# beehive-lab/GPULlama3.java

Measured on NVIDIA H100. Metric: decode_tokens_per_s, higher is better.
Workload: dtype q8_0xq8_0->int32, f32 accumulate

## Files before the change

### gpullama3.java_b200/csrc/decode_kernels.cuh

```cuda
#pragma once
#include "common.cuh"
#include "seqsum2.cuh"

enum { MODE_STORE = 0, MODE_RESID = 1 };

__device__ __forceinline__ float emb_get_raw(const DevMat &e, int token, int i) {
    size_t idx = (size_t)token * e.cols + i;
    if (e.type == 8) {
        float q = (float)((const int8_t *)e.qs)[idx];
        return __fmul_rn(q, __half2float(e.sc[idx >> 5]));
    } else if (e.type == 1) {
        return __half2float(((const __half *)e.qs)[idx]);
    }
    return ((const float *)e.qs)[idx];
}
__device__ __forceinline__ float emb_get(const DevMat &e, int token, int i, float es) { return __fmul_rn(emb_get_raw(e, token, i), es); }

#define NORM_THREADS SEQSUM2_THREADS
__host__ __device__ inline int norm_padded(int dim) { return (dim + SEQSUM2_THREADS - 1) / SEQSUM2_THREADS * SEQSUM2_THREADS; }
__host__ __device__ inline size_t norm_smem_bytes(int dim) { return (size_t)norm_padded(dim) * 4 + 16 + seqsum2_scratch_bytes(); }

template <bool EMBED>
__device__ __forceinline__ void rmsnorm_quant_row(float *__restrict__ x, const int *__restrict__ tok, const DevMat &emb, float emb_scale,
                                                  const float *__restrict__ w, float eps, int dim, int8_t *__restrict__ xq,
                                                  float *__restrict__ xs, float *__restrict__ xb, long long *__restrict__ prof,
                                                  const TraceBuf &tr, const TpCtx &tp, int tp_wait_op) {
    extern __shared__ __align__(16) float sm[];
    float *sq = sm;
    __shared__ float s_ss;
    const int tid = threadIdx.x;
    long long t0 = 0, t1 = 0, t2 = 0, t3 = 0;
    if (prof) t0 = clock64();
    trace_entry(tr);
    pdl_launch_dependents();
    pdl_wait();
    trace_mark(tr, 2);
    if (prof) t1 = clock64();
    if (tp.n > 1 && tp_wait_op >= 0) {
        if (tid == 0) tp_wait(tp, TP_SLOT_X, tp_seq(tp, (unsigned)tp_wait_op));
        __syncthreads();
    }
    int token = 0;
    if (EMBED) token = *tok;
    for (int i = tid; i < dim; i += NORM_THREADS) {
        float v;
        if (EMBED) { v = emb_get(emb, token, i, emb_scale); x[i] = v; }
        else v = ldcg_f32c(x + i);
        sq[i] = __fmul_rn(v, v);
    }
    for (int i = dim + tid; i < norm_padded(dim); i += NORM_THREADS) sq[i] = 0.0f;
    __syncthreads();
    if (prof) t2 = clock64();
    int info0 = 0, info1 = 0;
    SeqSum2Scratch scratch = seqsum2_carve(reinterpret_cast<unsigned char *>(sm + norm_padded(dim)));
    float ss = block_seqsum_exact_v2(sq, dim, scratch);
    if (prof && tid == 0) { info0 = scratch.info[0]; info1 = scratch.info[1]; }
    if (prof) t3 = clock64();
    if (EMBED) __threadfence_block();
    if (tid == 0) {
        ss = __fdiv_rn(ss, (float)dim);
        ss = __fadd_rn(ss, eps);
        s_ss = (float)(1.0 / sqrt((double)ss));
    }
    __syncthreads();
    ss = s_ss;
    const int lane = tid & 31, warp = tid >> 5;
    constexpr int NWN = NORM_THREADS / 32;
    const int nb = dim / 32;
#pragma unroll 1
    for (int b0 = warp; b0 < nb; b0 += 4 * NWN) {
        float xv[4], wv[4];
#pragma unroll
        for (int u = 0; u < 4; u++) {
            const int b = b0 + u * NWN;
            xv[u] = 0.0f; wv[u] = 0.0f;
            if (b < nb) { xv[u] = ldcg_f32c(x + b * 32 + lane); wv[u] = w[b * 32 + lane]; }
        }
#pragma unroll
        for (int u = 0; u < 4; u++) {
            const int b = b0 + u * NWN;
            if (b < nb) {
                const int i = b * 32 + lane;
                const float v = __fmul_rn(wv[u], __fmul_rn(ss, xv[u]));
                if (xb) xb[i] = v;
                if (xq) {
                    float as;
                    int q = quant_block_lane(v, as);
                    xq[i] = (int8_t)q;
                    if (lane == 0) xs[b] = as;
                }
            }
        }
    }
    trace_mark(tr, 3);
    if (prof) {
        __syncthreads();
        if (tid == 0) { long long t4 = clock64(); prof[0] = t1 - t0; prof[1] = t2 - t1; prof[2] = t3 - t2; prof[3] = t4 - t3;
                        prof[4] = info0; prof[5] = info1; prof[6] = 0; }
    }
}

template <bool EMBED>
__global__ void __launch_bounds__(NORM_THREADS, 1) k_rmsnorm_quant(float *__restrict__ x, const StepState *__restrict__ st,
                                                               DevMat emb, float emb_scale, const float *__restrict__ w, float eps, int dim,
                                                               int8_t *__restrict__ xq, float *__restrict__ xs,
                                                               float *__restrict__ xb, long long *__restrict__ prof, TraceBuf tr, TpCtx tp, int tp_wait_op) {
    rmsnorm_quant_row<EMBED>(x, &st->token, emb, emb_scale, w, eps, dim, xq, xs, xb, prof, tr, tp, tp_wait_op);
}

template <int T>
__global__ void __launch_bounds__(T, 1) k_test_seqsum2(const float *__restrict__ terms, int n, float *__restrict__ out, int *__restrict__ info) {
    extern __shared__ __align__(16) float sm[];
    float *sq = sm;
    const int E = (n + T - 1) / T, np = T * E;
    SeqSum2Scratch scratch = seqsum2_carve(reinterpret_cast<unsigned char *>(sm + np), T);
    for (int i = threadIdx.x; i < np; i += T) sq[i] = i < n ? terms[i] : 0.0f;
    if (threadIdx.x == 0) { scratch.info[0] = -1; scratch.info[1] = -2; }
    __syncthreads();
    const float s = block_seqsum_exact_v2_t<T>(sq, n, scratch, (int)threadIdx.x, SeqSum2BlockSync());
    if (threadIdx.x == 0) { out[0] = s; info[0] = scratch.info[0]; info[1] = scratch.info[1]; }
}

template <int R>
__device__ __forceinline__ void q8_row_terms(const int8_t *__restrict__ qs, const __half *__restrict__ sc, size_t row0,
                                             int cols, int nb, const int4 *__restrict__ sxq, const float *__restrict__ sxs,
                                             float *__restrict__ terms, int nbp, int lane) {
    constexpr int JB = R >= 4 ? 2 : 4;
    for (int b0 = 0; b0 < nb; b0 += 32 * JB) {
        int wv[R][JB][8];
        __half sv[R][JB];
#pragma unroll
        for (int r = 0; r < R; r++)
#pragma unroll
            for (int j = 0; j < JB; j++) {
                int b = b0 + j * 32 + lane;
                if (b < nb) {
                    ldg256_stream(qs + (row0 + r) * (size_t)cols + (size_t)b * 32, wv[r][j]);
                    sv[r][j] = sc[(row0 + r) * (size_t)nb + b];
                }
            }
#pragma unroll
        for (int j = 0; j < JB; j++) {
            int b = b0 + j * 32 + lane;
            if (b < nb) {
                int4 a0 = sxq[b], a1 = sxq[nb + b];
                float as = sxs[b];
#pragma unroll
                for (int r = 0; r < R; r++) {
                    int isum = __dp4a(wv[r][j][0], a0.x, 0);
                    isum = __dp4a(wv[r][j][1], a0.y, isum);
                    isum = __dp4a(wv[r][j][2], a0.z, isum);
                    isum = __dp4a(wv[r][j][3], a0.w, isum);
                    isum = __dp4a(wv[r][j][4], a1.x, isum);
                    isum = __dp4a(wv[r][j][5], a1.y, isum);
                    isum = __dp4a(wv[r][j][6], a1.z, isum);
                    isum = __dp4a(wv[r][j][7], a1.w, isum);
                    terms[r * nbp + b] = __fmul_rn((float)isum, __fmul_rn(__half2float(sv[r][j]), as));
                }
            }
        }
    }
}

__device__ __forceinline__ void stage_activation(const int8_t *__restrict__ xq, const float *__restrict__ xs, int cols,
                                                 int4 *sxq, float *sxs) {
    const int nb = cols >> 5;
    const int4 *src = reinterpret_cast<const int4 *>(xq);
    for (int c = threadIdx.x; c < cols / 16; c += blockDim.x) sxq[(c & 1) * nb + (c >> 1)] = src[c];
    for (int b = threadIdx.x; b < nb; b += blockDim.x) sxs[b] = xs[b];
}

__host__ __device__ inline size_t q8_smem_bytes(int cols, int rows_per_warp, int warps) {
    int nb = cols / 32, nbp = nb | 1;
    return (size_t)cols + (size_t)nb * 4 + (size_t)warps * rows_per_warp * nbp * 4 + 64;
}

template <int R, int MODE>
__global__ void __launch_bounds__(256) k_matvec_q8(const int8_t *__restrict__ qs, const __half *__restrict__ sc,
                                                   const int8_t *__restrict__ xq, const float *__restrict__ xs, int rows,
                                                   int cols, float *__restrict__ out, float oscale) {
    extern __shared__ __align__(16) unsigned char smraw[];
    const int nb = cols >> 5, nbp = nb | 1;
    int4 *sxq = reinterpret_cast<int4 *>(smraw);
    float *sxs = reinterpret_cast<float *>(smraw + cols);
    float *terms_all = sxs + nb;
    stage_activation(xq, xs, cols, sxq, sxs);
    __syncthreads();
    const int lane = threadIdx.x & 31, warp = threadIdx.x >> 5;
    float *terms = terms_all + (size_t)warp * R * nbp;
    const int nwarps_total = gridDim.x * (blockDim.x >> 5);
    for (size_t row0 = (size_t)(blockIdx.x * (blockDim.x >> 5) + warp) * R; row0 < (size_t)rows; row0 += (size_t)nwarps_total * R) {
        q8_row_terms<R>(qs, sc, row0, cols, nb, sxq, sxs, terms, nbp, lane);
        __syncwarp();
        if (lane < R) {
            const float *t = terms + lane * nbp;
            float acc = 0.0f;
            for (int b = 0; b < nb; b++) acc = __fadd_rn(acc, t[b]);
            size_t row = row0 + lane;
            acc = __fmul_rn(acc, oscale);
            if (MODE == MODE_RESID) out[row] = __fadd_rn(out[row], acc);
            else out[row] = acc;
        }
        __syncwarp();
    }
}

__device__ __forceinline__ float swiglu(float g, float u) {
    float s = __fdiv_rn(g, (float)(1.0 + exp((double)(-g))));
    return __fmul_rn(s, u);
}

__global__ void __launch_bounds__(256) k_gateup_q8(const int8_t *__restrict__ qs1, const __half *__restrict__ sc1,
                                                   const int8_t *__restrict__ qs3, const __half *__restrict__ sc3,
                                                   const int8_t *__restrict__ xq, const float *__restrict__ xs, int hidden,
                                                   int cols, int8_t *__restrict__ hq, float *__restrict__ hs,
                                                   float *__restrict__ hb_dbg) {
    extern __shared__ __align__(16) unsigned char smraw[];
    __shared__ float hvals[32];
    const int nb = cols >> 5, nbp = nb | 1;
    int4 *sxq = reinterpret_cast<int4 *>(smraw);
    float *sxs = reinterpret_cast<float *>(smraw + cols);
    float *terms_all = sxs + nb;
    stage_activation(xq, xs, cols, sxq, sxs);
    __syncthreads();
    const int lane = threadIdx.x & 31, warp = threadIdx.x >> 5;
    float *terms = terms_all + (size_t)warp * 4 * nbp;
    for (int blk = blockIdx.x; blk < hidden / 32; blk += gridDim.x) {
#pragma unroll 1
        for (int half = 0; half < 2; half++) {
            int u0 = blk * 32 + warp * 4 + half * 2;
            q8_row_terms<2>(qs1, sc1, (size_t)u0, cols, nb, sxq, sxs, terms, nbp, lane);
            q8_row_terms<2>(qs3, sc3, (size_t)u0, cols, nb, sxq, sxs, terms + 2 * nbp, nbp, lane);
            __syncwarp();
            float acc = 0.0f;
            if (lane < 4) {
                const float *t = terms + lane * nbp;
                for (int b = 0; b < nb; b++) acc = __fadd_rn(acc, t[b]);
            }
            float up = __shfl_down_sync(0xffffffffu, acc, 2);
            if (lane < 2) hvals[warp * 4 + half * 2 + lane] = swiglu(acc, up);
            __syncwarp();
        }
        __syncthreads();
        if (warp == 0) {
            float v = hvals[lane];
            if (hb_dbg) hb_dbg[blk * 32 + lane] = v;
            float as;
            int q = quant_block_lane(v, as);
            hq[blk * 32 + lane] = (int8_t)q;
            if (lane == 0) hs[blk] = as;
        }
        __syncthreads();
    }
}

template <int MODE>
__global__ void __launch_bounds__(256) k_matvec_f16(const __half *__restrict__ w, const float *__restrict__ x, int rows,
                                                    int cols, int lanes, float *__restrict__ out, float oscale) {
    extern __shared__ __align__(16) unsigned char smraw[];
    float *sx = reinterpret_cast<float *>(smraw);
    constexpr int TC = 256;
    __half *tiles = reinterpret_cast<__half *>(smraw + (size_t)cols * 4);
    for (int i = threadIdx.x; i < cols; i += blockDim.x) sx[i] = x[i];
    __syncthreads();
    const int lane = threadIdx.x & 31, warp = threadIdx.x >> 5;
    const int L = lanes > 0 ? lanes : 1;
    const int RW = 32 / L;
    __half *tile = tiles + (size_t)warp * RW * TC;
    const int r = lane / L, c = lane % L;
    const int nwarps_total = gridDim.x * (blockDim.x >> 5);
    const int upper = lanes > 0 ? cols - (cols % L) : 0;
    for (size_t row0 = (size_t)(blockIdx.x * (blockDim.x >> 5) + warp) * RW; row0 < (size_t)rows; row0 += (size_t)nwarps_total * RW) {
        float acc = 0.0f;
        for (int c0 = 0; c0 < cols; c0 += TC) {
            int tc = min(TC, cols - c0);
            int chunks_per_row = tc >> 3;
            for (int q = lane; q < RW * chunks_per_row; q += 32) {
                int rr = q / chunks_per_row, cc = q % chunks_per_row;
                size_t row = row0 + rr;
                int4 v = make_int4(0, 0, 0, 0);
                if (row < (size_t)rows) v = ldg128_stream(w + row * (size_t)cols + c0 + cc * 8);
                *reinterpret_cast<int4 *>(tile + rr * TC + cc * 8) = v;
            }
            __syncwarp();
            if (lanes > 0) {
                int lim = min(tc, upper - c0);
                for (int i = c; i < lim; i += L) {
                    float wf = f16_bits_to_f32_daz(__half_as_ushort(tile[r * TC + i]));
                    acc = fmaf(wf, sx[c0 + i], acc);
                }
            } else {
                for (int i = 0; i < tc; i++) acc = __fadd_rn(acc, __fmul_rn(__half2float(tile[r * TC + i]), sx[c0 + i]));
            }
            __syncwarp();
        }
        float result = acc;
        if (lanes > 0) {
            result = 0.0f;
            for (int k = 0; k < L; k++) {
                float a = __shfl_sync(0xffffffffu, acc, r * L + k);
                result = __fadd_rn(result, a);
            }
            size_t row = row0 + r;
            if (row < (size_t)rows)
                for (int j = upper; j < cols; j++)
                    result = __fadd_rn(result, __fmul_rn(__half2float(w[row * (size_t)cols + j]), sx[j]));
        }
        size_t row = row0 + r;
        if (c == 0 && row < (size_t)rows) {
            result = __fmul_rn(result, oscale);
            if (MODE == MODE_RESID) out[row] = __fadd_rn(out[row], result);
            else out[row] = result;
        }
    }
}

__global__ void k_swiglu(float *__restrict__ hb, const float *__restrict__ hb2, int n) {
    int i = blockIdx.x * blockDim.x + threadIdx.x;
    if (i < n) hb[i] = swiglu(hb[i], hb2[i]);
}

#define ATT_THREADS 512

template <int HS>
__device__ __forceinline__ void rope_kv_prologue(float *qkv, const float *qsrc, const float *ksrc, const float *vsrc, float *kc, float *vc, int pos,
                                                 int h, int kv_mul, int kvh, int qd, int kvd, const float *cr, const float *ci, int arch,
                                                 const float *qnorm_w, const float *knorm_w, const float *qkv_bias, float eps, float *sq, float *sk,
                                                 float *so, float *s_val) {
    const int tid = threadIdx.x;
    constexpr int HALF = HS / 2;
    if (tid < HS) {
        const bool is_q = tid < HALF;
        const int p = is_q ? tid : tid - HALF;
        const float *src = is_q ? qsrc : ksrc;
        int i0, i1;
        if (arch & KF_NEOX) { i0 = p; i1 = p + HALF; } else { i0 = 2 * p; i1 = 2 * p + 1; }
        float v0 = src[i0], v1 = src[i1];
        if (arch & KF_QKVBIAS) {
            const float *b = qkv_bias + (is_q ? h * HS : qd + kvh * HS);
            v0 = __fadd_rn(v0, b[i0]);
            v1 = __fadd_rn(v1, b[i1]);
        }
        if (arch & KF_QKNORM) {
            float *sqr = is_q ? so : sk;
            sqr[i0] = __fmul_rn(v0, v0);
            sqr[i1] = __fmul_rn(v1, v1);
        }
        if (arch & KF_QKNORM) {
            asm volatile("bar.sync 3, %0;" ::"n"(HS) : "memory");
            if (p == 0) {
                const float *sqr = is_q ? so : sk;
                float ss = 0.0f;
                for (int i = 0; i < HS; i++) ss = __fadd_rn(ss, sqr[i]);
                ss = __fdiv_rn(ss, (float)HS);
                ss = __fadd_rn(ss, eps);
                s_val[is_q ? 0 : 1] = (float)(1.0 / sqrt((double)ss));
            }
            asm volatile("bar.sync 3, %0;" ::"n"(HS) : "memory");
            const float ss = s_val[is_q ? 0 : 1];
            const float *nw = is_q ? qnorm_w : knorm_w;
            v0 = __fmul_rn(nw[i0], __fmul_rn(ss, v0));
            v1 = __fmul_rn(nw[i1], __fmul_rn(ss, v1));
            asm volatile("bar.sync 3, %0;" ::"n"(HS) : "memory");
        }
        const float fcr = cr[(size_t)pos * HALF + p], fci = ci[(size_t)pos * HALF + p];
        const float r0 = __fsub_rn(__fmul_rn(v0, fcr), __fmul_rn(v1, fci));
        const float r1 = __fadd_rn(__fmul_rn(v0, fci), __fmul_rn(v1, fcr));
        float *dst = is_q ? sq : sk;
        dst[i0] = r0;
        dst[i1] = r1;
        if (h % kv_mul == 0) {
            if (!is_q) {
                const size_t o = (size_t)pos * kvd + kvh * HS;
                kc[o + i0] = r0;
                kc[o + i1] = r1;
            }
        }
        if (is_q) { qkv[h * HS + i0] = r0; qkv[h * HS + i1] = r1; }
    } else if (tid < 2 * HS) {
        const int j = tid - HS;
        float w = vsrc[j];
        if (arch & KF_QKVBIAS) {
            w = __fadd_rn(w, qkv_bias[qd + kvd + kvh * HS + j]);
            so[j] = w;
        }
        if (h % kv_mul == 0) vc[(size_t)pos * kvd + kvh * HS + j] = w;
    }
}

template <bool CG, typename T> __device__ __forceinline__ T kv_ld(const T *p) {
    if constexpr (CG) return __ldcg(p);
    else return __ldg(p);
}

template <int HS, bool CACHED = false>
__device__ __forceinline__ void attention_head(float *__restrict__ qkv, float *__restrict__ kc, float *__restrict__ vc,
                                               const int *__restrict__ posp, const float *__restrict__ cr, const float *__restrict__ ci,
                                               int n_heads, int n_kv_heads, int arch, const float *__restrict__ qnorm_w,
                                               const float *__restrict__ knorm_w, const float *__restrict__ qkv_bias, float eps, float sqrt_hs,
                                               int8_t *__restrict__ xq, float *__restrict__ xs, float *__restrict__ xb, const TraceBuf &tr,
                                               const TpCtx &tp, unsigned tp_out_op, int head_base, float *att_scratch, int ctx) {
    extern __shared__ __align__(16) float sm[];
    __shared__ float red[ATT_THREADS / 32];
    __shared__ float s_val[2];
    float *sq = sm, *sk = sm + HS, *so = sm + 2 * HS;
    float *att = att_scratch ? att_scratch + (size_t)blockIdx.x * ctx : sm + 3 * HS;
    const int h = blockIdx.x, tid = threadIdx.x, lane = tid & 31, warp = tid >> 5;
    trace_entry(tr);
    pdl_launch_dependents();
    const int kv_mul = n_heads / n_kv_heads, kvh = h / kv_mul;
    const int qd = n_heads * HS, kvd = n_kv_heads * HS;
    pdl_wait();
    trace_mark(tr, 2);
    const int pos = *posp, nt = pos + 1;
    {
        constexpr int LINES = HS / 32;
        for (int i = tid; i < pos * LINES; i += ATT_THREADS) {
            const size_t off = (size_t)(i / LINES) * kvd + kvh * HS + (i % LINES) * 32;
            asm volatile("prefetch.global.L2 [%0];" ::"l"(kc + off));
            asm volatile("prefetch.global.L2 [%0];" ::"l"(vc + off));
        }
    }
    const float *qsrc = qkv + h * HS, *ksrc = qkv + qd + kvh * HS, *vsrc = qkv + qd + kvd + kvh * HS;
// ... 229 lines not shown
```

### gpullama3.java_b200/csrc/decode_persistent.cuh

```cuda
#pragma once
#include "decode_kernels.cuh"
#include "norm_slots.cuh"
#include "seqsum2.cuh"
#include "stream_matvec.cuh"

#define PD_WARPS 16
#define PD_CT (PD_WARPS * 32)
#define PD_THREADS (PD_CT + 32)
#define PD_MAX_STAGES 32
#define PD_TIMEOUT_NS 4000000000ull
#define PD_STAMPS 20

enum { PD_S_QKV = 0, PD_S_ATT = 1, PD_S_WO = 2, PD_S_GU = 3, PD_S_W2 = 4, PD_S_LM = 5, PD_S_ARG = 6, PD_S_SLOTS = 8,
       PD_S_TICK = 8, PD_S_LMTICK = 9, PD_S_ERR = 10, PD_S_WORDS = 16 };

struct PdLayer {
    TileMat qkv, wo, gu, w2;
    const float *attn_norm, *ffn_norm, *q_norm, *k_norm;
    const float *qkv_bias;
    float *kc, *vc;
};

struct PdArgs {
    const PdLayer *layers;
    int n_layers;
    TileMat lm_head;
    const float *out_norm;
    DevMat emb;
    int dim, hidden, qd;
    int n_heads, n_kv_heads;
    int head_size, arch , ctx;
    float eps, sqrt_hs;
    float emb_scale, res_scale, logit_scale;
    const float *rope_cr, *rope_ci;
    StepState *st;
    const int *seq_tokens;
    int *out_ids;
    float *x, *qkv, *hb, *logits;
    int8_t *attq;
    float *atts;
    int8_t *hq;
    float *hs;
    unsigned *blk_cnt;
    float *part_val;
    int *part_idx;
    unsigned *sync;
    unsigned *host_err;
    float *att_scratch;
    unsigned long long *trace;
    int with_logits;
    TpCtx tp;
    unsigned pd_flags_off;
    int head_base, dim_base, hid_base, voc_base;
};

struct PdSmem {
    size_t off_bar, off_xq, off_xs, off_nbuf, off_wbuf, off_rope, off_seq, off_terms, off_hvals, off_misc, off_ring, total;
    int stages, stage_bytes, tstride, nbuf_floats;
};

__host__ __device__ inline PdSmem pd_layout(int dim, int qd, int hidden, int head_size, int att_floats, int max_seg, size_t budget) {
    PdSmem L;
    const int unit = smv_unit_bytes(max_seg);
    L.stage_bytes = (4 * unit + 127) & ~127;
    L.tstride = ((max_seg / 32 + 3) & ~3) + 4;
    int maxc = dim > qd ? dim : qd;
    if (hidden > maxc) maxc = hidden;
    const int E = (dim + PD_CT - 1) / PD_CT;
    const int sq_floats = PD_CT * seqsum2_stride(E);
    L.nbuf_floats = sq_floats > att_floats ? sq_floats : att_floats;
    size_t o = 0;
    L.off_bar = o; o += 2 * PD_MAX_STAGES * 8 + PD_MAX_STAGES * 4;
    o = (o + 15) & ~(size_t)15;
    L.off_xq = o; o += (size_t)maxc;
    L.off_xs = o; o += (size_t)(maxc / 32) * 4;
    o = (o + 15) & ~(size_t)15;
    L.off_nbuf = o; o += (size_t)L.nbuf_floats * 4;
    o = (o + 15) & ~(size_t)15;
    L.off_wbuf = o; o += (size_t)dim * 4;
    L.off_rope = o; o += (size_t)head_size * 4;
    o = (o + 15) & ~(size_t)15;
    L.off_seq = o; o += seqsum2_scratch_bytes(PD_CT);
    o = (o + 15) & ~(size_t)15;
    L.off_terms = o; o += (size_t)PD_WARPS * 4 * L.tstride * 4;
    L.off_hvals = o; o += SMV_HVALS * 4;
    L.off_misc = o; o += 96 * 4;
    o = (o + 127) & ~(size_t)127;
    L.off_ring = o;
    long room = (long)budget - (long)o;
    int s = room > 0 ? (int)(room / L.stage_bytes) : 0;
    if (s > PD_MAX_STAGES) s = PD_MAX_STAGES;
    L.stages = s;
    L.total = o + (size_t)s * L.stage_bytes;
    return L;
}

__device__ __forceinline__ unsigned pd_ld_relaxed_gpu(const unsigned *p) {
    unsigned v;
    asm volatile("ld.relaxed.gpu.global.u32 %0, [%1];" : "=r"(v) : "l"(p) : "memory");
    return v;
}
__device__ __forceinline__ unsigned pd_ld_relaxed_sys(const unsigned *p) {
    unsigned v;
    asm volatile("ld.relaxed.sys.global.u32 %0, [%1];" : "=r"(v) : "l"(p) : "memory");
    return v;
}
template <bool SYS> __device__ __noinline__ void pd_spin(const unsigned *p, unsigned target, unsigned *err, unsigned *host_err, unsigned code) {
    unsigned it = 0;
    unsigned long long t0 = 0;
    for (;;) {
        const unsigned v = SYS ? pd_ld_relaxed_sys(p) : pd_ld_relaxed_gpu(p);
        if ((int)(v - target) >= 0) {
            unsigned w;
            if (SYS) asm volatile("ld.acquire.sys.global.u32 %0, [%1];" : "=r"(w) : "l"(p) : "memory");
            else asm volatile("ld.acquire.gpu.global.u32 %0, [%1];" : "=r"(w) : "l"(p) : "memory");
            return;
        }
        if ((++it & 255u) == 0u) {
            if (*reinterpret_cast<volatile unsigned *>(err)) return;
            const unsigned long long now = gtime();
            if (!t0) t0 = now;
            else if (now - t0 > PD_TIMEOUT_NS) {
                atomicCAS(err, 0u, code);
                *reinterpret_cast<volatile unsigned *>(host_err) = code;
                return;
            }
        }
    }
}

__device__ __forceinline__ void pd_bar_sync() { asm volatile("bar.sync 1, %0;" ::"n"(PD_CT) : "memory"); }

struct PdConsumerSync {
    __device__ __forceinline__ void operator()() const { pd_bar_sync(); }
};

__device__ __noinline__ void pd_arrive(const PdArgs &a, int slot, unsigned target, unsigned epoch, bool cross, int tid) {
    pd_bar_sync();
    if (tid == 0) {
        const bool x = cross && a.tp.n > 1;
        __threadfence();
        const unsigned old = atomicAdd(a.sync + slot, 1u);
        if (x && old + 1u == target) {
            __threadfence_system();
            for (int k = 0; k < a.tp.n; k++) {
                unsigned *f = reinterpret_cast<unsigned *>(a.tp.peer[k] + a.pd_flags_off) + slot * TP_MAX + a.tp.rank;
                asm volatile("st.relaxed.sys.global.u32 [%0], %1;" ::"l"(f), "r"(epoch) : "memory");
            }
        }
    }
}
__device__ __noinline__ void pd_wait(const PdArgs &a, int slot, unsigned target, unsigned epoch, bool cross, int tid) {
    if (tid == 0) {
        if (cross && a.tp.n > 1) {
            const unsigned *f = reinterpret_cast<const unsigned *>(a.tp.peer[a.tp.rank] + a.pd_flags_off) + slot * TP_MAX;
            for (int k = 0; k < a.tp.n; k++) pd_spin<true>(f + k, epoch, a.sync + PD_S_ERR, a.host_err, 1u + (unsigned)slot);
        } else pd_spin<false>(a.sync + slot, target, a.sync + PD_S_ERR, a.host_err, 1u + (unsigned)slot);
    }
    pd_bar_sync();
}

__device__ __forceinline__ void pd_stamp(const PdArgs &a, int layer, int k, int tid) {
    if (a.trace && tid == 0) a.trace[((size_t)blockIdx.x * (a.n_layers + 1) + layer) * PD_STAMPS + k] = gtime();
}

struct PdWalk {
    const PdArgs *a;
    int n_mats, mi;
    TileMat W;
    int g1, gb, nw, s, w;
    unsigned tile_bytes;
    __device__ __forceinline__ void open() {
        for (; mi < n_mats; mi++) {
            const int l = mi >> 2;
            if (l < a->n_layers) {
                const PdLayer &Ly = a->layers[l];
                const int k = mi & 3;
                W = k == 0 ? Ly.qkv : k == 1 ? Ly.wo : k == 2 ? Ly.gu : Ly.w2;
            } else W = a->lm_head;
            const int ngroups = tile_groups(W);
            gb = (int)(((long long)blockIdx.x * ngroups) / gridDim.x);
            g1 = (int)(((long long)(blockIdx.x + 1) * ngroups) / gridDim.x);
            if (gb < g1) {
                nw = min(PD_WARPS, g1 - gb);
                s = 0; w = 0;
                tile_bytes = 4u * (unsigned)W.unit_bytes;
                return;
            }
        }
    }
    __device__ __forceinline__ void init(const PdArgs *args) {
        a = args;
        n_mats = 4 * a->n_layers + (a->with_logits ? 1 : 0);
        mi = 0;
        open();
    }
    __device__ __forceinline__ bool valid() const { return mi < n_mats; }
    __device__ __forceinline__ const unsigned char *addr() const { return W.base + ((size_t)(gb + w) * W.nseg + s) * tile_bytes; }
    __device__ __forceinline__ void next() {
        if (++w < nw) return;
        w = 0;
        if (++s < W.nseg) return;
        s = 0;
        gb += PD_WARPS;
        if (gb < g1) { nw = min(PD_WARPS, g1 - gb); return; }
        mi++;
        open();
    }
};

__device__ __forceinline__ void pd_produce(const PdArgs &a, unsigned char *smem, const PdSmem &L, unsigned bar0) {
    const int S = L.stages;
    const unsigned long long pol = l2_policy_evict_first();
    PdWalk cur;
    cur.init(&a);
    for (unsigned seq = 0; cur.valid(); cur.next(), seq++) {
        const int st = seq % S;
        mbar_wait(bar0 + 8 * (PD_MAX_STAGES + st), ((seq / S) & 1u) ^ 1u);
        const unsigned full = bar0 + 8 * st;
        mbar_expect_tx(full, cur.tile_bytes);
        bulk_g2s_evict_first(smem_u32(smem + L.off_ring + (size_t)st * L.stage_bytes), cur.addr(), cur.tile_bytes, full, pol);
    }
}

__device__ __noinline__ float pd_walk_rolled(float acc, const float *t, int nbs) {
    int b = 0;
    if (nbs >= 4) {
        float4 c = *reinterpret_cast<const float4 *>(t);
#pragma unroll 1
        for (; b + 4 <= nbs; b += 4) {
            float4 n = c;
            if (b + 8 <= nbs) n = *reinterpret_cast<const float4 *>(t + b + 4);
            acc = __fadd_rn(acc, c.x); acc = __fadd_rn(acc, c.y); acc = __fadd_rn(acc, c.z); acc = __fadd_rn(acc, c.w);
            c = n;
        }
    }
#pragma unroll 1
    for (; b < nbs; b++) acc = __fadd_rn(acc, t[b]);
    return acc;
}
__device__ __noinline__ float pd_swiglu(float g, float u) { return swiglu_exact(g, u); }
__device__ __noinline__ int pd_quant_block(float v, float *ascale) {
    float as;
    const int q = quant_block_lane(v, as);
    *ascale = as;
    return q;
}
__device__ __noinline__ float pd_emb_get(const DevMat &e, int token, int i, float es) { return emb_get(e, token, i, es); }
__device__ __noinline__ float pd_exp_narrow(float x) { return (float)exp((double)x); }

template <int MODE>
__device__ __noinline__ void pd_consume_matrix(const TileMat &W, const PdArgs &a, unsigned char *smem, const PdSmem &L, unsigned bar0, volatile unsigned *rel,
                                                  unsigned &seq_base, float *out, bool argmax, bool l0_emb, int token, int row_base, int tid) {
    const int lane = tid & 31, warp = tid >> 5, S = L.stages, tstride = L.tstride, stage_bytes = L.stage_bytes;
    const int w_unit = W.unit_bytes, w_seg = W.seg;
    const int ngroups = tile_groups(W);
    const float oscale = MODE == SMV_RESID ? a.res_scale : argmax ? a.logit_scale : 1.0f;
    const int g0 = (int)(((long long)blockIdx.x * ngroups) / gridDim.x), g1 = (int)(((long long)(blockIdx.x + 1) * ngroups) / gridDim.x);
    const int nseg = W.nseg, nbs = w_seg >> 5;
    const unsigned char *ring = smem + L.off_ring;
    const int tp_n = a.tp.n;
    float *terms = reinterpret_cast<float *>(smem + L.off_terms) + (size_t)warp * 4 * tstride;
    const unsigned char *sact = smem + L.off_xq;
    const float *sxs = reinterpret_cast<const float *>(smem + L.off_xs);
    float *hvals = reinterpret_cast<float *>(smem + L.off_hvals);
    const int hsel = (lane >> 2) & 1;
    float best = -INFINITY;
    int best_i = 0x7fffffff;
#pragma unroll 1
    for (int gb = g0; gb < g1; gb += PD_WARPS) {
        const int nw = min(PD_WARPS, g1 - gb);
        if (warp < nw) {
            const int G = gb + warp;
            float acc = 0.0f;
#pragma unroll 1
            for (int s = 0; s < nseg; s++) {
                const unsigned seq = seq_base + (unsigned)(s * nw + warp);
                const int st = seq % S;
                const unsigned lap = seq / S;
                if (lane == 0)
                    while (rel[st] != lap) {}
                __syncwarp();
                mbar_wait(bar0 + 8 * st, lap & 1u);
                const unsigned char *tile = ring + (size_t)st * stage_bytes;
#pragma unroll 1
                for (int b = lane; b < nbs; b += 32) {
                    const unsigned char *ab = sact + ((size_t)(s * nbs + b) << 5);
                    const int4 a0 = *reinterpret_cast<const int4 *>(ab + 16 * hsel);
                    const int4 a1 = *reinterpret_cast<const int4 *>(ab + 16 * (hsel ^ 1));
                    const float as = sxs[s * nbs + b];
#pragma unroll
                    for (int r = 0; r < 4; r++) {
                        const unsigned char *wb = tile + (size_t)r * w_unit + ((size_t)b << 5);
                        const int4 w0 = *reinterpret_cast<const int4 *>(wb + 16 * hsel);
                        const int4 w1 = *reinterpret_cast<const int4 *>(wb + 16 * (hsel ^ 1));
                        const __half sc = *reinterpret_cast<const __half *>(tile + (size_t)r * w_unit + w_seg + 2 * b);
                        int isum = __dp4a(w0.x, a0.x, 0);
                        isum = __dp4a(w0.y, a0.y, isum);
                        isum = __dp4a(w0.z, a0.z, isum);
                        isum = __dp4a(w0.w, a0.w, isum);
                        isum = __dp4a(w1.x, a1.x, isum);
                        isum = __dp4a(w1.y, a1.y, isum);
                        isum = __dp4a(w1.z, a1.z, isum);
                        isum = __dp4a(w1.w, a1.w, isum);
                        terms[r * tstride + b] = __fmul_rn((float)isum, __fmul_rn(__half2float(sc), as));
                    }
                }
                __syncwarp();
                if (lane == 0) {
                    rel[st] = lap + 1u;
                    mbar_arrive(bar0 + 8 * (PD_MAX_STAGES + st));
                }
                if (lane < 4) acc = pd_walk_rolled(acc, terms + lane * tstride, nbs);
                __syncwarp();
            }
            if (MODE == SMV_GATEUP) {
                const float up = __shfl_down_sync(0xffffffffu, acc, 2);
                if (lane < 2) {
                    const int unit = 2 * G + lane;
                    const float hval = pd_swiglu(acc, up);
                    out[unit] = hval;
                    hvals[unit - 2 * g0] = hval;
                }
            } else if (lane < 4 && 4 * G + lane < W.rows) {
                const size_t row = (size_t)4 * G + lane;
                acc = __fmul_rn(acc, oscale);
                if (MODE == SMV_RESID) {
                    const size_t grow = (size_t)row_base + row;
                    const float base = l0_emb ? pd_emb_get(a.emb, token, (int)grow, a.emb_scale) : out[grow];
                    const float v = __fadd_rn(base, acc);
                    if (tp_n > 1) {
                        for (int k = 0; k < tp_n; k++) tp_ptr<float>(a.tp, k, a.tp.off_x)[grow] = v;
                    } else out[grow] = v;
                } else {
                    out[row] = acc;
                    const int grow = row_base + (int)row;
                    if (acc > best) { best = acc; best_i = grow; }
                }
            }
        }
        seq_base += (unsigned)(nseg * nw);
    }
    if (MODE == SMV_GATEUP) {
        pd_bar_sync();
        const int u0 = 2 * g0, u1 = 2 * g1;
        if (u1 > u0) {
            for (int blk = (u0 >> 5) + warp; blk <= ((u1 - 1) >> 5); blk += PD_WARPS) {
                const int lo = max(blk << 5, u0), hi = min((blk << 5) + 32, u1);
                float v = 0.0f;
                bool mine = true;
                if (hi - lo == 32) v = hvals[(blk << 5) + lane - u0];
                else {
                    unsigned old = 0;
                    if (lane == 0) {
                        __threadfence();
                        old = atomicAdd(&a.blk_cnt[blk], (unsigned)(hi - lo));
                    }
                    old = __shfl_sync(0xffffffffu, old, 0);
                    mine = (old + (unsigned)(hi - lo) == 32u);
                    if (mine) {
                        __threadfence();
                        v = ldcg_f32(out + (blk << 5) + lane);
                        if (lane == 0) a.blk_cnt[blk] = 0u;
                    }
                }
                if (mine) {
                    float as;
                    const int q = pd_quant_block(v, &as);
                    const int gblk = (row_base >> 5) + blk;
                    if (a.tp.n > 1) {
                        for (int k = 0; k < a.tp.n; k++) {
                            tp_ptr<int8_t>(a.tp, k, a.tp.off_hq)[(gblk << 5) + lane] = (int8_t)q;
                            if (lane == 0) tp_ptr<float>(a.tp, k, a.tp.off_hs)[gblk] = as;
                        }
                    } else {
                        a.hq[(gblk << 5) + lane] = (int8_t)q;
                        if (lane == 0) a.hs[gblk] = as;
                    }
                }
            }
        }
    } else if (MODE == SMV_STORE && argmax) {
        int *cand_i = reinterpret_cast<int *>(hvals + 64);
        pd_bar_sync();
        if (lane < 4) { hvals[warp * 4 + lane] = best; cand_i[warp * 4 + lane] = best_i; }
        pd_bar_sync();
        if (tid == 0) {
            float bv = -INFINITY;
            int bi = 0x7fffffff;
            for (int k = 0; k < PD_WARPS * 4; k++) {
                const float v = hvals[k];
                const int ix = cand_i[k];
                if (v > bv || (v == bv && ix < bi)) { bv = v; bi = ix; }
            }
            a.part_val[blockIdx.x] = bv;
            a.part_idx[blockIdx.x] = bi;
        }
    }
}

__device__ __noinline__ float pd_seqsum(const float *sq, int n, int S, unsigned char *smem, const PdSmem &L, int tid) {
    SeqSum2Scratch scratch = seqsum2_carve(smem + L.off_seq, PD_CT);
    return block_seqsum_exact_v2_t<PD_CT>(sq, n, scratch, tid, PdConsumerSync(), S);
}

__device__ __forceinline__ void pd_prefetch_w(const float *w, float *sbuf, int dim, int tid) {
    const int n4 = dim >> 2;
    for (int i4 = tid; i4 < n4; i4 += PD_CT)
        asm volatile("cp.async.cg.shared.global [%0], [%1], 16;" ::"r"(smem_u32(sbuf + 4 * i4)), "l"(w + 4 * i4) : "memory");
    asm volatile("cp.async.commit_group;" ::: "memory");
}

struct PdNormOps {
    const PdArgs &a;
    const float *wbuf;
    unsigned char *smem;
    const PdSmem &L;
    int tid, stamp_layer;
    __device__ __forceinline__ void sync() const { pd_bar_sync(); }
    __device__ __forceinline__ float seqsum(const float *sq, int n, int S) const { return pd_seqsum(sq, n, S, smem, L, tid); }
    __device__ __forceinline__ float emb(int token, int i) const { return pd_emb_get(a.emb, token, i, a.emb_scale); }
    __device__ __forceinline__ float4 x4(int i4) const { return ldcg_f32x4(a.x + 4 * i4); }
    __device__ __forceinline__ void store_x(int, float4) const {}
    __device__ __forceinline__ float scale(float ss, int dim, float eps) const {
        float *misc = reinterpret_cast<float *>(smem + L.off_misc);
        if (tid == 0) {
            ss = __fdiv_rn(ss, (float)dim);
            ss = __fadd_rn(ss, eps);
            misc[20] = (float)(1.0 / sqrt((double)ss));
        }
        asm volatile("cp.async.wait_group 0;" ::: "memory");
        pd_bar_sync();
        return misc[20];
    }
    template <int U> __device__ __forceinline__ float4 w4(const float4 (&)[U], int, int i4) const { return *reinterpret_cast<const float4 *>(wbuf + 4 * i4); }
    __device__ __forceinline__ void stamp(int k) const { if (stamp_layer >= 0) pd_stamp(a, stamp_layer, k, tid); }
};

template <int U>
__device__ __noinline__ void pd_norm_u(const PdArgs &a, const float *wbuf, bool from_emb, int token, unsigned char *smem, const PdSmem &L, int tid, int stamp_layer) {
    const float4 wv[U] = {};
    norm_quant_slots<PD_CT, U>(PdNormOps{a, wbuf, smem, L, tid, stamp_layer}, from_emb, token, a.dim, a.eps, wv, reinterpret_cast<float *>(smem + L.off_nbuf),
                               reinterpret_cast<unsigned *>(smem + L.off_xq), reinterpret_cast<float *>(smem + L.off_xs), tid);
}

__device__ __forceinline__ void pd_norm_to_smem(const PdArgs &a, const float *wbuf, bool from_emb, int token, unsigned char *smem, const PdSmem &L, int tid, int stamp_layer = -1) {
    const int U = ((a.dim >> 2) + PD_CT - 1) / PD_CT;
    if (U <= 1) pd_norm_u<1>(a, wbuf, from_emb, token, smem, L, tid, stamp_layer);
    else if (U == 2) pd_norm_u<2>(a, wbuf, from_emb, token, smem, L, tid, stamp_layer);
    else pd_norm_u<4>(a, wbuf, from_emb, token, smem, L, tid, stamp_layer);
}

__device__ __noinline__ void pd_load_act(const int8_t *q, const float *s, int cols, unsigned char *smem, const PdSmem &L, int tid) {
    int4 *sxq = reinterpret_cast<int4 *>(smem + L.off_xq);
    float *sxs = reinterpret_cast<float *>(smem + L.off_xs);
    const int4 *src = reinterpret_cast<const int4 *>(q);
    const int n16 = cols >> 4, nb = cols >> 5;
    for (int c0 = 0; c0 < n16; c0 += 4 * PD_CT) {
        int4 v[4];
        float sc[2];
#pragma unroll
        for (int u = 0; u < 4; u++) {
            const int c = c0 + u * PD_CT + tid;
            v[u] = c < n16 ? __ldcg(src + c) : make_int4(0, 0, 0, 0);
        }
#pragma unroll
        for (int u = 0; u < 2; u++) {
            const int b = (c0 >> 1) + u * PD_CT + tid;
            sc[u] = b < nb ? __ldcg(s + b) : 0.0f;
        }
#pragma unroll
        for (int u = 0; u < 4; u++) {
            const int c = c0 + u * PD_CT + tid;
            if (c < n16) sxq[c] = v[u];
        }
#pragma unroll
        for (int u = 0; u < 2; u++) {
            const int b = (c0 >> 1) + u * PD_CT + tid;
            if (b < nb) sxs[b] = sc[u];
        }
    }
    pd_bar_sync();
}

template <int HS>
__device__ __noinline__ void pd_attention_head(const PdArgs &a, const PdLayer &Ly, int h, int pos, unsigned char *smem, const PdSmem &L, int tid, int layer) {
    float *sm = reinterpret_cast<float *>(smem + L.off_nbuf);
    float *misc = reinterpret_cast<float *>(smem + L.off_misc);
    float *red = misc, *s_val = misc + 16;
    float *sq = sm, *sk = sm + HS, *so = sm + 2 * HS;
    const int ctx_pad = (a.ctx + PD_CT - 1) / PD_CT * PD_CT;
    float *att = a.att_scratch ? a.att_scratch + (size_t)h * ctx_pad : sm + 3 * HS;
    const int lane = tid & 31, warp = tid >> 5;
    constexpr int HALF = HS / 2;
    const int nt = pos + 1;
    const int kv_mul = a.n_heads / a.n_kv_heads, kvh = h / kv_mul;
    const int qd = a.n_heads * HS, kvd = a.n_kv_heads * HS;
    float *qkv = a.qkv, *kc = Ly.kc, *vc = Ly.vc;
    const float *qsrc = qkv + h * HS, *ksrc = qkv + qd + kvh * HS, *vsrc = qkv + qd + kvd + kvh * HS;
    float vcur_own = 0.0f;
    if (tid < HS) {
        const bool is_q = tid < HALF;
        const int p = is_q ? tid : tid - HALF;
        const float *src = is_q ? qsrc : ksrc;
        int i0, i1;
        if (a.arch & KF_NEOX) { i0 = p; i1 = p + HALF; } else { i0 = 2 * p; i1 = 2 * p + 1; }
        float v0 = ldcg_f32c(src + i0), v1 = ldcg_f32c(src + i1);
        if (a.arch & KF_QKVBIAS) {
            const float *b = Ly.qkv_bias + (is_q ? h * HS : qd + kvh * HS);
            v0 = __fadd_rn(v0, b[i0]);
            v1 = __fadd_rn(v1, b[i1]);
        }
        const float *srope = reinterpret_cast<const float *>(smem + L.off_rope);
        const float fcr = srope[p], fci = srope[HALF + p];
        const bool owner = (h % kv_mul == 0) && !is_q;
        if (a.arch & KF_QKNORM) {
            float *sqr = is_q ? so : sk;
            sqr[i0] = __fmul_rn(v0, v0);
            sqr[i1] = __fmul_rn(v1, v1);
            asm volatile("bar.sync 3, %0;" ::"n"(HS) : "memory");
            if (p == 0) {
                float ss = 0.0f;
                for (int i = 0; i < HS; i++) ss = __fadd_rn(ss, sqr[i]);
                ss = __fdiv_rn(ss, (float)HS);
                ss = __fadd_rn(ss, a.eps);
                s_val[is_q ? 0 : 1] = (float)(1.0 / sqrt((double)ss));
            }
            asm volatile("bar.sync 3, %0;" ::"n"(HS) : "memory");
            const float ss = s_val[is_q ? 0 : 1];
            const float *nw = is_q ? Ly.q_norm : Ly.k_norm;
            v0 = __fmul_rn(nw[i0], __fmul_rn(ss, v0));
            v1 = __fmul_rn(nw[i1], __fmul_rn(ss, v1));
            asm volatile("bar.sync 3, %0;" ::"n"(HS) : "memory");
        }
        const float r0 = __fsub_rn(__fmul_rn(v0, fcr), __fmul_rn(v1, fci));
        const float r1 = __fadd_rn(__fmul_rn(v0, fci), __fmul_rn(v1, fcr));
        float *dst = is_q ? sq : sk;
        dst[i0] = r0;
        dst[i1] = r1;
        if (owner) {
            const size_t o = (size_t)pos * kvd + kvh * HS;
            kc[o + i0] = r0;
            kc[o + i1] = r1;
        }
    } else if (tid < 2 * HS) {
        const int j = tid - HS;
        vcur_own = ldcg_f32c(vsrc + j);
        if (a.arch & KF_QKVBIAS) vcur_own = __fadd_rn(vcur_own, Ly.qkv_bias[qd + kvd + kvh * HS + j]);
        if (h % kv_mul == 0) vc[(size_t)pos * kvd + kvh * HS + j] = vcur_own;
    }
    pd_bar_sync();
    if (tid >= HS && tid < 2 * HS) so[tid - HS] = vcur_own;
    constexpr int QE = HS / 4, QV = HS / 16;
    const int quad = tid & 3, qbase = lane & ~3;
    constexpr int VB = 32;
    const int vd = tid >> 2;
    const bool vlive = vd < HS;
    float vv[VB];
    {
        const float *vcol = vc + kvh * HS + vd;
        const int vt0 = quad * VB;
#pragma unroll
        for (int u = 0; u < VB; u++) vv[u] = (vlive && vt0 + u < pos) ? __ldcg(vcol + (size_t)(vt0 + u) * kvd) : 0.0f;
    }
    float lmax = -INFINITY;
#pragma unroll 1
    for (int t0 = 0; t0 < nt; t0 += PD_CT / 4) {
        const int t = t0 + (tid >> 2);
        float4 kk[QV];
        if (t < pos) {
            const float4 *k = reinterpret_cast<const float4 *>(kc + (size_t)t * kvd + kvh * HS + quad * QE);
#pragma unroll
            for (int u = 0; u < QV; u++) kk[u] = __ldcg(k + u);
        } else {
#pragma unroll
            for (int u = 0; u < QV; u++) kk[u] = t == pos ? *reinterpret_cast<const float4 *>(sk + quad * QE + 4 * u) : make_float4(0.f, 0.f, 0.f, 0.f);
        }
        float acc = 0.0f;
#pragma unroll 1
        for (int qd = 0; qd < 4; qd++) {
            if (quad == qd) {
                const float *qq = sq + qd * QE;
#pragma unroll
                for (int u = 0; u < QV; u++) {
                    acc = __fadd_rn(acc, __fmul_rn(qq[4 * u + 0], kk[u].x));
                    acc = __fadd_rn(acc, __fmul_rn(qq[4 * u + 1], kk[u].y));
                    acc = __fadd_rn(acc, __fmul_rn(qq[4 * u + 2], kk[u].z));
                    acc = __fadd_rn(acc, __fmul_rn(qq[4 * u + 3], kk[u].w));
                }
            }
            acc = __shfl_sync(0xffffffffu, acc, qbase + qd);
        }
        if (quad == 0 && t < nt) {
            const float sc = (a.arch & KF_ATTSCALE) ? __fmul_rn(acc, a.sqrt_hs) : __fdiv_rn(acc, a.sqrt_hs);
            att[t] = sc;
            lmax = fmaxf(lmax, sc);
        }
    }
    lmax = warp_max_f(lmax);
    if (lane == 0) red[warp] = lmax;
    pd_bar_sync();
    pd_stamp(a, layer, 13, tid);
    float mx = red[0];
#pragma unroll
    for (int w = 1; w < PD_WARPS; w++) mx = fmaxf(mx, red[w]);
    for (int t = tid; t < nt; t += PD_CT) att[t] = pd_exp_narrow(__fsub_rn(att[t], mx));
    pd_bar_sync();
    float sum;
    if (nt >= 512) {
        const int E = (nt + PD_CT - 1) / PD_CT;
        for (int t = nt + tid; t < PD_CT * E; t += PD_CT) att[t] = 0.0f;
        pd_bar_sync();
        sum = pd_seqsum(att, nt, 0, smem, L, tid);
    } else {
        if (tid == 0) s_val[0] = seq2_literal(0.0f, att, nt, (reinterpret_cast<uintptr_t>(att) & 15) == 0);
        pd_bar_sync();
        sum = s_val[0];
    }
    for (int t = tid; t < nt; t += PD_CT) att[t] = __fdiv_rn(att[t], sum);
    pd_bar_sync();
    pd_stamp(a, layer, 14, tid);
    {
        const float *vcol = vc + kvh * HS + vd;
        const float vcur = vlive ? so[vd] : 0.0f;
        float acc = 0.0f;
#pragma unroll 1
        for (int r0 = 0; r0 < pos; r0 += 4 * VB) {
            if (r0 > 0) {
                const int vt0 = r0 + quad * VB;
#pragma unroll
                for (int u = 0; u < VB; u++) vv[u] = (vlive && vt0 + u < pos) ? __ldcg(vcol + (size_t)(vt0 + u) * kvd) : 0.0f;
            }
#pragma unroll 1
            for (int qd = 0; qd < 4; qd++) {
                if (quad == qd) {
                    const int vt0 = r0 + qd * VB;
#pragma unroll
                    for (int u = 0; u < VB; u++)
                        if (vt0 + u < pos) acc = __fadd_rn(__fmul_rn(att[vt0 + u], vv[u]), acc);
                }
                acc = __shfl_sync(0xffffffffu, acc, qbase + qd);
            }
        }
        if (vlive && quad == 0) so[vd] = __fadd_rn(__fmul_rn(att[pos], vcur), acc);
    }
    pd_bar_sync();
    const int gh = a.head_base + h;
    for (int b = warp; b < HS / 32; b += PD_WARPS) {
        float as;
        const int q = pd_quant_block(so[b * 32 + lane], &as);
        if (a.tp.n > 1) {
            for (int k = 0; k < a.tp.n; k++) {
                tp_ptr<int8_t>(a.tp, k, a.tp.off_attq)[gh * HS + b * 32 + lane] = (int8_t)q;
                if (lane == 0) tp_ptr<float>(a.tp, k, a.tp.off_atts)[(gh * HS) / 32 + b] = as;
            }
        } else {
            a.attq[gh * HS + b * 32 + lane] = (int8_t)q;
            if (lane == 0) a.atts[(gh * HS) / 32 + b] = as;
        }
    }
    pd_stamp(a, layer, 15, tid);
}

template <int HS>
__global__ void __launch_bounds__(PD_THREADS, 1) k_decode_persistent(const __grid_constant__ PdArgs a, const __grid_constant__ PdSmem L) {
    extern __shared__ __align__(128) unsigned char smem[];
    const int tid = threadIdx.x, lane = tid & 31, warp = tid >> 5;
    const int S = L.stages;
    const unsigned bar0 = smem_u32(smem + L.off_bar);
    volatile unsigned *rel = reinterpret_cast<volatile unsigned *>(smem + L.off_bar + 2 * PD_MAX_STAGES * 8);
    if (tid == 0) {
        for (int s = 0; s < S; s++) {
            mbar_init(bar0 + 8 * s, 1);
            mbar_init(bar0 + 8 * (PD_MAX_STAGES + s), 1);
            rel[s] = 0u;
        }
        asm volatile("fence.mbarrier_init.release.cluster;" ::: "memory");
    }
    __syncthreads();

    if (warp == PD_WARPS) {
        if (lane == 0) pd_produce(a, smem, L, bar0);
        return;
    }

    const int token = a.st->token, pos = a.st->pos;
    const unsigned tick = *reinterpret_cast<volatile unsigned *>(a.sync + PD_S_TICK);
    const unsigned lmtick = *reinterpret_cast<volatile unsigned *>(a.sync + PD_S_LMTICK);
    const unsigned nC = gridDim.x, nL = (unsigned)a.n_layers, nH = (unsigned)a.n_heads;
    float *wbufA = reinterpret_cast<float *>(smem + L.off_wbuf), *wbufF = wbufA;
    pd_prefetch_w(a.n_layers ? a.layers[0].attn_norm : a.out_norm, wbufA, a.dim, tid);
    if (tid < a.head_size) {
        const int half = a.head_size >> 1;
        float *srope = reinterpret_cast<float *>(smem + L.off_rope);
        srope[tid] = tid < half ? __ldg(a.rope_cr + (size_t)pos * half + tid) : __ldg(a.rope_ci + (size_t)pos * half + (tid - half));
    }
    unsigned seq_base = 0;
#pragma unroll 1
    for (int l = 0; l < a.n_layers; l++) {
        const PdLayer &Ly = a.layers[l];
        const unsigned e = tick * nL + (unsigned)l + 1u;
        pd_stamp(a, l, 0, tid);
        pd_norm_to_smem(a, wbufA, l == 0, token, smem, L, tid, l);
        if (a.trace && l == 1) {
            const int E = (a.dim + PD_CT - 1) / PD_CT;
            pd_stamp(a, l, 16, tid);
            const float again = pd_seqsum(reinterpret_cast<const float *>(smem + L.off_nbuf), a.dim, seqsum2_stride(E), smem, L, tid);
            if (tid == 0) reinterpret_cast<float *>(smem + L.off_misc)[30] = again;
            pd_stamp(a, l, 17, tid);
        }
        pd_prefetch_w(Ly.ffn_norm, wbufF, a.dim, tid);
        pd_stamp(a, l, 1, tid);
        pd_consume_matrix<SMV_STORE>(Ly.qkv, a, smem, L, bar0, rel, seq_base, a.qkv, false, false, token, 0, tid);
        pd_stamp(a, l, 2, tid);
        if (blockIdx.x < nH) {
            const int kvh = (int)blockIdx.x / (a.n_heads / a.n_kv_heads), kvd = a.n_kv_heads * a.head_size;
            const int lines = a.head_size >> 5;
            for (int i = tid; i < pos * lines; i += PD_CT) {
                const size_t off = (size_t)(i / lines) * kvd + kvh * a.head_size + (i % lines) * 32;
                asm volatile("prefetch.global.L2 [%0];" ::"l"(Ly.kc + off));
                asm volatile("prefetch.global.L2 [%0];" ::"l"(Ly.vc + off));
            }
        }
        pd_arrive(a, PD_S_QKV, e * nC, e, false, tid);
        if (blockIdx.x < nH) {
            pd_wait(a, PD_S_QKV, e * nC, e, false, tid);
            pd_stamp(a, l, 12, tid);
            pd_attention_head<HS>(a, Ly, blockIdx.x, pos, smem, L, tid, l);
            pd_arrive(a, PD_S_ATT, e * nH, e, true, tid);
        }
        pd_wait(a, PD_S_ATT, e * nH, e, true, tid);
        pd_stamp(a, l, 3, tid);
        pd_load_act(a.attq, a.atts, a.qd, smem, L, tid);
        pd_consume_matrix<SMV_RESID>(Ly.wo, a, smem, L, bar0, rel, seq_base, a.x, false, l == 0, token, a.dim_base, tid);
        pd_stamp(a, l, 4, tid);
        pd_arrive(a, PD_S_WO, e * nC, e, true, tid);
        pd_wait(a, PD_S_WO, e * nC, e, true, tid);
        pd_stamp(a, l, 5, tid);
        pd_norm_to_smem(a, wbufF, false, token, smem, L, tid);
        pd_prefetch_w(l + 1 < a.n_layers ? a.layers[l + 1].attn_norm : a.out_norm, wbufA, a.dim, tid);
        pd_stamp(a, l, 6, tid);
        pd_consume_matrix<SMV_GATEUP>(Ly.gu, a, smem, L, bar0, rel, seq_base, a.hb, false, false, token, a.hid_base, tid);
        pd_stamp(a, l, 7, tid);
        pd_arrive(a, PD_S_GU, e * nC, e, true, tid);
        pd_wait(a, PD_S_GU, e * nC, e, true, tid);
        pd_load_act(a.hq, a.hs, a.hidden, smem, L, tid);
        pd_stamp(a, l, 8, tid);
        pd_consume_matrix<SMV_RESID>(Ly.w2, a, smem, L, bar0, rel, seq_base, a.x, false, false, token, a.dim_base, tid);
        pd_stamp(a, l, 9, tid);
        pd_arrive(a, PD_S_W2, e * nC, e, true, tid);
        pd_wait(a, PD_S_W2, e * nC, e, true, tid);
    }
    int best_i = 0;
    if (a.with_logits) {
        const unsigned le = lmtick + 1u;
        pd_stamp(a, a.n_layers, 0, tid);
        pd_norm_to_smem(a, wbufA, false, token, smem, L, tid);
        pd_stamp(a, a.n_layers, 1, tid);
        pd_consume_matrix<SMV_STORE>(a.lm_head, a, smem, L, bar0, rel, seq_base, a.logits, true, false, token, a.voc_base, tid);
        pd_stamp(a, a.n_layers, 2, tid);
        pd_arrive(a, PD_S_LM, le * nC, le, false, tid);
        if (blockIdx.x != 0) return;
        pd_wait(a, PD_S_LM, le * nC, le, false, tid);
        float best = -INFINITY;
        best_i = 0x7fffffff;
        for (int i = tid; i < (int)nC; i += PD_CT) argmax_merge(best, best_i, ldcg_f32c(a.part_val + i), __ldcg(a.part_idx + i));
#pragma unroll
        for (int o = 16; o > 0; o >>= 1) {
            const float ov = __shfl_xor_sync(0xffffffffu, best, o);
            const int oi = __shfl_xor_sync(0xffffffffu, best_i, o);
            argmax_merge(best, best_i, ov, oi);
        }
        float *sv = reinterpret_cast<float *>(smem + L.off_misc) + 32;
        int *si = reinterpret_cast<int *>(sv + 16);
        if (lane == 0) { sv[warp] = best; si[warp] = best_i; }
        pd_bar_sync();
        if (tid == 0) {
            best = sv[0]; best_i = si[0];
            for (int w = 1; w < PD_WARPS; w++) argmax_merge(best, best_i, sv[w], si[w]);
            if (a.tp.n > 1) {
                for (int k = 0; k < a.tp.n; k++) {
                    tp_ptr<float>(a.tp, k, a.tp.off_pv)[a.tp.rank] = best;
                    tp_ptr<int>(a.tp, k, a.tp.off_pi)[a.tp.rank] = best_i;
                }
                __threadfence_system();
                for (int k = 0; k < a.tp.n; k++) {
                    unsigned *f = reinterpret_cast<unsigned *>(a.tp.peer[k] + a.pd_flags_off) + PD_S_ARG * TP_MAX + a.tp.rank;
                    asm volatile("st.relaxed.sys.global.u32 [%0], %1;" ::"l"(f), "r"(le) : "memory");
                }
                const unsigned *f = reinterpret_cast<const unsigned *>(a.tp.peer[a.tp.rank] + a.pd_flags_off) + PD_S_ARG * TP_MAX;
                for (int k = 0; k < a.tp.n; k++) pd_spin<true>(f + k, le, a.sync + PD_S_ERR, a.host_err, 1u + PD_S_ARG);
                best = -INFINITY; best_i = 0x7fffffff;
                for (int k = 0; k < a.tp.n; k++)
                    argmax_merge(best, best_i, ldcg_f32c(tp_ptr<float>(a.tp, a.tp.rank, a.tp.off_pv) + k),
                                 __float_as_int(ldcg_f32c(reinterpret_cast<const float *>(tp_ptr<int>(a.tp, a.tp.rank, a.tp.off_pi)) + k)));
            }
            if (best_i == 0x7fffffff) best_i = 0;
        }
    } else if (blockIdx.x != 0) {
        return;
    }
    if (tid == 0) {
        StepState *st = a.st;
        const int step = st->step;
        if (a.with_logits && a.out_ids) a.out_ids[step] = best_i;
        const int next = step + 1;
        if (st->feedback && a.with_logits) st->token = best_i;
        else if (next < st->n_seq) st->token = a.seq_tokens[next];
        st->step = next;
        st->pos = st->pos + 1;
        *reinterpret_cast<volatile unsigned *>(a.sync + PD_S_TICK) = tick + 1u;
        if (a.with_logits) *reinterpret_cast<volatile unsigned *>(a.sync + PD_S_LMTICK) = lmtick + 1u;
        pd_stamp(a, a.n_layers, 3, tid);
    }
}
```

### gpullama3.java_b200/csrc/plan.cu

```cuda
#include "../../include/b200llama.h"
#include "decode_kernels.cuh"
#include "prefill.cuh"
#include "stream_matvec.cuh"
#include "stream_matvec_f16.cuh"
#include "kquant.cuh"
#include "decode_persistent.cuh"
#include "sampler.cuh"
#include "decode_batch.cuh"
#include "moe.cuh"

#include <math.h>
#include <stdarg.h>
#include <stdio.h>
#include <stdlib.h>
#include <string.h>

#include <chrono>
#include <string>
#include <thread>
#include <utility>
#include <vector>

namespace {

// ... 2169 lines not shown
                        (long long)start_positions[i] + lengths[i] - 1, c.context_length);
        off[i] = (int)total;
        total += lengths[i];
    }
    if (total && !tokens) return fail(p, B200_ERR_BAD_ARG, "tokens must not be NULL");
    for (int i = 0; i < n_seqs; i++)
        for (int j = 0; j < lengths[i]; j++)
            if (tokens[off[i] + j] < 0 || tokens[off[i] + j] >= c.vocab_size)
                return fail(p, B200_ERR_BAD_ARG, "sequence %d: token %d (index %d) out of range", i, tokens[off[i] + j], j);
    const PrefillCtx &pc = p->prefill;
    const bool tc = (pc.ready && pc.mode == B200_PREFILL_TENSOR_CORE) || (pc.q8_ready && pc.mode == B200_PREFILL_TENSOR_CORE_W8A16);
    if (tc && total > p->prefill_batch) {
        int i = 0;
        while (off[i] + lengths[i] <= p->prefill_batch) i++;
        return fail(p, B200_ERR_BAD_ARG, "sequence %d: the call's %lld tokens exceed prefill_batch_size %d (split the prompts into chunks)", i, (long long)total,
                    p->prefill_batch);
    }
    if (!total) return B200_OK;
    CK(cudaSetDevice(p->device));
    return tc ? prefill_slots_tc(p, n_seqs, slots, start_positions, lengths, off.data(), tokens, (int)total)
              : prefill_slots_exact(p, n_seqs, slots, start_positions, lengths, off.data(), tokens);
}

int b200_decode_multi_rows(b200_plan *p, int32_t *max_rows) {
    if (!p || !max_rows) return B200_ERR_BAD_ARG;
    *max_rows = multi_why(p) ? 0 : batch_max_rows(p);
    return B200_OK;
}

int b200_forward_decode_multi(b200_plan *p, int32_t slot, int32_t n, const int32_t *tokens, int32_t start_pos, int32_t *ids_out, float *logits) {
    if (!p) return B200_ERR_BAD_ARG;
    if (const char *why = multi_why(p)) return fail(p, B200_ERR_UNSUPPORTED, "%s", why);
    auto &B = p->bt;
    const b200_config &c = p->cfg;
    const int R = batch_max_rows(p);
    if (!tokens || !ids_out) return fail(p, B200_ERR_BAD_ARG, "tokens and ids_out must not be NULL");
    if (n < 1 || n > R) return fail(p, B200_ERR_BAD_ARG, "n = %d rows: need 1 <= n <= %d (b200_decode_multi_rows)", n, R);
    if (slot < -1 || slot >= B.n_slots) return fail(p, B200_ERR_BAD_ARG, "slot %d out of range (%d slots; -1 is the plan's own cache)", slot, B.n_slots);
    for (int i = 0; i < n; i++) {
        if (tokens[i] < 0 || tokens[i] >= c.vocab_size) return fail(p, B200_ERR_BAD_ARG, "row %d: token %d out of range", i, tokens[i]);
        if (start_pos < 0 || (int64_t)start_pos + i >= c.context_length)
            return fail(p, B200_ERR_BAD_ARG, "row %d: position %lld outside the KV cache (%d)", i, (long long)start_pos + i, c.context_length);
    }
    CK(cudaSetDevice(p->device));
    int rc;
    if ((rc = multi_ready(p))) return rc;
    const bool own = slot < 0;
    if (!B.gs[own][1][n] && (rc = capture_batch(p, n, false, true, own))) return rc;
    for (int i = 0; i < n; i++) { B.h_rows->token[i] = tokens[i]; B.h_rows->pos[i] = start_pos + i; B.h_rows->slot[i] = own ? 0 : slot; }
    CK(cudaMemcpyAsync(B.rows, B.h_rows, sizeof(BatchRows), cudaMemcpyHostToDevice, p->stream));
    CK(cudaGraphLaunch(B.gs[own][1][n], p->stream));
    const size_t vpad = (size_t)sampler_padded(c.vocab_size);
    if (logits)
        for (int i = 0; i < n; i++) CK(cudaMemcpyAsync(logits + (size_t)i * c.vocab_size, B.logits + i * vpad, (size_t)c.vocab_size * 4, cudaMemcpyDeviceToHost, p->stream));
    CK(cudaMemcpyAsync(B.h_out, B.ids, (size_t)n * 4, cudaMemcpyDeviceToHost, p->stream));
    CK(cudaStreamSynchronize(p->stream));
    memcpy(ids_out, B.h_out, (size_t)n * 4);
    return B200_OK;
}

int b200_batch_info(b200_plan *p, int32_t *n_slots, int32_t *launches_per_step, float *device_ms_last_step) {
    if (!p) return B200_ERR_BAD_ARG;
    if (n_slots) *n_slots = p->bt.n_slots;
    if (launches_per_step) *launches_per_step = p->bt.last_n ? p->bt.launches[p->bt.last_n] : 0;
    if (device_ms_last_step) *device_ms_last_step = p->bt.last_ms;
    return B200_OK;
}

int b200_read_buffer(b200_plan *p, const char *name, int32_t layer, void *dst, size_t bytes) {
    if (!p || !name || !dst) return B200_ERR_BAD_ARG;
    const b200_config &c = p->cfg;
    const void *src = nullptr;
    size_t sz = 0;
    std::string s = name;
    size_t ctx_kv = (size_t)c.context_length * p->kvd_l;
    if (s == "x") { src = p->x; sz = (size_t)c.dim * 4; }
    else if (s == "xb") { src = p->xb; sz = (size_t)(c.dim > p->qd ? c.dim : p->qd) * 4; }
    else if (s == "q" || s == "qkv") { src = p->qkv; sz = (size_t)(p->qd_l + 2 * p->kvd_l) * 4; }
    else if (s == "hb") { src = p->hb; sz = (size_t)(c.hidden_dim > p->moe_hv ? c.hidden_dim : p->moe_hv) * 4; }
    else if (s == "logits") { src = p->logits; sz = (size_t)c.vocab_size * 4; }
    else if (s == "xq") { src = p->xq; sz = (size_t)(c.dim > p->qd ? c.dim : p->qd); }
    else if (s == "xs") { src = p->xs; sz = (size_t)((c.dim > p->qd ? c.dim : p->qd) / 32) * 4; }
    else if (s == "hq") { src = p->hq; sz = (size_t)(c.hidden_dim > p->moe_hv ? c.hidden_dim : p->moe_hv); }
    else if (s == "hs") { src = p->hs; sz = (size_t)((c.hidden_dim > p->moe_hv ? c.hidden_dim : p->moe_hv) / 32) * 4; }
    else if (s == "moe_ids" || s == "moe_weights") {
        if (!p->is_moe) return fail(p, B200_ERR_BAD_ARG, "%s: not a Qwen2-MoE plan", name);
        const size_t k = (size_t)p->moe.n_experts_used;
        if (s == "moe_ids") { src = p->moe_ids; sz = (size_t)c.n_layers * k * 4; }
        else { src = p->moe_w; sz = (size_t)c.n_layers * (k + 1) * 4; }
    }
    else if (s == "key_cache" || s == "value_cache") {
        if (layer < 0 || layer >= c.n_layers) return fail(p, B200_ERR_BAD_ARG, "layer out of range");
        src = (s == "key_cache" ? p->key_cache : p->value_cache) + (size_t)layer * ctx_kv;
        sz = ctx_kv * 4;
    } else if (s == "slot_key_cache" || s == "slot_value_cache") {
        if (layer < 0 || layer >= p->bt.n_slots * c.n_layers) return fail(p, B200_ERR_BAD_ARG, "slot layer %d out of range (%d slots)", layer, p->bt.n_slots);
        src = (s == "slot_key_cache" ? p->bt.slot_k : p->bt.slot_v) + (size_t)layer * ctx_kv;
        sz = ctx_kv * 4;
    } else if (s.rfind("pf_", 0) == 0) {
        const PrefillCtx &pc = p->prefill;
        if (!pc.ready && !pc.q8_ready) return fail(p, B200_ERR_STATE, "%s: the plan has no tensor-core prefill buffers (%s)", name, pc.why);
        const size_t rows = (size_t)pc.bpad;
        if (s == "pf_x") { src = pc.X; sz = rows * c.dim * 4; }
        else if (s == "pf_qkv") { src = pc.QKV; sz = rows * (p->qd + 2 * p->kvd) * 4; }
        else if (s == "pf_a16") { src = pc.A16; sz = rows * c.dim * 2; }
        else if (s == "pf_att16") { src = pc.ATT16; sz = rows * p->qd * 2; }
        else if (s == "pf_h16") { src = pc.H16; sz = rows * c.hidden_dim * 2; }
        else return fail(p, B200_ERR_BAD_ARG, "unknown buffer %s", name);
    } else return fail(p, B200_ERR_BAD_ARG, "unknown buffer %s", name);
    if (bytes < sz) sz = bytes;
    CK(cudaSetDevice(p->device));
    CK(cudaStreamSynchronize(p->stream));
    CK(cudaMemcpy(dst, src, sz, cudaMemcpyDeviceToHost));
    return B200_OK;
}

int b200_time_kernel(b200_plan *p, int32_t which, int32_t reps, float *avg_ms, int64_t *algorithmic_bytes) {
    if (!p || !avg_ms || reps <= 0) return B200_ERR_BAD_ARG;
    if (p->cfg.tp_size > 1) return fail(p, B200_ERR_UNSUPPORTED, "b200_time_kernel is single-GPU only");
    if (p->is_moe) return fail(p, B200_ERR_UNSUPPORTED, "b200_time_kernel times the dense FFN and attention matrices; a Qwen2-MoE plan has no dense FFN");
    const b200_config &c = p->cfg;
    const bool q8 = p->wtype == B200_GGML_Q8_0;
    CK(cudaSetDevice(p->device));
    std::vector<float> save(c.dim);
    CK(cudaStreamSynchronize(p->stream));
    CK(cudaMemcpy(save.data(), p->x, (size_t)c.dim * 4, cudaMemcpyDeviceToHost));
    if (p->use_stream) {
        auto tb = [&](const TileMat &m) -> int64_t { return (int64_t)m.rows * m.cols / 32 * 34; };
        int64_t bytes = 0;
        int launches = 0, rc;
        auto one = [&](int l) -> int {
            LayerW &L = p->layers[l];
            bool keep = p->use_pdl;
            p->use_pdl = false;
            int r;
            const bool fz = p->fuse_norm;
            const int64_t nw = fz ? (int64_t)c.dim * 4 : 0;
            switch (which) {
            case 0:
                bytes = tb(L.tgu) + nw;
                r = fz ? launch_stream_norm<SMV_GATEUP>(p, L.tgu, L.ffn_norm, false, p->hb, p->hq, p->hs, false, TraceBuf{nullptr, 0, 0})
                       : launch_stream<SMV_GATEUP>(p, L.tgu, p->xq, p->xs, p->hb, p->hq, p->hs);
                break;
            case 1: bytes = tb(L.tw2); r = launch_stream<SMV_RESID>(p, L.tw2, p->hq, p->hs, p->x, nullptr, nullptr); break;
            case 2:
                bytes = tb(L.tqkv) + nw;
                r = fz ? launch_stream_norm<SMV_STORE>(p, L.tqkv, L.attn_norm, false, p->qkv, nullptr, nullptr, false, TraceBuf{nullptr, 0, 0})
                       : launch_stream<SMV_STORE>(p, L.tqkv, p->xq, p->xs, p->qkv, nullptr, nullptr);
                break;
            case 3: bytes = tb(L.two); r = launch_stream<SMV_RESID>(p, L.two, p->xq, p->xs, p->x, nullptr, nullptr); break;
            default:
                bytes = tb(p->tout) + nw;
                r = fz ? launch_stream_norm<SMV_STORE>(p, p->tout, p->out_norm, false, p->logits, nullptr, nullptr, false, TraceBuf{nullptr, 0, 0})
                       : launch_stream<SMV_STORE>(p, p->tout, p->xq, p->xs, p->logits, nullptr, nullptr);
                break;
            }
            p->use_pdl = keep;
            return r;
        };
        if (which < 0 || which > 4) return fail(p, B200_ERR_BAD_ARG, "unknown kernel id %d", which);
        for (int l = 0; l < c.n_layers; l++) if ((rc = one(l))) return rc;
        CK(cudaEventRecord(p->ev0, p->stream));
        for (int r = 0; r < reps; r++)
            for (int l = 0; l < c.n_layers; l++) { if ((rc = one(l))) return rc; launches++; }
        CK(cudaEventRecord(p->ev1, p->stream));
        CK(cudaStreamSynchronize(p->stream));
        float ms = 0;
        CK(cudaEventElapsedTime(&ms, p->ev0, p->ev1));
        *avg_ms = ms / launches;
        if (algorithmic_bytes) *algorithmic_bytes = bytes;
        CK(cudaMemcpy(p->x, save.data(), (size_t)c.dim * 4, cudaMemcpyHostToDevice));
        return B200_OK;
    }
    auto mat_bytes = [&](const DevMat &m) -> int64_t {
        int64_t e = (int64_t)m.rows * m.cols;
        return q8 ? e / 32 * 34 : e * 2;
    };
    int64_t bytes = 0;
    int launches = 0;
    const bool sf = p->use_f16_stream;
    auto one = [&](int l) -> int {
        LayerW &L = p->layers[l];
        if (sf) {
            const bool keep = p->use_pdl;
            p->use_pdl = false;
            int r;
            switch (which) {
            case 0: bytes = mat_bytes(L.w1) + mat_bytes(L.w3); r = launch_stream_f16<SF_GATEUP>(p, L.w1, &L.w3, p->xb, p->hb); break;
            case 1: bytes = mat_bytes(L.w2); r = launch_stream_f16<SF_RESID>(p, L.w2, nullptr, p->hb, p->x); break;
            case 2: bytes = mat_bytes(L.qkv); r = launch_stream_f16<SF_STORE>(p, L.qkv, nullptr, p->xb, p->qkv); break;
            case 3: bytes = mat_bytes(L.wo); r = launch_stream_f16<SF_RESID>(p, L.wo, nullptr, p->xb, p->x); break;
            default: bytes = mat_bytes(p->out); r = launch_stream_f16<SF_STORE>(p, p->out, nullptr, p->xb, p->logits); break;
            }
            p->use_pdl = keep;
            return r;
        }
        switch (which) {
        case 0:
            if (q8) {
                k_gateup_q8<<<c.hidden_dim / 32, 256, q8_smem_bytes(c.dim, 4, 8), p->stream>>>(
                    (const int8_t *)L.w1.qs, L.w1.sc, (const int8_t *)L.w3.qs, L.w3.sc, p->xq, p->xs, c.hidden_dim, c.dim, p->hq, p->hs, p->hb);
                CK(cudaGetLastError());
            } else {
                int rc;
                if ((rc = launch_matvec_f16<MODE_STORE>(p, L.w1, p->xb, p->hb))) return rc;
                if ((rc = launch_matvec_f16<MODE_STORE>(p, L.w3, p->xb, p->hb2))) return rc;
            }
            bytes = mat_bytes(L.w1) + mat_bytes(L.w3);
            return B200_OK;
        case 1: bytes = mat_bytes(L.w2); return q8 ? launch_matvec_q8<MODE_RESID>(p, L.w2, p->hq, p->hs, p->x) : launch_matvec_f16<MODE_RESID>(p, L.w2, p->hb, p->x);
        case 2: bytes = mat_bytes(L.qkv); return q8 ? launch_matvec_q8<MODE_STORE>(p, L.qkv, p->xq, p->xs, p->qkv) : launch_matvec_f16<MODE_STORE>(p, L.qkv, p->xb, p->qkv);
        case 3: bytes = mat_bytes(L.wo); return q8 ? launch_matvec_q8<MODE_RESID>(p, L.wo, p->xq, p->xs, p->x) : launch_matvec_f16<MODE_RESID>(p, L.wo, p->xb, p->x);
        default: bytes = mat_bytes(p->out); return q8 ? launch_matvec_q8<MODE_STORE>(p, p->out, p->xq, p->xs, p->logits) : launch_matvec_f16<MODE_STORE>(p, p->out, p->xb, p->logits);
        }
    };
    if (which < 0 || which > 4) return fail(p, B200_ERR_BAD_ARG, "unknown kernel id %d", which);
    int rc;
    for (int l = 0; l < c.n_layers; l++) if ((rc = one(l))) return rc;
    CK(cudaEventRecord(p->ev0, p->stream));
    for (int r = 0; r < reps; r++)
        for (int l = 0; l < c.n_layers; l++) { if ((rc = one(l))) return rc; launches++; }
    CK(cudaEventRecord(p->ev1, p->stream));
    CK(cudaStreamSynchronize(p->stream));
    float ms = 0;
    CK(cudaEventElapsedTime(&ms, p->ev0, p->ev1));
    *avg_ms = ms / launches;
    if (algorithmic_bytes) *algorithmic_bytes = bytes;
    CK(cudaMemcpy(p->x, save.data(), (size_t)c.dim * 4, cudaMemcpyHostToDevice));
    return B200_OK;
}

int b200_tp_handle(b200_plan *p, void *handle64) {
    if (!p || !handle64) return B200_ERR_BAD_ARG;
    if (p->cfg.tp_size <= 1 || !p->comm) return fail(p, B200_ERR_STATE, "not a tensor-parallel plan");
    CK(cudaSetDevice(p->device));
    cudaIpcMemHandle_t h;
    CK(cudaIpcGetMemHandle(&h, p->comm));
    static_assert(sizeof(cudaIpcMemHandle_t) == 64, "IPC handle size");
    memcpy(handle64, &h, 64);
    return B200_OK;
}

int b200_tp_attach(b200_plan *p, const void *handles, int32_t n) {
    if (!p || !handles) return B200_ERR_BAD_ARG;
    if (p->cfg.tp_size <= 1 || !p->comm) return fail(p, B200_ERR_STATE, "not a tensor-parallel plan");
    if (n != p->cfg.tp_size) return fail(p, B200_ERR_BAD_ARG, "expected %d handles, got %d", p->cfg.tp_size, n);
    if (p->attached) return fail(p, B200_ERR_STATE, "already attached");
    CK(cudaSetDevice(p->device));
    for (int k = 0; k < n; k++) {
        if (k == p->cfg.tp_rank) { p->tp.peer[k] = p->comm; continue; }
        cudaIpcMemHandle_t h;
        memcpy(&h, (const unsigned char *)handles + (size_t)k * 64, 64);
        void *ptr = nullptr;
        CK(cudaIpcOpenMemHandle(&ptr, h, cudaIpcMemLazyEnablePeerAccess));
        p->peer_open[k] = ptr;
        p->tp.peer[k] = (unsigned char *)ptr;
    }
    p->tp.n = n;
    p->attached = true;
    int rc;
    if ((rc = capture_all(p))) return rc;
    CK(cudaStreamSynchronize(p->stream));
    return B200_OK;
}

int b200_trace_decode(b200_plan *p, int32_t token, int32_t position, uint64_t *records, int32_t cap, int32_t *n_out) {
    if (!p || !records || !n_out) return B200_ERR_BAD_ARG;
    if (!p->g_trace) return fail(p, B200_ERR_UNSUPPORTED, "tracing needs a streaming path (Q8_0 tiles or the FP16 rings)");
    int rc;
    if ((rc = check_pos(p, token, position))) return rc;
    CK(cudaSetDevice(p->device));
    int n = p->launches_decode;
    std::vector<unsigned long long> init((size_t)n * 4);
    for (int i = 0; i < n; i++) { init[i * 4] = 0; init[i * 4 + 1] = ~0ull; init[i * 4 + 2] = 0; init[i * 4 + 3] = 0; }
    CK(cudaMemcpyAsync(p->trace_rec, init.data(), init.size() * 8, cudaMemcpyHostToDevice, p->stream));
    if ((rc = set_state(p, token, position, 0, 0))) return rc;
    CK(cudaGraphLaunch(p->g_trace, p->stream));
    CK(cudaStreamSynchronize(p->stream));
    int m = n < cap ? n : cap;
    CK(cudaMemcpy(records, p->trace_rec, (size_t)m * 32, cudaMemcpyDeviceToHost));
    *n_out = m;
    return B200_OK;
}

int b200_profile_norm(b200_plan *p, int64_t *cycles4) {
    if (!p || !cycles4) return B200_ERR_BAD_ARG;
    CK(cudaSetDevice(p->device));
    long long *d = nullptr;
    CK(cudaMalloc(&d, 128));
    const b200_config &c = p->cfg;
    const size_t norm_smem = norm_smem_bytes(c.dim);
    const bool q8 = p->wtype == B200_GGML_Q8_0;
    for (int i = 0; i < 3; i++)
        k_rmsnorm_quant<false><<<1, NORM_THREADS, norm_smem, p->stream>>>(p->x, p->st, p->emb, 1.0f, p->layers[0].attn_norm, c.rms_norm_eps, c.dim,
                                                                 q8 ? p->xq : nullptr, q8 ? p->xs : nullptr, q8 ? nullptr : p->xb, d, TraceBuf{nullptr, 0, 0}, p->tp, -1);
    cudaError_t e = cudaStreamSynchronize(p->stream);
    long long h[6] = {0};
    if (e == cudaSuccess) e = cudaMemcpy(h, d, sizeof(h), cudaMemcpyDeviceToHost);
    cudaFree(d);
    for (int i = 0; i < 16; i++) cycles4[i] = i < 6 ? h[i] : 0;
    return e == cudaSuccess ? B200_OK : B200_ERR_CUDA;
}

int b200_test_seqsum2(const float *terms, int32_t n, int32_t threads, float *out, int32_t *info) {
    if (!terms || !out || n <= 0 || n > 8192) return B200_ERR_BAD_ARG;
    if (threads != 256 && threads != 512 && threads != 1024) return B200_ERR_BAD_ARG;
    float *d = nullptr, *o = nullptr;
    if (cudaMalloc(&d, (size_t)n * 4) != cudaSuccess) return B200_ERR_OOM;
    if (cudaMalloc(&o, 16) != cudaSuccess) { cudaFree(d); return B200_ERR_OOM; }
    cudaError_t e = cudaMemcpy(d, terms, (size_t)n * 4, cudaMemcpyHostToDevice);
    if (e == cudaSuccess) {
        if (threads == 1024) {
            const size_t smem = (size_t)1024 * ((n + 1023) / 1024) * 4 + seqsum2_scratch_bytes(1024);
            e = cudaFuncSetAttribute(k_test_seqsum2<1024>, cudaFuncAttributeMaxDynamicSharedMemorySize, (int)smem);
            if (e == cudaSuccess) k_test_seqsum2<1024><<<1, 1024, smem>>>(d, n, o, reinterpret_cast<int *>(o) + 1);
        } else if (threads == 512) {
            const size_t smem = (size_t)512 * ((n + 511) / 512) * 4 + seqsum2_scratch_bytes(512);
            e = cudaFuncSetAttribute(k_test_seqsum2<512>, cudaFuncAttributeMaxDynamicSharedMemorySize, (int)smem);
            if (e == cudaSuccess) k_test_seqsum2<512><<<1, 512, smem>>>(d, n, o, reinterpret_cast<int *>(o) + 1);
        } else {
            const size_t smem = (size_t)256 * ((n + 255) / 256) * 4 + seqsum2_scratch_bytes(256);
            e = cudaFuncSetAttribute(k_test_seqsum2<256>, cudaFuncAttributeMaxDynamicSharedMemorySize, (int)smem);
            if (e == cudaSuccess) k_test_seqsum2<256><<<1, 256, smem>>>(d, n, o, reinterpret_cast<int *>(o) + 1);
        }
    }
    if (e == cudaSuccess) e = cudaGetLastError();
    if (e == cudaSuccess) e = cudaDeviceSynchronize();
    int32_t host[3] = {0, 0, 0};
    if (e == cudaSuccess) e = cudaMemcpy(host, o, 12, cudaMemcpyDeviceToHost);
    memcpy(out, host, 4);
    if (info) { info[0] = host[1]; info[1] = host[2]; }
    cudaFree(d);
    cudaFree(o);
    return e == cudaSuccess ? B200_OK : B200_ERR_CUDA;
}

int b200_test_sample(const float *logits, int32_t n, float temperature, float topp, float uniform01, int32_t *token_out, int32_t *info, float *probs_out) {
    if (!logits || !token_out || n < 1) return B200_ERR_BAD_ARG;
    if (!(temperature > 0.0f) || !(uniform01 >= 0.0f && uniform01 < 1.0f)) return B200_ERR_BAD_ARG;
    const size_t padded = (size_t)sampler_padded(n) * 4;
    float *dl = nullptr;
    int *di = nullptr, *dout = nullptr;
    int rc = B200_OK;
    auto ok = [&](cudaError_t e) { if (e != cudaSuccess && rc == B200_OK) rc = e == cudaErrorMemoryAllocation ? B200_ERR_OOM : B200_ERR_CUDA; return rc == B200_OK; };
    if (ok(cudaMalloc(&dl, padded)) && ok(cudaMalloc(&di, (size_t)n * 4)) && ok(cudaMalloc(&dout, 8 * 4)) && ok(cudaMemset(dl, 0, padded)) &&
        ok(cudaMemcpy(dl, logits, (size_t)n * 4, cudaMemcpyHostToDevice)) && ok(cudaMemset(di, 0xFF, (size_t)n * 4)) && ok(cudaMemset(dout, 0xFF, 8 * 4)) &&
        ok(cudaFuncSetAttribute(k_sample, cudaFuncAttributeMaxDynamicSharedMemorySize, (int)sampler_smem_bytes()))) {
        SamplerArgs a;
        a.logits = dl; a.n = n; a.temperature = temperature; a.topp = topp; a.r01 = uniform01;
        a.indices = di; a.out_id = dout; a.info = dout + 1;
        k_sample<<<1, SAMPLER_THREADS, sampler_smem_bytes()>>>(a);
        int32_t h[5];
        if (ok(cudaGetLastError()) && ok(cudaDeviceSynchronize()) && ok(cudaMemcpy(h, dout, 5 * 4, cudaMemcpyDeviceToHost))) {
            *token_out = h[0];
            if (info) for (int k = 0; k < 4; k++) info[k] = h[1 + k];
            if (probs_out) ok(cudaMemcpy(probs_out, dl, (size_t)n * 4, cudaMemcpyDeviceToHost));
        }
    }
    cudaFree(dl); cudaFree(di); cudaFree(dout);
    return rc;
}

int b200_requant_kquant(int32_t ggml_type, const void *src, int64_t n_elems, void *dst_q8_0) {
    if (!src || !dst_q8_0 || n_elems <= 0 || n_elems % 256 || !kq_is_kquant(ggml_type)) return B200_ERR_BAD_ARG;
    const size_t raw = (size_t)(n_elems / 256) * kq_block_bytes(ggml_type), q8 = (size_t)(n_elems / 32) * 34;
    unsigned char *ds = nullptr, *dd = nullptr;
    int rc = B200_OK;
    auto ok = [&](cudaError_t e) { if (e != cudaSuccess && rc == B200_OK) rc = e == cudaErrorMemoryAllocation ? B200_ERR_OOM : B200_ERR_CUDA; return rc == B200_OK; };
    if (ok(cudaMalloc(&ds, raw)) && ok(cudaMalloc(&dd, q8)) && ok(cudaMemcpy(ds, src, raw, cudaMemcpyHostToDevice)) &&
        ok(launch_requant_kquant(ggml_type, ds, dd, n_elems / 32, 0)) && ok(cudaDeviceSynchronize()))
        ok(cudaMemcpy(dst_q8_0, dd, q8, cudaMemcpyDeviceToHost));
    cudaFree(ds); cudaFree(dd);
    return rc;
}

int b200_gemm_f16(const uint16_t *a, const uint16_t *b, float *c, int32_t m, int32_t n, int32_t k, int32_t iters, float *ms) {
    const int stages = getenv("B200_GEMM_STAGES") ? atoi(getenv("B200_GEMM_STAGES")) : 0;
    const int resid = getenv("B200_GEMM_RESID") ? atoi(getenv("B200_GEMM_RESID")) : 0;
    if (!a || !b || !c || m <= 0 || n <= 0 || k <= 0 || m % 128 || n % 128 || k % 64) return B200_ERR_BAD_ARG;
    __half *da = nullptr, *db = nullptr;
    float *dc = nullptr;
    cudaEvent_t e0 = nullptr, e1 = nullptr;
    int rc = B200_OK;
    auto ok = [&](cudaError_t e) { if (e != cudaSuccess && rc == B200_OK) rc = e == cudaErrorMemoryAllocation ? B200_ERR_OOM : B200_ERR_CUDA; return rc == B200_OK; };
    if (ok(cudaMalloc(&da, (size_t)m * k * 2)) && ok(cudaMalloc(&db, (size_t)n * k * 2)) && ok(cudaMalloc(&dc, (size_t)m * n * 4)) &&
        ok(cudaMemcpy(da, a, (size_t)m * k * 2, cudaMemcpyHostToDevice)) && ok(cudaMemcpy(db, b, (size_t)n * k * 2, cudaMemcpyHostToDevice)) &&
        ok(cudaMemset(dc, resid ? 0 : 0xFF, (size_t)m * n * 4))) {
        if (pg::gemm_f16(da, db, dc, m, n, k, stages, resid, 0)) rc = B200_ERR_CUDA;
        ok(cudaDeviceSynchronize());
        if (rc == B200_OK && iters > 0 && ms && ok(cudaEventCreate(&e0)) && ok(cudaEventCreate(&e1)) && ok(cudaEventRecord(e0, 0))) {
            for (int i = 0; i < iters && rc == B200_OK; i++)
                if (pg::gemm_f16(da, db, dc, m, n, k, stages, resid, 0)) rc = B200_ERR_CUDA;
            float t = 0.f;
            if (ok(cudaEventRecord(e1, 0)) && ok(cudaEventSynchronize(e1)) && ok(cudaEventElapsedTime(&t, e0, e1))) *ms = t / iters;
            if (rc == B200_OK && resid) {
                if (ok(cudaMemset(dc, 0, (size_t)m * n * 4)) && pg::gemm_f16(da, db, dc, m, n, k, stages, resid, 0)) rc = B200_ERR_CUDA;
                ok(cudaDeviceSynchronize());
            }
        }
        if (rc == B200_OK) ok(cudaMemcpy(c, dc, (size_t)m * n * 4, cudaMemcpyDeviceToHost));
    }
    if (e0) cudaEventDestroy(e0);
    if (e1) cudaEventDestroy(e1);
    cudaFree(da); cudaFree(db); cudaFree(dc);
    return rc;
}

int b200_test_gemm(int32_t mode, int32_t stages, int32_t splits, int32_t m, int32_t m_valid, int32_t n, int32_t k, const uint16_t *a, const uint16_t *b,
                   const uint16_t *b2, void *c) {
    const bool gateup = mode == pg::GEMM_GATEUP;
    if (mode < pg::GEMM_F32 || mode > pg::GEMM_GATEUP || (stages != pg::GEMM_STAGES && stages != pg::GEMM_STAGES_DEEP)) return B200_ERR_BAD_ARG;
    if (!a || !b || !c || (gateup && !b2) || m <= 0 || n <= 0 || k <= 0 || m % pg::BM || k % pg::BK || n % (gateup ? pg::BN / 2 : pg::BN)) return B200_ERR_BAD_ARG;
    if (m_valid < 1 || m_valid > m || splits < 1) return B200_ERR_BAD_ARG;
    const size_t c_bytes = (size_t)m * n * (gateup ? 2 : 4);
    __half *da = nullptr, *db = nullptr, *db2 = nullptr;
    void *dc = nullptr;
    int rc = B200_OK;
    auto ok = [&](cudaError_t e) { if (e != cudaSuccess && rc == B200_OK) rc = e == cudaErrorMemoryAllocation ? B200_ERR_OOM : B200_ERR_CUDA; return rc == B200_OK; };
    if (ok(cudaMalloc(&da, (size_t)m * k * 2)) && ok(cudaMalloc(&db, (size_t)n * k * 2)) && (!gateup || ok(cudaMalloc(&db2, (size_t)n * k * 2))) &&
        ok(cudaMalloc(&dc, c_bytes)) && ok(cudaMemcpy(da, a, (size_t)m * k * 2, cudaMemcpyHostToDevice)) &&
        ok(cudaMemcpy(db, b, (size_t)n * k * 2, cudaMemcpyHostToDevice)) && (!gateup || ok(cudaMemcpy(db2, b2, (size_t)n * k * 2, cudaMemcpyHostToDevice))) &&
        ok(cudaMemcpy(dc, c, c_bytes, cudaMemcpyHostToDevice))) {
        CUtensorMap ma, mb, mb2, mc;
        const uint32_t b_rows = gateup ? pg::BN / 2 : pg::BN;
        if (pg::make_map(&ma, da, (uint64_t)m, (uint64_t)k, pg::BM) || pg::make_map(&mb, db, (uint64_t)n, (uint64_t)k, b_rows) ||
            pg::make_map(&mb2, gateup ? db2 : db, (uint64_t)n, (uint64_t)k, b_rows) || (!gateup && pg::make_map_c(&mc, dc, (uint64_t)m, (uint64_t)n)))
            rc = B200_ERR_CUDA;
        if (gateup) mc = mb;
        int lr = 0;
        if (rc == B200_OK) {
            const int mt = m / pg::BM, nt = n / (gateup ? pg::BN / 2 : pg::BN);
            const bool deep = stages == pg::GEMM_STAGES_DEEP;
            if (mode == pg::GEMM_F32)
                lr = deep ? pg::gemm_launch<pg::GEMM_F32, pg::GEMM_STAGES_DEEP>(ma, mb, mb2, mc, dc, n, m_valid, mt, nt, k, 0, splits)
                          : pg::gemm_launch<pg::GEMM_F32, pg::GEMM_STAGES>(ma, mb, mb2, mc, dc, n, m_valid, mt, nt, k, 0, splits);
            else if (mode == pg::GEMM_RESID)
                lr = deep ? pg::gemm_launch<pg::GEMM_RESID, pg::GEMM_STAGES_DEEP>(ma, mb, mb2, mc, dc, n, m_valid, mt, nt, k, 0, splits)
                          : pg::gemm_launch<pg::GEMM_RESID, pg::GEMM_STAGES>(ma, mb, mb2, mc, dc, n, m_valid, mt, nt, k, 0, splits);
            else
                lr = deep ? pg::gemm_launch<pg::GEMM_GATEUP, pg::GEMM_STAGES_DEEP>(ma, mb, mb2, mc, dc, n, m_valid, mt, nt, k, 0, splits)
                          : pg::gemm_launch<pg::GEMM_GATEUP, pg::GEMM_STAGES>(ma, mb, mb2, mc, dc, n, m_valid, mt, nt, k, 0, splits);
            if (lr == -6) rc = B200_ERR_BAD_ARG;
            else if (lr) rc = B200_ERR_CUDA;
        }
        if (ok(cudaDeviceSynchronize()) && rc == B200_OK) ok(cudaMemcpy(c, dc, c_bytes, cudaMemcpyDeviceToHost));
    }
    cudaFree(da); cudaFree(db); cudaFree(db2); cudaFree(dc);
    return rc;
}

int b200_test_gemm_q8(int32_t mode, int32_t stages, int32_t splits, int32_t m, int32_t m_valid, int32_t n, int32_t k, const uint16_t *a, const void *bq,
                      const void *bq2, void *c) {
    const bool gateup = mode == pg::GEMM_GATEUP;
    if (mode < pg::GEMM_F32 || mode > pg::GEMM_GATEUP || (stages != pg::GEMM_STAGES && stages != pg::GEMM_STAGES_DEEP_Q8)) return B200_ERR_BAD_ARG;
    if (!a || !bq || !c || (gateup && !bq2) || m <= 0 || n <= 0 || k <= 0 || m % pg::BM || k % pg::BK || n % (gateup ? pg::BN / 2 : pg::BN)) return B200_ERR_BAD_ARG;
    if (m_valid < 1 || m_valid > m || splits < 1) return B200_ERR_BAD_ARG;
    const int nseg = smv_pick_nseg(k);
    if (!nseg || (k / nseg) % pg::BK) return B200_ERR_BAD_ARG;
    const int seg = k / nseg, unit = smv_unit_bytes(seg), rows = gateup ? 2 * n : n;
    const size_t c_bytes = (size_t)m * n * (gateup ? 2 : 4), q8_bytes = (size_t)n * (k / 32) * 34, stream_bytes = (size_t)rows * nseg * unit;
    __half *da = nullptr;
    unsigned char *draw = nullptr, *dstream = nullptr;
    void *dc = nullptr;
    int rc = B200_OK;
    auto ok = [&](cudaError_t e) { if (e != cudaSuccess && rc == B200_OK) rc = e == cudaErrorMemoryAllocation ? B200_ERR_OOM : B200_ERR_CUDA; return rc == B200_OK; };
    if (ok(cudaMalloc(&da, (size_t)m * k * 2)) && ok(cudaMalloc(&draw, q8_bytes * (gateup ? 2 : 1))) && ok(cudaMalloc(&dstream, stream_bytes)) &&
        ok(cudaMalloc(&dc, c_bytes)) && ok(cudaMemcpy(da, a, (size_t)m * k * 2, cudaMemcpyHostToDevice)) && ok(cudaMemcpy(draw, bq, q8_bytes, cudaMemcpyHostToDevice)) &&
        (!gateup || ok(cudaMemcpy(draw + q8_bytes, bq2, q8_bytes, cudaMemcpyHostToDevice))) && ok(cudaMemcpy(dc, c, c_bytes, cudaMemcpyHostToDevice))) {
        RepackSrc src{};
        src.raw[0] = draw;
        src.rows[0] = n;
        if (gateup) { src.raw[1] = draw + q8_bytes; src.rows[1] = n; }
        src.gateup = gateup ? 1 : 0;
        k_repack_tiles<<<(unsigned)((size_t)rows * nseg), 128>>>(src, dstream, rows, k, seg, nseg, unit);
        ok(cudaGetLastError());
        CUtensorMap ma, mq, ms, mc;
        if (rc == B200_OK && (pg::make_map(&ma, da, (uint64_t)m, (uint64_t)k, pg::BM) || pg::make_map_q8(&mq, dstream, (uint64_t)rows, nseg, unit, 0) ||
                              pg::make_map_q8(&ms, dstream, (uint64_t)rows, nseg, unit, 1) || (!gateup && pg::make_map_c(&mc, dc, (uint64_t)m, (uint64_t)n))))
            rc = B200_ERR_CUDA;
        if (gateup) mc = mq;
        int lr = 0;
        if (rc == B200_OK) {
            using pg::B_Q8;
            constexpr int S4 = pg::GEMM_STAGES, S5 = pg::GEMM_STAGES_DEEP_Q8;
            const int mt = m / pg::BM, nt = n / (gateup ? pg::BN / 2 : pg::BN);
            const bool deep = stages == S5;
            if (mode == pg::GEMM_F32)
                lr = deep ? pg::gemm_launch<pg::GEMM_F32, S5, B_Q8>(ma, mq, ms, mc, dc, n, m_valid, mt, nt, k, 0, splits, seg)
                          : pg::gemm_launch<pg::GEMM_F32, S4, B_Q8>(ma, mq, ms, mc, dc, n, m_valid, mt, nt, k, 0, splits, seg);
            else if (mode == pg::GEMM_RESID)
                lr = deep ? pg::gemm_launch<pg::GEMM_RESID, S5, B_Q8>(ma, mq, ms, mc, dc, n, m_valid, mt, nt, k, 0, splits, seg)
                          : pg::gemm_launch<pg::GEMM_RESID, S4, B_Q8>(ma, mq, ms, mc, dc, n, m_valid, mt, nt, k, 0, splits, seg);
            else
                lr = deep ? pg::gemm_launch<pg::GEMM_GATEUP, S5, B_Q8>(ma, mq, ms, mc, dc, n, m_valid, mt, nt, k, 0, splits, seg)
                          : pg::gemm_launch<pg::GEMM_GATEUP, S4, B_Q8>(ma, mq, ms, mc, dc, n, m_valid, mt, nt, k, 0, splits, seg);
            if (lr == -6) rc = B200_ERR_BAD_ARG;
            else if (lr) rc = B200_ERR_CUDA;
        }
        if (ok(cudaDeviceSynchronize()) && rc == B200_OK) ok(cudaMemcpy(c, dc, c_bytes, cudaMemcpyDeviceToHost));
    }
    cudaFree(da); cudaFree(draw); cudaFree(dstream); cudaFree(dc);
    return rc;
}

int b200_test_pf_attention(const float *q, const float *k, const float *v, int32_t n, int32_t start_pos, int32_t n_heads, int32_t n_kv_heads,
                           int32_t head_size, int32_t out_rows, uint16_t *out) {
    if (!q || !k || !v || !out || n < 1 || start_pos < 0 || out_rows < n || n_kv_heads < 1 || n_heads % n_kv_heads) return B200_ERR_BAD_ARG;
    const int kv_mul = n_heads / n_kv_heads, hs = head_size;
    if ((hs != 64 && hs != 128) || kv_mul > 64) return B200_ERR_BAD_ARG;
    const int qd = n_heads * hs, kvd = n_kv_heads * hs, ldq = qd + 2 * kvd, nkeys = start_pos + n;
    const size_t kv_elems = (size_t)nkeys * kvd;
    float *dqkv = nullptr, *dk = nullptr, *dv = nullptr;
    __half *dkh = nullptr, *dvh = nullptr, *dout = nullptr;
    int rc = B200_OK;
    auto ok = [&](cudaError_t e) { if (e != cudaSuccess && rc == B200_OK) rc = e == cudaErrorMemoryAllocation ? B200_ERR_OOM : B200_ERR_CUDA; return rc == B200_OK; };
    if (ok(cudaMalloc(&dqkv, (size_t)n * ldq * 4)) && ok(cudaMalloc(&dk, kv_elems * 4)) && ok(cudaMalloc(&dv, kv_elems * 4)) &&
        ok(cudaMalloc(&dkh, kv_elems * 2)) && ok(cudaMalloc(&dvh, kv_elems * 2)) && ok(cudaMalloc(&dout, (size_t)out_rows * qd * 2)) &&
        ok(cudaMemset(dqkv, 0xFF, (size_t)n * ldq * 4)) && ok(cudaMemcpy2D(dqkv, (size_t)ldq * 4, q, (size_t)qd * 4, (size_t)qd * 4, n, cudaMemcpyHostToDevice)) &&
        ok(cudaMemcpy(dk, k, kv_elems * 4, cudaMemcpyHostToDevice)) && ok(cudaMemcpy(dv, v, kv_elems * 4, cudaMemcpyHostToDevice)) &&
        ok(cudaMemcpy(dout, out, (size_t)out_rows * qd * 2, cudaMemcpyHostToDevice))) {
        const float inv_sqrt_hs = (float)(1.0 / sqrt((double)hs));
        const int qt = PM_ROWS / kv_mul;
        const dim3 ag((n + qt - 1) / qt, n_kv_heads);
        const size_t n4 = kv_elems / 4;
        k_pf_kv_to_f16<<<(unsigned)((n4 + 255) / 256 < 1184 ? (n4 + 255) / 256 : 1184), 256, 0, 0>>>(dk, dv, dkh, dvh, n4);
        if (hs == 128) {
            if (ok(cudaFuncSetAttribute(k_pf_attention_mma<128>, cudaFuncAttributeMaxDynamicSharedMemorySize, (int)pm_smem_bytes<128>())))
                k_pf_attention_mma<128><<<ag, PM_THREADS, pm_smem_bytes<128>(), 0>>>(dqkv, ldq, dkh, dvh, kvd, kv_mul, n, start_pos, inv_sqrt_hs, dout, qd);
        } else {
            if (ok(cudaFuncSetAttribute(k_pf_attention_mma<64>, cudaFuncAttributeMaxDynamicSharedMemorySize, (int)pm_smem_bytes<64>())))
                k_pf_attention_mma<64><<<ag, PM_THREADS, pm_smem_bytes<64>(), 0>>>(dqkv, ldq, dkh, dvh, kvd, kv_mul, n, start_pos, inv_sqrt_hs, dout, qd);
        }
        if (ok(cudaGetLastError()) && ok(cudaDeviceSynchronize())) ok(cudaMemcpy(out, dout, (size_t)out_rows * qd * 2, cudaMemcpyDeviceToHost));
    }
    cudaFree(dqkv); cudaFree(dk); cudaFree(dv); cudaFree(dkh); cudaFree(dvh); cudaFree(dout);
    return rc;
}

int b200_test_pf_attention_packed(int32_t n_seqs, const int32_t *lengths, const int32_t *start_positions, const float *q, const float *k, const float *v,
                                  int32_t n_heads, int32_t n_kv_heads, int32_t head_size, uint16_t *out) {
    if (!lengths || !start_positions || !q || !k || !v || !out || n_seqs < 1 || n_kv_heads < 1 || n_heads % n_kv_heads) return B200_ERR_BAD_ARG;
    const int kv_mul = n_heads / n_kv_heads, hs = head_size;
    if ((hs != 64 && hs != 128) || kv_mul > 64) return B200_ERR_BAD_ARG;
    const int qd = n_heads * hs, kvd = n_kv_heads * hs, ldq = qd + 2 * kvd;
    std::vector<int> row0(n_seqs), hrow(n_seqs);
    int n = 0, rows = 0;
    for (int i = 0; i < n_seqs; i++) {
        if (lengths[i] < 1 || start_positions[i] < 0) return B200_ERR_BAD_ARG;
        row0[i] = n; hrow[i] = rows;
        n += lengths[i]; rows += start_positions[i] + lengths[i];
    }
    const std::vector<PfTile> tiles = pf_tiles(n_seqs, lengths, start_positions, row0.data(), hrow.data(), kv_mul);
    const size_t kv_elems = (size_t)rows * kvd;
    float *dqkv = nullptr, *dk = nullptr, *dv = nullptr;
    __half *dkh = nullptr, *dvh = nullptr, *dout = nullptr;
    PfTile *dt = nullptr;
    int rc = B200_OK;
    auto ok = [&](cudaError_t e) { if (e != cudaSuccess && rc == B200_OK) rc = e == cudaErrorMemoryAllocation ? B200_ERR_OOM : B200_ERR_CUDA; return rc == B200_OK; };
    if (ok(cudaMalloc(&dqkv, (size_t)n * ldq * 4)) && ok(cudaMalloc(&dk, kv_elems * 4)) && ok(cudaMalloc(&dv, kv_elems * 4)) &&
        ok(cudaMalloc(&dkh, kv_elems * 2)) && ok(cudaMalloc(&dvh, kv_elems * 2)) && ok(cudaMalloc(&dout, (size_t)n * qd * 2)) &&
        ok(cudaMalloc(&dt, tiles.size() * sizeof(PfTile))) &&
        ok(cudaMemset(dqkv, 0xFF, (size_t)n * ldq * 4)) && ok(cudaMemcpy2D(dqkv, (size_t)ldq * 4, q, (size_t)qd * 4, (size_t)qd * 4, n, cudaMemcpyHostToDevice)) &&
        ok(cudaMemcpy(dk, k, kv_elems * 4, cudaMemcpyHostToDevice)) && ok(cudaMemcpy(dv, v, kv_elems * 4, cudaMemcpyHostToDevice)) &&
        ok(cudaMemcpy(dout, out, (size_t)n * qd * 2, cudaMemcpyHostToDevice)) &&
        ok(cudaMemcpy(dt, tiles.data(), tiles.size() * sizeof(PfTile), cudaMemcpyHostToDevice))) {
        const float inv_sqrt_hs = (float)(1.0 / sqrt((double)hs));
        const dim3 ag((unsigned)tiles.size(), n_kv_heads);
        const size_t n4 = kv_elems / 4;
        k_pf_kv_to_f16<<<(unsigned)((n4 + 255) / 256 < 1184 ? (n4 + 255) / 256 : 1184), 256, 0, 0>>>(dk, dv, dkh, dvh, n4);
        if (hs == 128) {
            if (ok(cudaFuncSetAttribute(k_pf_attention_mma_packed<128>, cudaFuncAttributeMaxDynamicSharedMemorySize, (int)pm_smem_bytes<128>())))
                k_pf_attention_mma_packed<128><<<ag, PM_THREADS, pm_smem_bytes<128>(), 0>>>(dqkv, ldq, dkh, dvh, kvd, kv_mul, dt, inv_sqrt_hs, dout, qd);
        } else {
            if (ok(cudaFuncSetAttribute(k_pf_attention_mma_packed<64>, cudaFuncAttributeMaxDynamicSharedMemorySize, (int)pm_smem_bytes<64>())))
                k_pf_attention_mma_packed<64><<<ag, PM_THREADS, pm_smem_bytes<64>(), 0>>>(dqkv, ldq, dkh, dvh, kvd, kv_mul, dt, inv_sqrt_hs, dout, qd);
        }
        if (ok(cudaGetLastError()) && ok(cudaDeviceSynchronize())) ok(cudaMemcpy(out, dout, (size_t)n * qd * 2, cudaMemcpyDeviceToHost));
    }
    cudaFree(dqkv); cudaFree(dk); cudaFree(dv); cudaFree(dkh); cudaFree(dvh); cudaFree(dout); cudaFree(dt);
    return rc;
}

int b200_upload_info(b200_plan *p, double *seconds, double *host_copy_seconds, int64_t *h2d_bytes) {
    if (!p) return B200_ERR_BAD_ARG;
    if (seconds) *seconds = p->up.total_s;
    if (host_copy_seconds) *host_copy_seconds = p->up.host_copy_s;
    if (h2d_bytes) *h2d_bytes = p->up.h2d_bytes;
    return B200_OK;
}

int b200_launches_per_decode(b200_plan *p) {
    if (!p) return 0;
    return (p->decode_mode == B200_DECODE_PERSISTENT && p->g_pdecode) ? 1 : p->launches_decode;
}
int64_t b200_device_bytes(b200_plan *p) { return p ? p->bytes : 0; }

void b200_plan_free(b200_plan *p) {
    if (!p) return;
    cudaSetDevice(p->device);
    if (p->stream) cudaStreamSynchronize(p->stream);
    prefill_free(p->prefill);
    batch_free(p);
    if (p->g_decode) cudaGraphExecDestroy(p->g_decode);
    if (p->g_prefill) cudaGraphExecDestroy(p->g_prefill);
    if (p->g_trace) cudaGraphExecDestroy(p->g_trace);
    if (p->g_pdecode) cudaGraphExecDestroy(p->g_pdecode);
    if (p->g_pprefill) cudaGraphExecDestroy(p->g_pprefill);
    if (p->g_ptrace) cudaGraphExecDestroy(p->g_ptrace);
    if (p->h_err) cudaFreeHost(p->h_err);
    for (int k = 0; k < TP_MAX; k++) if (p->peer_open[k]) cudaIpcCloseMemHandle(p->peer_open[k]);
    for (void *d : p->allocs) cudaFree(d);
    if (p->h_st) cudaFreeHost(p->h_st);
    if (p->h_ids) cudaFreeHost(p->h_ids);
    if (p->ev0) cudaEventDestroy(p->ev0);
    if (p->ev1) cudaEventDestroy(p->ev1);
    if (p->stream) cudaStreamDestroy(p->stream);
    delete p;
}

const char *b200_last_error(b200_plan *p) { return p ? p->err.c_str() : "null plan"; }
const char *b200_version(void) { return "b200llama 0.1 sm_90a"; }

}
```

### gpullama3.java_b200/csrc/sampler.cuh

```cuda
#pragma once
#include "common.cuh"
#include "seqsum2.cuh"

#define SAMPLER_THREADS 1024

struct SamplerArgs {
    float *logits;
    int n;
    float temperature, topp, r01;
    int *indices;
    int *out_id;
    int *info;
};

__host__ __device__ inline int sampler_padded(int n) { return (n + SAMPLER_THREADS - 1) / SAMPLER_THREADS * SAMPLER_THREADS; }
__host__ __device__ inline size_t sampler_smem_bytes() { return seqsum2_scratch_bytes(SAMPLER_THREADS) + 96 * 4; }

__device__ __forceinline__ int sampler_cmp(const float *p, int a, int b) {
    const float va = p[a], vb = p[b];
    return vb < va ? -1 : (vb > va ? 1 : 0);
}
__device__ void sampler_sift_down(int *arr, int from, int n, const float *p) {
    int prev = from, next;
    while ((next = 2 * prev + 1) < n) {
        const int r = 2 * prev + 2;
        if (r < n && sampler_cmp(p, arr[r], arr[next]) < 0) next = r;
        if (sampler_cmp(p, arr[next], arr[prev]) < 0) {
            const int t = arr[prev]; arr[prev] = arr[next]; arr[next] = t;
            prev = next;
        } else break;
    }
}

__global__ void __launch_bounds__(SAMPLER_THREADS, 1) k_sample(SamplerArgs a) {
    extern __shared__ __align__(16) unsigned char smp_sm[];
    SeqSum2Scratch scratch = seqsum2_carve(smp_sm, SAMPLER_THREADS);
    float *red = reinterpret_cast<float *>(smp_sm + seqsum2_scratch_bytes(SAMPLER_THREADS));
    int *redi = reinterpret_cast<int *>(red + 32);
    const int tid = threadIdx.x, lane = tid & 31, warp = tid >> 5, n = a.n;
    float *p = a.logits;

    float mx = -INFINITY;
    for (int i = tid; i < n; i += SAMPLER_THREADS) {
        const float v = __fdiv_rn(p[i], a.temperature);
        p[i] = v;
        mx = fmaxf(mx, v);
    }
    mx = warp_max_f(mx);
    if (lane == 0) red[warp] = mx;
    __syncthreads();
    mx = red[0];
    for (int w = 1; w < SAMPLER_THREADS / 32; w++) mx = fmaxf(mx, red[w]);
    for (int i = tid; i < n; i += SAMPLER_THREADS) p[i] = (float)exp((double)__fsub_rn(p[i], mx));
    __syncthreads();
    const float sum = block_seqsum_exact_v2_t<SAMPLER_THREADS>(p, n, scratch, tid, SeqSum2BlockSync());
    if (tid == 0 && a.info) { a.info[2] = scratch.info[0]; a.info[3] = scratch.info[1]; }
    __syncthreads();
    for (int i = tid; i < n; i += SAMPLER_THREADS) p[i] = __fdiv_rn(p[i], sum);
    __syncthreads();

    const bool use_topp = a.topp > 0.0f && a.topp < 1.0f;
    if (!use_topp) {
        if (tid == 0) {
            float cdf = 0.0f;
            int id = n - 1;
            for (int i = 0; i < n; i++) {
                cdf = __fadd_rn(cdf, p[i]);
                if (a.r01 < cdf) { id = i; break; }
            }
            *a.out_id = id;
            if (a.info) { a.info[0] = n; a.info[1] = n; }
        }
        return;
    }
    const float cutoff = __fdiv_rn(__fsub_rn(1.0f, a.topp), (float)(n - 1));
    __shared__ int s_base;
    if (tid == 0) s_base = 0;
    __syncthreads();
    for (int c0 = 0; c0 < n; c0 += SAMPLER_THREADS) {
        const int i = c0 + tid;
        const bool keep = i < n && p[i] >= cutoff;
        const unsigned bal = __ballot_sync(0xffffffffu, keep);
        if (lane == 0) redi[warp] = __popc(bal);
        __syncthreads();
        if (warp == 0) {
            const int c = redi[lane];
            int v = c;
#pragma unroll
            for (int d = 1; d < 32; d <<= 1) {
                const int u = __shfl_up_sync(0xffffffffu, v, d);
                if (lane >= d) v += u;
            }
            redi[lane] = v - c;
            if (lane == 31) redi[32] = v;
        }
        __syncthreads();
        if (keep) a.indices[s_base + redi[warp] + __popc(bal & ((1u << lane) - 1u))] = i;
        __syncthreads();
        if (tid == 0) s_base += redi[32];
        __syncthreads();
    }
    if (tid != 0) return;
    int *idx = a.indices;
    const int n0 = s_base;
    if (n0 == 0) {
        *a.out_id = n - 1;
        if (a.info) { a.info[0] = 0; a.info[1] = 0; }
        return;
    }
    for (int i = n0 / 2 - 1; i >= 0; --i) sampler_sift_down(idx, i, n0, p);
    float cumulative = 0.0f;
    int last = 0;
    for (int i = n0 - 1; i >= 0; i--) {
        const int t = idx[0]; idx[0] = idx[i]; idx[i] = t;
        cumulative = __fadd_rn(cumulative, p[idx[i]]);
        if (cumulative > a.topp) { last = i; break; }
        sampler_sift_down(idx, 0, i - 1, p);
    }
    const float r = __fmul_rn(a.r01, cumulative);
    float cdf = 0.0f;
    int id = idx[last];
    for (int i = n0 - 1; i >= last; i--) {
        cdf = __fadd_rn(cdf, p[idx[i]]);
        if (r < cdf) { id = idx[i]; break; }
    }
    *a.out_id = id;
    if (a.info) { a.info[0] = n0; a.info[1] = n0 - last; }
}
```

### gpullama3.java_b200/csrc/seqsum2.cuh

```cuda
#pragma once
#include "common.cuh"

#define SEQSUM2_THREADS 1024
#define SEQSUM2_LITERAL INT_MIN

struct SeqPair {
    unsigned a0, a1;
};
__device__ __forceinline__ SeqPair seq_compose(SeqPair L, SeqPair R) {
    SeqPair o;
    o.a0 = L.a0 + ((L.a0 & 1u) ? R.a1 : R.a0);
    o.a1 = L.a1 + (((1u + L.a1) & 1u) ? R.a1 : R.a0);
    o.a0 = min(o.a0, 1u << 26);
    o.a1 = min(o.a1, 1u << 26);
    return o;
}

__device__ __forceinline__ int f32_exponent(float f) { return (int)((__float_as_uint(f) >> 23) & 0xffu) - 127; }

__device__ __forceinline__ bool seq_pair(float t, int e, SeqPair &pr) {
    const unsigned tb = __float_as_uint(t);
    const int et = (int)(tb >> 23);
    pr.a0 = pr.a1 = 0u;
    if (et == 0) return true;
    const unsigned m = (tb & 0x7fffffu) | 0x800000u;
    int shift = (e + 127) - et;
    if (shift < 0) return false;
    if (shift > 25) shift = 25;
    const unsigned k = m >> shift;
    const unsigned rem = m & ((1u << shift) - 1u);
    const unsigned half = shift ? (1u << (shift - 1)) : 0u;
    if (shift && rem == half) {
        pr.a0 = k + (k & 1u);
        pr.a1 = k + ((k + 1u) & 1u);
    } else {
        pr.a0 = pr.a1 = k + ((shift && rem > half) ? 1u : 0u);
    }
    return true;
}

struct SeqItem {
    int cls;
    unsigned a0, a1;
    int last;
};

struct SeqSum2Scratch {
    float *wsum;
    SeqPair *wtail;
    int *wtail_f;
    int *wcls_last;
    int *wcls_first;
    int *wcnt;
    int *cls;
    SeqItem *items;
    float *result;
    int *info;
};
__host__ __device__ inline size_t seqsum2_scratch_bytes(int T = SEQSUM2_THREADS) {
    return 32 * 4 + 32 * sizeof(SeqPair) + 4 * 32 * 4 + (size_t)T * 4 + (size_t)T * sizeof(SeqItem) + 16 + 16;
}
__device__ __forceinline__ SeqSum2Scratch seqsum2_carve(unsigned char *p, int T = SEQSUM2_THREADS) {
    SeqSum2Scratch s;
    s.items = reinterpret_cast<SeqItem *>(p); p += (size_t)T * sizeof(SeqItem);
    s.wtail = reinterpret_cast<SeqPair *>(p); p += 32 * sizeof(SeqPair);
    s.cls = reinterpret_cast<int *>(p); p += (size_t)T * 4;
    s.wsum = reinterpret_cast<float *>(p); p += 32 * 4;
    s.wtail_f = reinterpret_cast<int *>(p); p += 32 * 4;
    s.wcls_last = reinterpret_cast<int *>(p); p += 32 * 4;
    s.wcls_first = reinterpret_cast<int *>(p); p += 32 * 4;
    s.wcnt = reinterpret_cast<int *>(p); p += 32 * 4;
    s.result = reinterpret_cast<float *>(p); p += 16;
    s.info = reinterpret_cast<int *>(p);
    return s;
}

__device__ __noinline__ void seq2_warp_segscan(SeqPair &p, int &f, int lane) {
#pragma unroll 1
    for (int d = 1; d < 32; d <<= 1) {
        const unsigned u0 = __shfl_up_sync(0xffffffffu, p.a0, d), u1 = __shfl_up_sync(0xffffffffu, p.a1, d);
        const int fu = __shfl_up_sync(0xffffffffu, f, d);
        if (lane >= d && !f) {
            SeqPair L;
            L.a0 = u0; L.a1 = u1;
            p = seq_compose(L, p);
            f = fu;
        }
    }
}

struct SeqSum2BlockSync {
    __device__ __forceinline__ void operator()() const { __syncthreads(); }
};

__host__ __device__ inline int seqsum2_stride(int E) { return (E % 4 == 0 && (E / 4) % 2 == 0) ? E + 4 : E; }

__device__ __noinline__ float seq2_literal(float s, const float *q, int E, bool vec) {
    int k = 0;
    if (vec) {
#pragma unroll 1
        for (; k + 4 <= E; k += 4) {
            const float4 v = *reinterpret_cast<const float4 *>(q + k);
            s = __fadd_rn(s, v.x); s = __fadd_rn(s, v.y); s = __fadd_rn(s, v.z); s = __fadd_rn(s, v.w);
        }
    }
#pragma unroll 1
    for (; k < E; k++) s = __fadd_rn(s, q[k]);
    return s;
}

__device__ __noinline__ float seq2_warp_scan_f(float v, int lane) {
#pragma unroll 1
    for (int d = 1; d < 32; d <<= 1) {
        const float u = __shfl_up_sync(0xffffffffu, v, d);
        if (lane >= d) v += u;
    }
    return v;
}

template <int T, class Sync>
__device__ float block_seqsum_exact_v2_t(const float *sq, int n, SeqSum2Scratch sc, int tid, Sync sync, int S = 0) {
    static_assert(T % 32 == 0 && T <= SEQSUM2_THREADS, "T threads = T/32 whole warps");
    constexpr int NW = T / 32;
    const int lane = tid & 31, warp = tid >> 5;
    const int E = (n + T - 1) / T;
    if (S == 0) S = E;
    const bool vec = ((E | S) & 3) == 0 && (reinterpret_cast<uintptr_t>(sq) & 15) == 0;
    const float *mine = sq + tid * S;

    float loc = 0.0f;
    {
        int k = 0;
        if (vec) {
#pragma unroll 1
            for (; k < E; k += 4) {
                const float4 v = *reinterpret_cast<const float4 *>(mine + k);
                loc += v.x; loc += v.y; loc += v.z; loc += v.w;
            }
        }
#pragma unroll 1
        for (; k < E; k++) loc += mine[k];
    }
    const float inc = seq2_warp_scan_f(loc, lane);
    if (lane == 31) sc.wsum[warp] = inc;
    sync();
    if (warp == 0) {
        const float w = lane < NW ? sc.wsum[lane] : 0.0f;
        const float v = seq2_warp_scan_f(w, lane);
        if (lane < NW) sc.wsum[lane] = v - w;
    }
    sync();
    const float wex = sc.wsum[warp];
    const float p_end = wex + inc, p_start = wex + (inc - loc);

    int cls = SEQSUM2_LITERAL;
    SeqPair pr;
    pr.a0 = pr.a1 = 0u;
    {
        const int e = f32_exponent(p_start);
        if (p_start > 0.0f && e > -100 && e < 128 && f32_exponent(p_end) == e) {
            const float b = __uint_as_float((unsigned)(e + 127) << 23);
            if (p_start >= b * (1.0f + 0x1p-9f) && p_end <= 2.0f * b * (1.0f - 0x1p-9f)) {
                bool ok = true;
                int k = 0;
                if (vec)
#pragma unroll 1
                    for (; k < E; k += 4) {
                        const float4 v = *reinterpret_cast<const float4 *>(mine + k);
                        SeqPair q0, q1, q2, q3;
                        const bool o0 = seq_pair(v.x, e, q0), o1 = seq_pair(v.y, e, q1), o2 = seq_pair(v.z, e, q2), o3 = seq_pair(v.w, e, q3);
                        ok = ok && o0 && o1 && o2 && o3;
                        pr = seq_compose(pr, seq_compose(seq_compose(q0, q1), seq_compose(q2, q3)));
                    }
#pragma unroll 1
                for (; ok && k < E; k++) {
                    SeqPair q;
                    if (!seq_pair(mine[k], e, q)) { ok = false; break; }
                    pr = seq_compose(pr, q);
                }
                if (ok) cls = e;
            }
        }
    }
    sc.cls[tid] = cls;
    if (lane == 31) sc.wcls_last[warp] = cls;
    if (lane == 0) sc.wcls_first[warp] = cls;
    sync();

    int prev_cls = __shfl_up_sync(0xffffffffu, cls, 1);
    if (lane == 0) prev_cls = warp ? sc.wcls_last[warp - 1] : SEQSUM2_LITERAL;
    int next_cls = __shfl_down_sync(0xffffffffu, cls, 1);
    if (lane == 31) next_cls = warp < NW - 1 ? sc.wcls_first[warp + 1] : SEQSUM2_LITERAL;
    const bool clean = cls != SEQSUM2_LITERAL;
    int f = (clean && prev_cls == cls) ? 0 : 1;
    seq2_warp_segscan(pr, f, lane);
    if (lane == 31) { sc.wtail[warp] = pr; sc.wtail_f[warp] = f; }
    sync();
    if (warp == 0) {
        SeqPair t;
        t.a0 = t.a1 = 0u;
        int tf = 1;
        if (lane < NW) { t = sc.wtail[lane]; tf = sc.wtail_f[lane]; }
        seq2_warp_segscan(t, tf, lane);
        if (lane < NW) sc.wtail[lane] = t;
    }
    sync();
    if (!f && warp > 0) pr = seq_compose(sc.wtail[warp - 1], pr);

    const bool is_item = !clean || next_cls != cls;
    const unsigned bal = __ballot_sync(0xffffffffu, is_item);
    if (lane == 0) sc.wcnt[warp] = __popc(bal);
    sync();
    if (warp == 0) {
        const int c = lane < NW ? sc.wcnt[lane] : 0;
        int v = c;
#pragma unroll 1
        for (int d = 1; d < 32; d <<= 1) {
            const int u = __shfl_up_sync(0xffffffffu, v, d);
            if (lane >= d) v += u;
        }
        if (lane < NW) sc.wcnt[lane] = v - c;
        if (lane == 31) sc.info[0] = v;
    }
    sync();
    if (is_item) {
        SeqItem it;
        it.cls = cls; it.a0 = pr.a0; it.a1 = pr.a1; it.last = tid;
        sc.items[sc.wcnt[warp] + __popc(bal & ((1u << lane) - 1u))] = it;
    }
    sync();

    if (tid == 0) {
        const int n_items = sc.info[0];
        float s = 0.0f;
        int fallbacks = 0;
        SeqItem nxt = sc.items[0];
#pragma unroll 1
        for (int i = 0; i < n_items; i++) {
            const SeqItem it = nxt;
            if (i + 1 < n_items) nxt = sc.items[i + 1];
            if (it.cls == SEQSUM2_LITERAL) {
                s = seq2_literal(s, sq + it.last * S, E, vec);
                continue;
            }
            const unsigned sb = __float_as_uint(s);
            bool ok = f32_exponent(s) == it.cls && (sb >> 23) != 0u;
            if (ok) {
                const unsigned M = (sb & 0x7fffffu) | 0x800000u;
                const unsigned M2 = M + ((M & 1u) ? it.a1 : it.a0);
                if (M2 < (1u << 24)) s = __uint_as_float(((unsigned)(it.cls + 127) << 23) | (M2 & 0x7fffffu));
                else ok = false;
            }
            if (!ok) {
                int first = it.last;
                while (first > 0 && sc.cls[first - 1] == it.cls) first--;
#pragma unroll 1
                for (int j = first; j <= it.last; j++) s = seq2_literal(s, sq + j * S, E, vec);
                fallbacks++;
            }
        }
        sc.result[0] = s;
        sc.info[1] = fallbacks;
    }
    sync();
    return sc.result[0];
}

__device__ __forceinline__ float block_seqsum_exact_v2(const float *sq, int n, SeqSum2Scratch sc) {
    return block_seqsum_exact_v2_t<SEQSUM2_THREADS>(sq, n, sc, (int)threadIdx.x, SeqSum2BlockSync());
}
```

### gpullama3.java_b200/csrc/stream_matvec.cuh

```cuda
#pragma once
#include "common.cuh"
#include "decode_kernels.cuh"
#include "norm_slots.cuh"

#define SMV_CONSUMER_WARPS 8
#define SMV_THREADS ((SMV_CONSUMER_WARPS + 1) * 32)
#define SMV_MAX_STAGES 16
#define SMV_HVALS 512

enum { SMV_STORE = 0, SMV_RESID = 1, SMV_GATEUP = 2 };

struct TileMat {
    const unsigned char *base;
    int rows, cols;
    int seg, nseg;
    int unit_bytes;
};

__host__ __device__ inline int smv_pick_nseg(int cols) {
    for (int n = 1; n <= 64; n++)
        if (cols % n == 0 && (cols / n) % 32 == 0 && cols / n <= 2560) return n;
    return 0;
}
__host__ __device__ inline int smv_unit_bytes(int seg) { return (seg + seg / 16 + 15) & ~15; }
__host__ __device__ inline int tile_groups(const TileMat &W) { return (W.rows + 3) >> 2; }

struct SmvSmem {
    size_t off_bar, off_xq, off_xs, off_terms, off_hvals, off_ring, total;
    int stages, stage_bytes, nbs_pad;
};

__host__ __device__ inline SmvSmem smv_layout(int cols, int seg, size_t budget) {
    SmvSmem L;
    int unit = smv_unit_bytes(seg);
    L.stage_bytes = (4 * unit + 127) & ~127;
    L.nbs_pad = ((seg / 32 + 3) & ~3) + 4;
    size_t o = 0;
    L.off_bar = o; o += 2 * SMV_MAX_STAGES * 8 + SMV_MAX_STAGES * 4;
    L.off_xq = o; o += (size_t)cols;
    L.off_xs = o; o += (size_t)(cols / 32) * 4;
    o = (o + 15) & ~(size_t)15;
    L.off_terms = o; o += (size_t)SMV_CONSUMER_WARPS * 4 * L.nbs_pad * 4;
    L.off_hvals = o; o += SMV_HVALS * 4;
    o = (o + 127) & ~(size_t)127;
    L.off_ring = o;
    long room = (long)budget - (long)o;
    int s = room > 0 ? (int)(room / L.stage_bytes) : 0;
    if (s > SMV_MAX_STAGES) s = SMV_MAX_STAGES;
    L.stages = s;
    L.total = o + (size_t)s * L.stage_bytes;
    return L;
}

__device__ __forceinline__ unsigned smem_u32(const void *p) { return (unsigned)__cvta_generic_to_shared(p); }
__device__ __forceinline__ void mbar_init(unsigned bar, unsigned count) {
    asm volatile("mbarrier.init.shared::cta.b64 [%0], %1;" ::"r"(bar), "r"(count));
}
__device__ __forceinline__ void mbar_expect_tx(unsigned bar, unsigned bytes) {
    asm volatile("mbarrier.arrive.expect_tx.shared::cta.b64 _, [%0], %1;" ::"r"(bar), "r"(bytes) : "memory");
}
__device__ __forceinline__ void mbar_arrive(unsigned bar) {
    asm volatile("mbarrier.arrive.shared::cta.b64 _, [%0];" ::"r"(bar) : "memory");
}
__device__ __forceinline__ void mbar_wait(unsigned bar, unsigned parity) {
    asm volatile(
        "{\n"
        ".reg .pred p;\n"
        "WAIT_LOOP:\n"
        "mbarrier.try_wait.parity.shared::cta.b64 p, [%0], %1;\n"
        "@p bra WAIT_DONE;\n"
        "bra WAIT_LOOP;\n"
        "WAIT_DONE:\n"
        "}\n" ::"r"(bar), "r"(parity)
        : "memory");
}
__device__ __forceinline__ unsigned long long l2_policy_evict_first() {
    unsigned long long pol;
    asm volatile("createpolicy.fractional.L2::evict_first.b64 %0, 1.0;" : "=l"(pol));
    return pol;
}
__device__ __forceinline__ void bulk_g2s_evict_first(unsigned dst, const void *src, unsigned bytes, unsigned bar, unsigned long long pol) {
    asm volatile("cp.async.bulk.shared::cluster.global.mbarrier::complete_tx::bytes.L2::cache_hint [%0], [%1], %2, [%3], %4;" ::"r"(dst), "l"(src),
                 "r"(bytes), "r"(bar), "l"(pol)
                 : "memory");
}
__device__ __forceinline__ void consumer_bar_sync() { asm volatile("bar.sync 1, %0;" ::"n"(SMV_CONSUMER_WARPS * 32) : "memory"); }
struct SmvConsumerSync {
    __device__ __forceinline__ void operator()() const { consumer_bar_sync(); }
};

__device__ __forceinline__ float ldcg_f32(const float *p) {
    float v;
    asm volatile("ld.global.cg.f32 %0, [%1];" : "=f"(v) : "l"(p));
    return v;
}

__device__ __forceinline__ float swiglu_exact(float g, float u) {
    float s = __fdiv_rn(g, (float)(1.0 + exp((double)(-g))));
    return __fmul_rn(s, u);
}

__device__ __forceinline__ float pd_walk_terms(float acc, const float *t, int nbs) {
    int b = 0;
    if (nbs >= 16) {
        float4 c0 = *reinterpret_cast<const float4 *>(t), c1 = *reinterpret_cast<const float4 *>(t + 4);
        float4 c2 = *reinterpret_cast<const float4 *>(t + 8), c3 = *reinterpret_cast<const float4 *>(t + 12);
        for (; b + 16 <= nbs; b += 16) {
            float4 n0 = c0, n1 = c1, n2 = c2, n3 = c3;
            if (b + 32 <= nbs) {
                n0 = *reinterpret_cast<const float4 *>(t + b + 16); n1 = *reinterpret_cast<const float4 *>(t + b + 20);
                n2 = *reinterpret_cast<const float4 *>(t + b + 24); n3 = *reinterpret_cast<const float4 *>(t + b + 28);
            }
            acc = __fadd_rn(acc, c0.x); acc = __fadd_rn(acc, c0.y); acc = __fadd_rn(acc, c0.z); acc = __fadd_rn(acc, c0.w);
            acc = __fadd_rn(acc, c1.x); acc = __fadd_rn(acc, c1.y); acc = __fadd_rn(acc, c1.z); acc = __fadd_rn(acc, c1.w);
            acc = __fadd_rn(acc, c2.x); acc = __fadd_rn(acc, c2.y); acc = __fadd_rn(acc, c2.z); acc = __fadd_rn(acc, c2.w);
            acc = __fadd_rn(acc, c3.x); acc = __fadd_rn(acc, c3.y); acc = __fadd_rn(acc, c3.z); acc = __fadd_rn(acc, c3.w);
            c0 = n0; c1 = n1; c2 = n2; c3 = n3;
        }
    }
    for (; b + 4 <= nbs; b += 4) {
        const float4 v = *reinterpret_cast<const float4 *>(t + b);
        acc = __fadd_rn(acc, v.x); acc = __fadd_rn(acc, v.y); acc = __fadd_rn(acc, v.z); acc = __fadd_rn(acc, v.w);
    }
    for (; b < nbs; b++) acc = __fadd_rn(acc, t[b]);
    return acc;
}

struct SmvArgs {
    TileMat W;
    const int8_t *xq;
    const float *xs;
    float *out;
    float oscale;
    int8_t *hq;
    float *hs;
    unsigned *blk_cnt;
    float *part_val;
    int *part_idx;
    TraceBuf tr;
    TpCtx tp;
    int wait_slot;
    unsigned wait_op;
    int out_slot;
    unsigned out_op;
    int row_base;
};

struct SmvNormArgs {
    const float *x;
    const float *w;
    const StepState *st;
    DevMat emb;
    float emb_scale, eps;
    int from_emb;
    float *x_out;
    unsigned off_sq, off_seq;
};

__host__ inline SmvSmem smv_layout_norm(int cols, int seg, size_t budget, unsigned *off_sq, unsigned *off_seq) {
    SmvSmem L = smv_layout(cols, seg, budget);
    const size_t sq = (size_t)norm_slots_sq_floats(cols, SMV_CONSUMER_WARPS * 32) * 4;
    const size_t nb = sq + seqsum2_scratch_bytes(SMV_CONSUMER_WARPS * 32);
    *off_sq = (unsigned)L.off_terms;
    *off_seq = (unsigned)(L.off_terms + sq);
    const size_t dead = L.off_ring - L.off_terms;
    size_t o = L.off_terms + (nb > dead ? nb : dead);
    o = (o + 127) & ~(size_t)127;
    L.off_ring = o;
    long room = (long)budget - (long)o;
    int s = room > 0 ? (int)(room / L.stage_bytes) : 0;
    if (s > SMV_MAX_STAGES) s = SMV_MAX_STAGES;
    L.stages = s;
    L.total = o + (size_t)s * L.stage_bytes;
    return L;
}

__device__ __noinline__ float smv_seqsum(const float *sq, int n, int S, unsigned char *scratch, int tid) {
    return block_seqsum_exact_v2_t<SMV_CONSUMER_WARPS * 32>(sq, n, seqsum2_carve(scratch, SMV_CONSUMER_WARPS * 32), tid, SmvConsumerSync(), S);
}

struct SmvNormOps {
    const SmvNormArgs &n;
    unsigned char *smem;
    int tid;
    bool write_x;
    __device__ __forceinline__ void sync() const { consumer_bar_sync(); }
    __device__ __forceinline__ float seqsum(const float *sq, int cnt, int S) const { return smv_seqsum(sq, cnt, S, smem + n.off_seq, tid); }
    __device__ __forceinline__ float emb(int token, int i) const { return emb_get(n.emb, token, i, n.emb_scale); }
    __device__ __forceinline__ float4 x4(int i4) const { return ldcg_f32x4(n.x + 4 * i4); }
    __device__ __forceinline__ void store_x(int i4, float4 v) const {
        if (write_x) *reinterpret_cast<float4 *>(n.x_out + 4 * i4) = v;
    }
    __device__ __forceinline__ float scale(float ss, int dim, float eps) const {
        ss = __fdiv_rn(ss, (float)dim);
        ss = __fadd_rn(ss, eps);
        return (float)(1.0 / sqrt((double)ss));
    }
    template <int U> __device__ __forceinline__ float4 w4(const float4 (&wv)[U], int u, int) const { return wv[u]; }
    __device__ __forceinline__ void stamp(int) const {}
};

template <int U>
__device__ __forceinline__ void smv_norm_prologue(const SmvNormArgs &n, int cols, unsigned char *smem, size_t off_xq, size_t off_xs, int tid, const TraceBuf &tr) {
    constexpr int T = SMV_CONSUMER_WARPS * 32;
    const int n4 = cols >> 2;
    float4 wv[U];
#pragma unroll
    for (int u = 0; u < U; u++) {
        const int i4 = u * T + tid;
        wv[u] = i4 < n4 ? __ldg(reinterpret_cast<const float4 *>(n.w) + i4) : make_float4(0.f, 0.f, 0.f, 0.f);
    }
    pdl_wait();
    trace_mark(tr, 2);
    const int token = n.from_emb ? n.st->token : 0;
    norm_quant_slots<T, U>(SmvNormOps{n, smem, tid, n.from_emb && blockIdx.x == 0}, n.from_emb != 0, token, cols, n.eps, wv,
                           reinterpret_cast<float *>(smem + n.off_sq), reinterpret_cast<unsigned *>(smem + off_xq), reinterpret_cast<float *>(smem + off_xs), tid);
}

template <int MODE, bool NORM>
__device__ __forceinline__ void smv_q8_body(const SmvArgs &a, const SmvSmem &L, const SmvNormArgs &na, unsigned char *smem) {
    const int tid = threadIdx.x, lane = tid & 31, warp = tid >> 5;
    const TileMat W = a.W;
    const int S = L.stages;
    const unsigned bar0 = smem_u32(smem + L.off_bar);
    const int ngroups = tile_groups(W);
    const int g0 = (int)(((long long)blockIdx.x * ngroups) / gridDim.x);
    const int g1 = (int)(((long long)(blockIdx.x + 1) * ngroups) / gridDim.x);
    const int nseg = W.nseg;
    const unsigned tile_bytes = 4u * (unsigned)W.unit_bytes;

    volatile unsigned *rel = reinterpret_cast<volatile unsigned *>(smem + L.off_bar + 2 * SMV_MAX_STAGES * 8);
    if (tid == 0) {
        for (int s = 0; s < S; s++) {
            mbar_init(bar0 + 8 * s, 1);
            mbar_init(bar0 + 8 * (SMV_MAX_STAGES + s), 1);
            rel[s] = 0u;
        }
        asm volatile("fence.mbarrier_init.release.cluster;" ::: "memory");
    }
    __syncthreads();
    trace_entry(a.tr);
    pdl_launch_dependents();

    if (warp == SMV_CONSUMER_WARPS) {
        if (lane == 0) {
            unsigned seq = 0;
            const unsigned long long pol = l2_policy_evict_first();
            for (int gb = g0; gb < g1; gb += SMV_CONSUMER_WARPS) {
                int nw = min(SMV_CONSUMER_WARPS, g1 - gb);
                for (int s = 0; s < nseg; s++)
#pragma unroll 1
                    for (int w = 0; w < nw; w++, seq++) {
                        int st = seq % S;
                        unsigned ph = (seq / S) & 1u;
                        mbar_wait(bar0 + 8 * (SMV_MAX_STAGES + st), ph ^ 1u);
                        unsigned full = bar0 + 8 * st;
                        mbar_expect_tx(full, tile_bytes);
                        const unsigned char *src = W.base + ((size_t)(gb + w) * nseg + s) * tile_bytes;
                        bulk_g2s_evict_first(smem_u32(smem + L.off_ring + (size_t)st * L.stage_bytes), src, tile_bytes, full, pol);
                    }
            }
        }
        return;
    }

    if (NORM) {
        const int U = ((W.cols >> 2) + SMV_CONSUMER_WARPS * 32 - 1) / (SMV_CONSUMER_WARPS * 32);
        if (U <= 1) smv_norm_prologue<1>(na, W.cols, smem, L.off_xq, L.off_xs, tid, a.tr);
        else if (U == 2) smv_norm_prologue<2>(na, W.cols, smem, L.off_xq, L.off_xs, tid, a.tr);
        else if (U <= 4) smv_norm_prologue<4>(na, W.cols, smem, L.off_xq, L.off_xs, tid, a.tr);
        else smv_norm_prologue<5>(na, W.cols, smem, L.off_xq, L.off_xs, tid, a.tr);
    } else {
        pdl_wait();
        trace_mark(a.tr, 2);
        if (a.tp.n > 1 && a.wait_slot >= 0) {
            if (tid == 0) tp_wait(a.tp, a.wait_slot, tp_seq(a.tp, a.wait_op));
            consumer_bar_sync();
        }
        {
            const int nb = W.cols >> 5;
            int4 *sxq = reinterpret_cast<int4 *>(smem + L.off_xq);
            float *sxs = reinterpret_cast<float *>(smem + L.off_xs);
            const int4 *src = reinterpret_cast<const int4 *>(a.xq);
            for (int c = tid; c < W.cols / 16; c += SMV_CONSUMER_WARPS * 32) sxq[c] = __ldcg(src + c);
            for (int b = tid; b < nb; b += SMV_CONSUMER_WARPS * 32) sxs[b] = __ldcg(a.xs + b);
        }
        consumer_bar_sync();
    }

    const int nbs = W.seg >> 5;
    float *terms = reinterpret_cast<float *>(smem + L.off_terms) + (size_t)warp * 4 * L.nbs_pad;
    const unsigned char *sact = smem + L.off_xq;
    const float *sxs = reinterpret_cast<const float *>(smem + L.off_xs);
    const int hsel = (lane >> 2) & 1;

    float *hvals = reinterpret_cast<float *>(smem + L.off_hvals);
    float best = -INFINITY;
    int best_i = 0x7fffffff;

    unsigned seq_base = 0;
    for (int gb = g0; gb < g1; gb += SMV_CONSUMER_WARPS) {
        const int nw = min(SMV_CONSUMER_WARPS, g1 - gb);
        if (warp < nw) {
            const int G = gb + warp;
            float acc = 0.0f;
            for (int s = 0; s < nseg; s++) {
                const unsigned seq = seq_base + (unsigned)(s * nw + warp);
                const int st = seq % S;
                const unsigned lap = seq / S;
                if (lane == 0)
                    while (rel[st] != lap) {}
                __syncwarp();
                mbar_wait(bar0 + 8 * st, lap & 1u);
                const unsigned char *tile = smem + L.off_ring + (size_t)st * L.stage_bytes;
                for (int b = lane; b < nbs; b += 32) {
                    const unsigned char *ab = sact + ((size_t)(s * nbs + b) << 5);
                    const int4 a0 = *reinterpret_cast<const int4 *>(ab + 16 * hsel);
                    const int4 a1 = *reinterpret_cast<const int4 *>(ab + 16 * (hsel ^ 1));
                    const float as = sxs[s * nbs + b];
#pragma unroll
                    for (int r = 0; r < 4; r++) {
                        const unsigned char *wb = tile + (size_t)r * W.unit_bytes + ((size_t)b << 5);
                        const int4 w0 = *reinterpret_cast<const int4 *>(wb + 16 * hsel);
                        const int4 w1 = *reinterpret_cast<const int4 *>(wb + 16 * (hsel ^ 1));
                        const __half sc = *reinterpret_cast<const __half *>(tile + (size_t)r * W.unit_bytes + W.seg + 2 * b);
                        int isum = __dp4a(w0.x, a0.x, 0);
                        isum = __dp4a(w0.y, a0.y, isum);
                        isum = __dp4a(w0.z, a0.z, isum);
                        isum = __dp4a(w0.w, a0.w, isum);
                        isum = __dp4a(w1.x, a1.x, isum);
                        isum = __dp4a(w1.y, a1.y, isum);
                        isum = __dp4a(w1.z, a1.z, isum);
                        isum = __dp4a(w1.w, a1.w, isum);
                        terms[r * L.nbs_pad + b] = __fmul_rn((float)isum, __fmul_rn(__half2float(sc), as));
                    }
                }
                __syncwarp();
                if (lane == 0) {
                    rel[st] = lap + 1u;
                    mbar_arrive(bar0 + 8 * (SMV_MAX_STAGES + st));
                }
                if (lane < 4) acc = pd_walk_terms(acc, terms + lane * L.nbs_pad, nbs);
                __syncwarp();
            }
            if (MODE == SMV_GATEUP) {
                const float up = __shfl_down_sync(0xffffffffu, acc, 2);
                if (lane < 2) {
                    const int unit = 2 * G + lane;
                    const float hval = swiglu_exact(acc, up);
                    a.out[unit] = hval;
                    hvals[unit - 2 * g0] = hval;
                }
            } else if (lane < 4 && 4 * G + lane < W.rows) {
                const size_t row = (size_t)4 * G + lane;
                acc = __fmul_rn(acc, a.oscale);
                if (MODE == SMV_RESID) {
                    if (a.tp.n > 1) {
                        const size_t grow = (size_t)a.row_base + row;
                        const float v = __fadd_rn(ldcg_f32c(a.out + grow), acc);
                        for (int k = 0; k < a.tp.n; k++) tp_ptr<float>(a.tp, k, a.tp.off_x)[grow] = v;
                    } else a.out[row] = __fadd_rn(a.out[row], acc);
                } else {
                    a.out[row] = acc;
                    const int grow = a.row_base + (int)row;
                    if (acc > best) { best = acc; best_i = grow; }
                }
            }
        }
        seq_base += (unsigned)(nseg * nw);
    }

    if (MODE == SMV_GATEUP) {
        consumer_bar_sync();
        const int u0 = 2 * g0, u1 = 2 * g1;
        if (u1 > u0) {
            for (int blk = (u0 >> 5) + warp; blk <= ((u1 - 1) >> 5); blk += SMV_CONSUMER_WARPS) {
                const int lo = max(blk << 5, u0), hi = min((blk << 5) + 32, u1);
                float v = 0.0f;
                bool mine = true;
                if (hi - lo == 32) v = hvals[(blk << 5) + lane - u0];
                else {
                    unsigned old = 0;
                    if (lane == 0) {
                        __threadfence();
                        old = atomicAdd(&a.blk_cnt[blk], (unsigned)(hi - lo));
                    }
                    old = __shfl_sync(0xffffffffu, old, 0);
                    mine = (old + (unsigned)(hi - lo) == 32u);
                    if (mine) {
                        __threadfence();
                        v = ldcg_f32(a.out + (blk << 5) + lane);
                        if (lane == 0) a.blk_cnt[blk] = 0u;
                    }
                }
                if (mine) {
                    float as;
                    int q = quant_block_lane(v, as);
                    if (a.tp.n > 1) {
                        const int gblk = (a.row_base >> 5) + blk;
                        for (int k = 0; k < a.tp.n; k++) {
                            tp_ptr<int8_t>(a.tp, k, a.tp.off_hq)[(gblk << 5) + lane] = (int8_t)q;
                            if (lane == 0) tp_ptr<float>(a.tp, k, a.tp.off_hs)[gblk] = as;
                        }
                    } else {
                        a.hq[(blk << 5) + lane] = (int8_t)q;
                        if (lane == 0) a.hs[blk] = as;
                    }
                }
            }
        }
    } else if (MODE == SMV_STORE) {
        if (a.part_val) {
            int *cand_i = reinterpret_cast<int *>(hvals + 64);
            if (lane < 4) { hvals[warp * 4 + lane] = best; cand_i[warp * 4 + lane] = best_i; }
            consumer_bar_sync();
            if (tid == 0) {
                float bv = -INFINITY;
                int bi = 0x7fffffff;
                for (int k = 0; k < SMV_CONSUMER_WARPS * 4; k++) {
                    float v = hvals[k];
                    int ix = cand_i[k];
                    if (v > bv || (v == bv && ix < bi)) { bv = v; bi = ix; }
                }
                a.part_val[blockIdx.x] = bv;
                a.part_idx[blockIdx.x] = bi;
            }
        }
    }
    if (a.tp.n > 1 && a.out_slot >= 0) {
        consumer_bar_sync();
        if (tid == 0) tp_cta_done(a.tp, a.out_slot, tp_seq(a.tp, a.out_op), gridDim.x);
    }
    trace_mark(a.tr, 3);
}

template <int MODE>
__global__ void __launch_bounds__(SMV_THREADS, 1) k_stream_matvec_q8(SmvArgs a, SmvSmem L) {
    extern __shared__ __align__(128) unsigned char smem[];
    smv_q8_body<MODE, false>(a, L, SmvNormArgs{}, smem);
}

template <int MODE>
__global__ void __maxnreg__(96) k_stream_matvec_q8_norm(SmvArgs a, SmvSmem L, SmvNormArgs n) {
    static_assert(MODE != SMV_RESID, "a residual matvec consumes an activation, not the residual stream");
    extern __shared__ __align__(128) unsigned char smem[];
    smv_q8_body<MODE, true>(a, L, n, smem);
}

struct RepackSrc {
    const unsigned char *raw[3];
    int rows[3];
    int row0[3];
    int gateup;
};

__global__ void k_repack_tiles(RepackSrc src, unsigned char *dst, int rows, int cols, int seg, int nseg, int unit_bytes) {
    const long long unit_id = blockIdx.x;
    const int r = (int)(unit_id % 4);
    const int s = (int)((unit_id / 4) % nseg);
    const long long G = unit_id / (4LL * nseg);
    long long row;
    const unsigned char *raw;
    if (src.gateup) {
        raw = src.raw[r >> 1];
        row = src.row0[r >> 1] + 2 * G + (r & 1);
    } else {
        row = 4 * G + r;
        int k = 0;
        while (k < 2 && row >= src.rows[k]) { row -= src.rows[k]; k++; }
        raw = src.raw[k];
        row += src.row0[k];
    }
    const int nbs = seg / 32;
    const bool pad = !src.gateup && 4 * G + r >= rows;
    const unsigned char *blocks = pad ? nullptr : raw + ((size_t)row * (cols / 32) + (size_t)s * nbs) * 34;
    unsigned char *u = dst + (size_t)unit_id * unit_bytes;
    const int words = unit_bytes / 2;
    for (int w = threadIdx.x; w < words; w += blockDim.x) {
        unsigned short v = 0;
        if (pad) {
        } else if (w < seg / 2) {
// ... 27 lines not shown
```

### gpullama3.java_b200/native.py

```python
from __future__ import annotations

import ctypes as C
import os

import numpy as np

_HERE = os.path.dirname(os.path.abspath(__file__))
LIB_PATH = os.path.join(_HERE, "csrc", "libb200llama.so")

B200_OK = 0
ERRORS = {-1: "BAD_ARG", -2: "UNSUPPORTED", -3: "OOM", -4: "CUDA", -5: "NCCL", -6: "STATE"}


class B200Error(RuntimeError):
    def __init__(self, code: int, msg: str):
        super().__init__(f"b200llama error {ERRORS.get(code, code)}: {msg}")
        self.code = code


class UnsupportedOperation(B200Error):
    """Counterpart of the reference's UnsupportedOperationException (ForwardPlanFactory.java:84-87)."""


class Config(C.Structure):
    _fields_ = [(n, C.c_int32) for n in ("arch", "dim", "hidden_dim", "n_layers", "n_heads", "n_kv_heads", "head_size",
                                        "vocab_size", "context_length")] + \
               [("rms_norm_eps", C.c_float), ("rope_theta", C.c_float), ("fp16_lanes", C.c_int32),
                ("tp_rank", C.c_int32), ("tp_size", C.c_int32)]


class MoeConfig(C.Structure):
    _fields_ = [(n, C.c_int32) for n in ("n_experts", "n_experts_used", "expert_hidden_dim", "shared_hidden_dim")]


class GraniteConfig(C.Structure):
    _fields_ = [(n, C.c_float) for n in ("embedding_scale", "residual_scale", "attention_scale", "logit_scale")]


class Tensor(C.Structure):
    _fields_ = [("name", C.c_char_p), ("data", C.c_void_p), ("ggml_type", C.c_int32), ("n_dims", C.c_int32),
                ("dims", C.c_int64 * 4)]


EXPORTS = ["b200_plan_create", "b200_plan_create_moe", "b200_plan_create_granite", "b200_forward_decode", "b200_forward_prefill", "b200_forward_batch_prefill", "b200_set_prefill_mode", "b200_prefill_info",
           "b200_set_decode_mode", "b200_decode_info", "b200_trace_persistent", "b200_test_seqsum2", "b200_test_sample", "b200_forward_decode_sample", "b200_upload_info", "b200_requant_kquant",
           "b200_decode_sequence", "b200_time_kernel", "b200_tp_handle", "b200_tp_attach", "b200_trace_decode", "b200_profile_norm", "b200_gemm_f16", "b200_test_gemm", "b200_test_gemm_q8", "b200_test_pf_attention", "b200_kv_reset", "b200_read_buffer", "b200_launches_per_decode",
           "b200_set_decode_slots", "b200_forward_decode_batch", "b200_slot_reset", "b200_slot_copy_kv", "b200_prefill_slots", "b200_test_pf_attention_packed", "b200_batch_info",
           "b200_forward_decode_multi", "b200_decode_multi_rows",
           "b200_device_bytes", "b200_plan_free", "b200_last_error", "b200_version"]

_lib = None


def lib() -> C.CDLL:
    global _lib
    if _lib is not None:
        return _lib
    if not os.path.exists(LIB_PATH):
        raise RuntimeError(f"{LIB_PATH} is missing: run `python -c 'import __graft_entry__ as g; g.build()'` "
                           "(there is no CPU fallback)")
    L = C.CDLL(LIB_PATH)
    vp, i32 = C.c_void_p, C.c_int32
    L.b200_plan_create.argtypes = [C.POINTER(Config), C.POINTER(Tensor), i32, i32, i32, C.POINTER(vp), C.c_char_p, C.c_size_t]
    L.b200_plan_create_moe.argtypes = [C.POINTER(Config), C.POINTER(MoeConfig), C.POINTER(Tensor), i32, i32, i32, C.POINTER(vp), C.c_char_p, C.c_size_t]
    L.b200_plan_create_granite.argtypes = [C.POINTER(Config), C.POINTER(GraniteConfig), C.POINTER(Tensor), i32, i32, i32, C.POINTER(vp), C.c_char_p, C.c_size_t]
    L.b200_forward_decode.argtypes = [vp, i32, i32, vp, C.POINTER(i32)]
    L.b200_forward_prefill.argtypes = [vp, i32, i32]
    L.b200_forward_decode_sample.argtypes = [vp, i32, i32, C.c_float, C.c_float, C.c_float, C.POINTER(i32), C.POINTER(i32)]
    L.b200_forward_batch_prefill.argtypes = [vp, vp, i32, i32]
    L.b200_decode_sequence.argtypes = [vp, vp, i32, i32, i32, vp, C.POINTER(C.c_float)]
    L.b200_kv_reset.argtypes = [vp]
    L.b200_profile_norm.argtypes = [vp, C.POINTER(C.c_int64)]
    L.b200_trace_decode.argtypes = [vp, i32, i32, vp, i32, C.POINTER(i32)]
    L.b200_tp_handle.argtypes = [vp, vp]
    L.b200_tp_attach.argtypes = [vp, vp, i32]
    L.b200_set_prefill_mode.argtypes = [vp, i32]
    L.b200_set_decode_mode.argtypes = [vp, i32]
    L.b200_decode_info.argtypes = [vp, C.POINTER(i32), C.POINTER(i32), C.POINTER(i32), C.POINTER(i32)]
    L.b200_trace_persistent.argtypes = [vp, i32, i32, vp, C.c_int64, C.POINTER(i32), C.POINTER(i32), C.POINTER(i32)]
    L.b200_test_seqsum2.argtypes = [vp, i32, i32, C.POINTER(C.c_float), C.POINTER(i32)]
    L.b200_test_sample.argtypes = [vp, i32, C.c_float, C.c_float, C.c_float, C.POINTER(i32), C.POINTER(i32), vp]
    L.b200_prefill_info.argtypes = [vp, C.POINTER(i32), C.POINTER(i32), C.POINTER(C.c_float)]
    L.b200_gemm_f16.argtypes = [vp, vp, vp, i32, i32, i32, i32, C.POINTER(C.c_float)]
    L.b200_test_gemm.argtypes = [i32, i32, i32, i32, i32, i32, i32, vp, vp, vp, vp]
    L.b200_test_gemm_q8.argtypes = [i32, i32, i32, i32, i32, i32, i32, vp, vp, vp, vp]
    L.b200_test_pf_attention.argtypes = [vp, vp, vp, i32, i32, i32, i32, i32, i32, vp]
    L.b200_time_kernel.argtypes = [vp, i32, i32, C.POINTER(C.c_float), C.POINTER(C.c_int64)]
    L.b200_read_buffer.argtypes = [vp, C.c_char_p, i32, vp, C.c_size_t]
    L.b200_set_decode_slots.argtypes = [vp, i32]
    L.b200_forward_decode_batch.argtypes = [vp, i32, vp, vp, vp, vp, vp, vp]
    L.b200_slot_reset.argtypes = [vp, i32]
    L.b200_slot_copy_kv.argtypes = [vp, i32, i32]
    L.b200_prefill_slots.argtypes = [vp, i32, vp, vp, vp, vp]
    L.b200_test_pf_attention_packed.argtypes = [i32, vp, vp, vp, vp, vp, i32, i32, i32, vp]
    L.b200_batch_info.argtypes = [vp, C.POINTER(i32), C.POINTER(i32), C.POINTER(C.c_float)]
    L.b200_forward_decode_multi.argtypes = [vp, i32, i32, vp, i32, vp, vp]
    L.b200_decode_multi_rows.argtypes = [vp, C.POINTER(i32)]
    L.b200_upload_info.argtypes = [vp, C.POINTER(C.c_double), C.POINTER(C.c_double), C.POINTER(C.c_int64)]
    L.b200_launches_per_decode.argtypes = [vp]
    L.b200_device_bytes.argtypes = [vp]
    L.b200_device_bytes.restype = C.c_int64
    L.b200_plan_free.argtypes = [vp]
    L.b200_plan_free.restype = None
    L.b200_last_error.argtypes = [vp]
    L.b200_last_error.restype = C.c_char_p
    L.b200_version.restype = C.c_char_p
    _lib = L
    return L


def _raise(code: int, msg: str):
    if code == -2:
        raise UnsupportedOperation(code, msg)
    raise B200Error(code, msg)


def test_seqsum(terms, want_info: bool = False, threads: int = 1024):
    t = np.ascontiguousarray(terms, dtype=np.float32)
    out = C.c_float(0)
    info = (C.c_int32 * 2)()
    rc = lib().b200_test_seqsum2(t.ctypes.data, len(t), threads, C.byref(out), info)
    if rc != B200_OK:
        _raise(rc, "b200_test_seqsum2 failed")
    return (out.value, info[0], info[1]) if want_info else out.value


def test_sample(logits, temperature: float, topp: float, uniform01: float):
    lg = np.ascontiguousarray(logits, dtype=np.float32)
    probs = np.empty(len(lg), dtype=np.float32)
    out = C.c_int32(-1)
    info = (C.c_int32 * 4)()
    rc = lib().b200_test_sample(lg.ctypes.data, len(lg), temperature, topp, uniform01, C.byref(out), info, probs.ctypes.data)
    if rc != B200_OK:
        _raise(rc, "b200_test_sample failed")
    return out.value, list(info), probs


def requant_kquant(ggml_type: int, raw, n_elems: int) -> np.ndarray:
    raw = np.ascontiguousarray(raw, dtype=np.uint8)
    out = np.empty(n_elems // 32 * 34, dtype=np.uint8)
    lib().b200_requant_kquant.argtypes = [C.c_int32, C.c_void_p, C.c_int64, C.c_void_p]
    rc = lib().b200_requant_kquant(int(ggml_type), raw.ctypes.data, int(n_elems), out.ctypes.data)
    if rc != B200_OK:
        _raise(rc, "b200_requant_kquant failed")
    return out


def gemm_f16(a, b, iters: int = 0):
    a = np.ascontiguousarray(a, dtype=np.float16)
    b = np.ascontiguousarray(b, dtype=np.float16)
    m, k = a.shape
    n, k2 = b.shape
    if k != k2:
        raise ValueError("inner dimensions differ")
    c = np.empty((m, n), dtype=np.float32)
    ms = C.c_float(0)
    rc = lib().b200_gemm_f16(a.ctypes.data, b.ctypes.data, c.ctypes.data, m, n, k, iters, C.byref(ms))
    if rc != B200_OK:
        _raise(rc, "b200_gemm_f16 failed")
    return c, (ms.value if iters > 0 else None)


GEMM_MODES = {"f32": 0, "resid": 1, "gateup": 2}


def test_gemm(mode: str, a, b, c, b2=None, m_valid: int | None = None, stages: int = 4, splits: int = 1) -> np.ndarray:
    a = np.ascontiguousarray(a, dtype=np.float16)
    b = np.ascontiguousarray(b, dtype=np.float16)
    gateup = mode == "gateup"
    c = np.array(c, dtype=np.float16 if gateup else np.float32, order="C", copy=True)
    m, k = a.shape
    n = b.shape[0]
    if b.shape != (n, k) or c.shape != (m, n):
        raise ValueError("shapes do not match")
    if gateup:
        b2 = np.ascontiguousarray(b2, dtype=np.float16)
        if b2.shape != b.shape:
            raise ValueError("b2 must have the shape of b")
    rc = lib().b200_test_gemm(GEMM_MODES[mode], stages, splits, m, m if m_valid is None else m_valid, n, k, a.ctypes.data, b.ctypes.data,
                              b2.ctypes.data if gateup else None, c.ctypes.data)
    if rc != B200_OK:
        _raise(rc, "b200_test_gemm failed")
    return c


def test_gemm_q8(mode: str, a, bq, c, bq2=None, m_valid: int | None = None, stages: int = 4, splits: int = 1) -> np.ndarray:
    a = np.ascontiguousarray(a, dtype=np.float16)
    bq = np.ascontiguousarray(bq, dtype=np.uint8)
    gateup = mode == "gateup"
    c = np.array(c, dtype=np.float16 if gateup else np.float32, order="C", copy=True)
    m, k = a.shape
    n = bq.shape[0]
    if bq.shape != (n, k // 32 * 34) or k % 32 or c.shape != (m, n):
        raise ValueError("shapes do not match")
    if gateup:
        bq2 = np.ascontiguousarray(bq2, dtype=np.uint8)
        if bq2.shape != bq.shape:
            raise ValueError("bq2 must have the shape of bq")
    rc = lib().b200_test_gemm_q8(GEMM_MODES[mode], stages, splits, m, m if m_valid is None else m_valid, n, k, a.ctypes.data, bq.ctypes.data,
                                 bq2.ctypes.data if gateup else None, c.ctypes.data)
    if rc != B200_OK:
        _raise(rc, "b200_test_gemm_q8 failed")
    return c


def test_pf_attention_packed(qs, ks, vs, starts, n_heads: int, n_kv_heads: int, sentinel: int = 0x7E5A) -> list:
    lens = np.array([len(q) for q in qs], dtype=np.int32)
    st = np.ascontiguousarray(starts, dtype=np.int32)
    hs = qs[0].shape[1] // n_heads
    q = np.ascontiguousarray(np.concatenate(qs), dtype=np.float32)
    k = np.ascontiguousarray(np.concatenate(ks), dtype=np.float32)
    v = np.ascontiguousarray(np.concatenate(vs), dtype=np.float32)
    if len(st) != len(qs) or any(len(ks[i]) != st[i] + lens[i] or len(vs[i]) != st[i] + lens[i] for i in range(len(qs))):
        raise ValueError("ks[i] / vs[i] must be [starts[i] + n_i, n_kv_heads * head_size]")
    out = np.full((int(lens.sum()), n_heads * hs), sentinel, dtype=np.uint16)
    rc = lib().b200_test_pf_attention_packed(len(qs), lens.ctypes.data, st.ctypes.data, q.ctypes.data, k.ctypes.data, v.ctypes.data, n_heads,
                                             n_kv_heads, hs, out.ctypes.data)
    if rc != B200_OK:
        _raise(rc, "b200_test_pf_attention_packed failed")
    return np.split(out, np.cumsum(lens)[:-1])


def test_pf_attention(q, k, v, n_heads: int, n_kv_heads: int, start_pos: int, impl: str = "mma", out_rows: int | None = None,
                      sentinel: int = 0x7E5A) -> np.ndarray:
    if impl != "mma":
        raise ValueError(f"no prefill attention kernel {impl!r}: the prefill runs k_pf_attention_mma (impl='mma')")
    q = np.ascontiguousarray(q, dtype=np.float32)
    k = np.ascontiguousarray(k, dtype=np.float32)
    v = np.ascontiguousarray(v, dtype=np.float32)
    n, qd = q.shape
    hs = qd // n_heads
    if k.shape != (start_pos + n, n_kv_heads * hs) or v.shape != k.shape:
        raise ValueError("k / v must be [start_pos + n, n_kv_heads * head_size]")
    rows = n if out_rows is None else out_rows
    out = np.full((rows, qd), sentinel, dtype=np.uint16)
    rc = lib().b200_test_pf_attention(q.ctypes.data, k.ctypes.data, v.ctypes.data, n, start_pos, n_heads, n_kv_heads, hs,
                                      rows, out.ctypes.data)
    if rc != B200_OK:
        _raise(rc, "b200_test_pf_attention failed")
    return out


GGML_SIZES = {0: (4, 1), 1: (2, 1), 8: (34, 32), 12: (144, 256), 13: (176, 256), 14: (210, 256)}


class NativePlan:

    def __init__(self, cfg: Config, tensors: dict, prefill_batch_size: int = 0, device: int = 0, moe: MoeConfig | None = None,
                 granite: GraniteConfig | None = None):
        L = lib()
        arr = (Tensor * len(tensors))()
        self._keep = []
        for i, (name, (tt, dims, raw)) in enumerate(tensors.items()):
            raw = np.ascontiguousarray(raw)
            ts_bs = GGML_SIZES.get(int(tt))
            n_el = int(np.prod(dims))
            if ts_bs is not None and (n_el % ts_bs[1] or raw.nbytes != n_el // ts_bs[1] * ts_bs[0]):
                raise B200Error(-1, f"tensor {name}: {raw.nbytes} bytes do not hold {n_el} elements of ggml type {int(tt)}")
            self._keep.append(raw)
            arr[i].name = name.encode()
            arr[i].data = raw.ctypes.data
            arr[i].ggml_type = int(tt)
            arr[i].n_dims = len(dims)
            for k, d in enumerate(dims):
                arr[i].dims[k] = int(d)
        out = C.c_void_p()
        err = C.create_string_buffer(512)
        if granite is not None:
            rc = L.b200_plan_create_granite(C.byref(cfg), C.byref(granite), arr, len(tensors), prefill_batch_size, device, C.byref(out), err, 512)
        elif moe is not None:
            rc = L.b200_plan_create_moe(C.byref(cfg), C.byref(moe), arr, len(tensors), prefill_batch_size, device, C.byref(out), err, 512)
        else:
            rc = L.b200_plan_create(C.byref(cfg), arr, len(tensors), prefill_batch_size, device, C.byref(out), err, 512)
        self._keep = None
        if rc != B200_OK:
            _raise(rc, err.value.decode())
        self._p = out
        self.cfg = cfg
        self.moe = moe

    def _ck(self, rc: int):
        if rc != B200_OK:
            _raise(rc, lib().b200_last_error(self._p).decode())

    def forward_decode(self, token: int, position: int, want_logits: bool = True, want_argmax: bool = True):
        logits = np.empty(self.cfg.vocab_size, dtype=np.float32) if want_logits else None
        am = C.c_int32(-1)
        self._ck(lib().b200_forward_decode(self._p, token, position, logits.ctypes.data if want_logits else None,
                                           C.byref(am) if want_argmax else None))
        return logits, (am.value if want_argmax else None)

    def forward_decode_sample(self, token: int, position: int, temperature: float, topp: float, uniform01: float, want_info: bool = False):
        out = C.c_int32(-1)
        info = (C.c_int32 * 4)()
        self._ck(lib().b200_forward_decode_sample(self._p, token, position, temperature, topp, uniform01, C.byref(out), info))
        return (out.value, list(info)) if want_info else out.value

    def forward_prefill(self, token: int, position: int):
        self._ck(lib().b200_forward_prefill(self._p, token, position))

    def set_prefill_mode(self, mode: int):
        self._ck(lib().b200_set_prefill_mode(self._p, mode))

    def set_decode_mode(self, mode: int):
        self._ck(lib().b200_set_decode_mode(self._p, mode))

    def decode_info(self):
        a, b, c, d = C.c_int32(0), C.c_int32(0), C.c_int32(0), C.c_int32(0)
        self._ck(lib().b200_decode_info(self._p, C.byref(a), C.byref(b), C.byref(c), C.byref(d)))
        return a.value, b.value, c.value, d.value

    def trace_persistent(self, token: int, position: int) -> np.ndarray:
        cap = 200 * (self.cfg.n_layers + 1) * 32
        buf = np.zeros(cap, dtype=np.uint64)
        a, b, c = C.c_int32(0), C.c_int32(0), C.c_int32(0)
        self._ck(lib().b200_trace_persistent(self._p, token, position, buf.ctypes.data, cap, C.byref(a), C.byref(b), C.byref(c)))
        return buf[: a.value * b.value * c.value].reshape(a.value, b.value, c.value)

    def prefill_info(self):
        mode, launches, ms = C.c_int32(0), C.c_int32(0), C.c_float(0)
        self._ck(lib().b200_prefill_info(self._p, C.byref(mode), C.byref(launches), C.byref(ms)))
        return mode.value, launches.value, ms.value

    def forward_batch_prefill(self, tokens, start_pos: int):
        t = np.ascontiguousarray(tokens, dtype=np.int32)
        self._ck(lib().b200_forward_batch_prefill(self._p, t.ctypes.data, len(t), start_pos))

    def decode_sequence(self, tokens, n: int, start_pos: int, feedback: bool = False):
        t = np.ascontiguousarray(tokens, dtype=np.int32)
        out = np.empty(n, dtype=np.int32)
        ms = C.c_float(0)
        self._ck(lib().b200_decode_sequence(self._p, t.ctypes.data, n, start_pos, 1 if feedback else 0, out.ctypes.data, C.byref(ms)))
        return out, ms.value

    def set_decode_slots(self, n_slots: int):
        self._ck(lib().b200_set_decode_slots(self._p, n_slots))

    def forward_decode_batch(self, slots, tokens, positions, sampling=None, want_logits: bool = False):
        s = np.ascontiguousarray(slots, dtype=np.int32)
        t = np.ascontiguousarray(tokens, dtype=np.int32)
        p = np.ascontiguousarray(positions, dtype=np.int32)
        n = len(s)
        if len(t) != n or len(p) != n:
            raise ValueError("slots, tokens and positions must have the same length")
        smp = None
        if sampling is not None:
            smp = np.ascontiguousarray(sampling, dtype=np.float32).reshape(-1)
            if smp.size != 3 * n:
                raise ValueError("sampling must hold (temperature, topp, uniform01) per row")
        ids = np.empty(n, dtype=np.int32)
        lg = np.empty((n, self.cfg.vocab_size), dtype=np.float32) if want_logits else None
        self._ck(lib().b200_forward_decode_batch(self._p, n, s.ctypes.data, t.ctypes.data, p.ctypes.data, smp.ctypes.data if smp is not None else None,
                                                 ids.ctypes.data, lg.ctypes.data if want_logits else None))
        return ids, lg

    def slot_reset(self, slot: int):
        self._ck(lib().b200_slot_reset(self._p, slot))

    def slot_copy_kv(self, slot: int, n_positions: int):
        self._ck(lib().b200_slot_copy_kv(self._p, slot, n_positions))

    def prefill_slots(self, slots, start_positions, token_lists):
        s = np.ascontiguousarray(slots, dtype=np.int32)
        st = np.ascontiguousarray(start_positions, dtype=np.int32)
        if len(st) != len(s) or len(token_lists) != len(s):
            raise ValueError("slots, start_positions and token_lists must have the same length")
        ln = np.array([len(t) for t in token_lists], dtype=np.int32)
        toks = np.ascontiguousarray(np.concatenate([np.asarray(t, dtype=np.int32).reshape(-1) for t in token_lists]) if len(s) else np.zeros(0), dtype=np.int32)
        self._ck(lib().b200_prefill_slots(self._p, len(s), s.ctypes.data, st.ctypes.data, ln.ctypes.data, toks.ctypes.data))

    def batch_info(self):
        a, b, ms = C.c_int32(0), C.c_int32(0), C.c_float(0)
        self._ck(lib().b200_batch_info(self._p, C.byref(a), C.byref(b), C.byref(ms)))
        return a.value, b.value, ms.value

    def forward_decode_multi(self, slot: int, tokens, start_pos: int, want_logits: bool = False):
        t = np.ascontiguousarray(tokens, dtype=np.int32).reshape(-1)
        n = len(t)
        ids = np.empty(max(n, 1), dtype=np.int32)
        lg = np.empty((n, self.cfg.vocab_size), dtype=np.float32) if want_logits else None
        self._ck(lib().b200_forward_decode_multi(self._p, slot, n, t.ctypes.data, start_pos, ids.ctypes.data, lg.ctypes.data if want_logits else None))
        return ids[:n], lg

    def decode_multi_rows(self) -> int:
        r = C.c_int32(0)
        self._ck(lib().b200_decode_multi_rows(self._p, C.byref(r)))
        return r.value

    def time_kernel(self, which: int, reps: int = 3):
        ms, nbytes = C.c_float(0), C.c_int64(0)
        self._ck(lib().b200_time_kernel(self._p, which, reps, C.byref(ms), C.byref(nbytes)))
        return ms.value, nbytes.value

    def tp_handle(self) -> bytes:
        buf = C.create_string_buffer(64)
        self._ck(lib().b200_tp_handle(self._p, buf))
        return buf.raw

    def tp_attach(self, handles: list):
        blob = b"".join(handles)
        self._ck(lib().b200_tp_attach(self._p, blob, len(handles)))

    def trace_decode(self, token: int, position: int):
        cap = self.launches_per_decode + 8
        rec = np.zeros((cap, 4), dtype=np.uint64)
        n = C.c_int32(0)
        self._ck(lib().b200_trace_decode(self._p, token, position, rec.ctypes.data, cap, C.byref(n)))
        return rec[: n.value]

    def profile_norm(self):
        a = (C.c_int64 * 16)()
        self._ck(lib().b200_profile_norm(self._p, a))
        return list(a)

    def kv_reset(self):
        self._ck(lib().b200_kv_reset(self._p))

    def read_buffer(self, name: str, n: int, dtype=np.float32, layer: int = 0) -> np.ndarray:
        out = np.empty(n, dtype=dtype)
        self._ck(lib().b200_read_buffer(self._p, name.encode(), layer, out.ctypes.data, out.nbytes))
        return out

    def moe_routing(self):
        k = self.moe.n_experts_used
        ids = self.read_buffer("moe_ids", self.cfg.n_layers * k, np.int32).reshape(self.cfg.n_layers, k)
        w = self.read_buffer("moe_weights", self.cfg.n_layers * (k + 1)).reshape(self.cfg.n_layers, k + 1)
        return ids, w
# ... 26 lines not shown
```

### include/b200llama.h

```cpp
#ifndef B200LLAMA_H
#define B200LLAMA_H

#include <stddef.h>
#include <stdint.h>

#ifdef __cplusplus
extern "C" {
#endif

#define B200_OK 0
#define B200_ERR_BAD_ARG (-1)
#define B200_ERR_UNSUPPORTED (-2)
#define B200_ERR_OOM (-3)
#define B200_ERR_CUDA (-4)
#define B200_ERR_NCCL (-5)
#define B200_ERR_STATE (-6)

#define B200_ARCH_LLAMA 0
#define B200_ARCH_QWEN3 1
#define B200_ARCH_PHI3 2
#define B200_ARCH_QWEN2 3
#define B200_ARCH_QWEN2_MOE 4
#define B200_ARCH_GRANITE 5

#define B200_GGML_F32 0
#define B200_GGML_F16 1
#define B200_GGML_Q8_0 8
#define B200_GGML_Q4_K 12
#define B200_GGML_Q5_K 13
#define B200_GGML_Q6_K 14

typedef struct b200_config {
    int32_t arch;
    int32_t dim;
    int32_t hidden_dim;
    int32_t n_layers;
    int32_t n_heads;
    int32_t n_kv_heads;
    int32_t head_size;
    int32_t vocab_size;
    int32_t context_length;
    float rms_norm_eps;
    float rope_theta;
    int32_t fp16_lanes;
    int32_t tp_rank;
    int32_t tp_size;
} b200_config;

typedef struct b200_tensor {
    const char *name;
    const void *data;
    int32_t ggml_type;
    int32_t n_dims;
    int64_t dims[4];
} b200_tensor;

typedef struct b200_moe_config {
    int32_t n_experts;
    int32_t n_experts_used;
    int32_t expert_hidden_dim;
    int32_t shared_hidden_dim;
} b200_moe_config;

typedef struct b200_granite_config {
    float embedding_scale;
    float residual_scale;
    float attention_scale;
    float logit_scale;
} b200_granite_config;

typedef struct b200_plan b200_plan;

int b200_plan_create(const b200_config *cfg, const b200_tensor *tensors, int32_t n_tensors,
                     int32_t prefill_batch_size, int32_t device, b200_plan **out, char *err, size_t err_len);

int b200_plan_create_moe(const b200_config *cfg, const b200_moe_config *moe, const b200_tensor *tensors, int32_t n_tensors,
                         int32_t prefill_batch_size, int32_t device, b200_plan **out, char *err, size_t err_len);

int b200_plan_create_granite(const b200_config *cfg, const b200_granite_config *granite, const b200_tensor *tensors, int32_t n_tensors,
                             int32_t prefill_batch_size, int32_t device, b200_plan **out, char *err, size_t err_len);

int b200_forward_decode(b200_plan *plan, int32_t token, int32_t position, float *logits, int32_t *argmax);

int b200_forward_decode_sample(b200_plan *plan, int32_t token, int32_t position, float temperature, float topp, float uniform01,
                               int32_t *token_out, int32_t *info);

int b200_forward_prefill(b200_plan *plan, int32_t token, int32_t position);

int b200_forward_batch_prefill(b200_plan *plan, const int32_t *tokens, int32_t n, int32_t start_pos);

#define B200_PREFILL_EXACT 0
#define B200_PREFILL_TENSOR_CORE 1
#define B200_PREFILL_TENSOR_CORE_W8A16 2
int b200_set_prefill_mode(b200_plan *plan, int32_t mode);

int b200_prefill_info(b200_plan *plan, int32_t *mode, int32_t *launches, float *device_ms);

#define B200_DECODE_GRAPH 0
#define B200_DECODE_PERSISTENT 1
int b200_set_decode_mode(b200_plan *plan, int32_t mode);

int b200_decode_info(b200_plan *plan, int32_t *mode, int32_t *launches, int32_t *ring_stages, int32_t *smem_bytes);

int b200_decode_sequence(b200_plan *plan, const int32_t *tokens, int32_t n, int32_t start_pos,
                         int32_t feedback, int32_t *out_ids, float *device_ms);

int b200_kv_reset(b200_plan *plan);

#define B200_MAX_DECODE_SLOTS 8

int b200_set_decode_slots(b200_plan *plan, int32_t n_slots);

int b200_forward_decode_batch(b200_plan *plan, int32_t n, const int32_t *slots, const int32_t *tokens, const int32_t *positions,
                              const float *sampling , int32_t *ids_out, float *logits );

int b200_slot_reset(b200_plan *plan, int32_t slot);

int b200_slot_copy_kv(b200_plan *plan, int32_t slot, int32_t n_positions);

int b200_prefill_slots(b200_plan *plan, int32_t n_seqs, const int32_t *slots, const int32_t *start_positions, const int32_t *lengths,
                       const int32_t *tokens);

int b200_forward_decode_multi(b200_plan *plan, int32_t slot, int32_t n, const int32_t *tokens, int32_t start_pos, int32_t *ids_out,
                              float *logits );

int b200_decode_multi_rows(b200_plan *plan, int32_t *max_rows);

int b200_batch_info(b200_plan *plan, int32_t *n_slots, int32_t *launches_per_step, float *device_ms_last_step);

int b200_read_buffer(b200_plan *plan, const char *name, int32_t layer, void *dst, size_t bytes);

int b200_time_kernel(b200_plan *plan, int32_t which, int32_t reps, float *avg_ms, int64_t *algorithmic_bytes);

int b200_tp_handle(b200_plan *plan, void *handle64);
int b200_tp_attach(b200_plan *plan, const void *handles, int32_t n);

int b200_trace_decode(b200_plan *plan, int32_t token, int32_t position, uint64_t *records, int32_t cap, int32_t *n_out);

int b200_trace_persistent(b200_plan *plan, int32_t token, int32_t position, uint64_t *stamps, int64_t cap, int32_t *n_ctas, int32_t *n_rows, int32_t *n_stamps);

int b200_profile_norm(b200_plan *plan, int64_t *cycles);

int b200_test_seqsum2(const float *terms, int32_t n, int32_t threads, float *out, int32_t *info );

int b200_test_sample(const float *logits, int32_t n, float temperature, float topp, float uniform01,
                     int32_t *token_out, int32_t *info , float *probs_out );

int b200_requant_kquant(int32_t ggml_type, const void *src, int64_t n_elems, void *dst_q8_0);

int b200_gemm_f16(const uint16_t *a, const uint16_t *b, float *c, int32_t m, int32_t n, int32_t k, int32_t iters, float *ms );

int b200_test_gemm(int32_t mode, int32_t stages, int32_t splits, int32_t m, int32_t m_valid, int32_t n, int32_t k, const uint16_t *a, const uint16_t *b,
                   const uint16_t *b2 , void *c);

int b200_test_gemm_q8(int32_t mode, int32_t stages, int32_t splits, int32_t m, int32_t m_valid, int32_t n, int32_t k, const uint16_t *a, const void *bq,
                      const void *bq2 , void *c);

int b200_test_pf_attention(const float *q, const float *k, const float *v, int32_t n, int32_t start_pos, int32_t n_heads,
                           int32_t n_kv_heads, int32_t head_size, int32_t out_rows, uint16_t *out);

int b200_test_pf_attention_packed(int32_t n_seqs, const int32_t *lengths, const int32_t *start_positions, const float *q, const float *k,
                                  const float *v, int32_t n_heads, int32_t n_kv_heads, int32_t head_size, uint16_t *out);

int b200_upload_info(b200_plan *plan, double *seconds, double *host_copy_seconds, int64_t *h2d_bytes);

int b200_launches_per_decode(b200_plan *plan);

int64_t b200_device_bytes(b200_plan *plan);

void b200_plan_free(b200_plan *plan);

const char *b200_last_error(b200_plan *plan);

const char *b200_version(void);

#ifdef __cplusplus
}
#endif
#endif
```

Before: 241.9.

## Rewrite exact sequential block sum with fewer barriers and redundant final fold

```diff
diff --git a/gpullama3.java_b200/csrc/decode_kernels.cuh b/gpullama3.java_b200/csrc/decode_kernels.cuh
--- a/gpullama3.java_b200/csrc/decode_kernels.cuh
+++ b/gpullama3.java_b200/csrc/decode_kernels.cuh
@@ -17,8 +17,12 @@
 __device__ __forceinline__ float emb_get(const DevMat &e, int token, int i, float es) { return __fmul_rn(emb_get_raw(e, token, i), es); }
 
 #define NORM_THREADS SEQSUM2_THREADS
+#define NORM_SUM_THREADS 256
 __host__ __device__ inline int norm_padded(int dim) { return (dim + SEQSUM2_THREADS - 1) / SEQSUM2_THREADS * SEQSUM2_THREADS; }
-__host__ __device__ inline size_t norm_smem_bytes(int dim) { return (size_t)norm_padded(dim) * 4 + 16 + seqsum2_scratch_bytes(); }
+__host__ __device__ inline size_t norm_smem_bytes(int dim) { return (size_t)norm_padded(dim) * 4 + 16 + seqsum3_scratch_bytes(NORM_SUM_THREADS); }
+struct NormSumSync {
+    __device__ __forceinline__ void operator()() const { asm volatile("bar.sync 1, %0;" ::"n"(NORM_SUM_THREADS) : "memory"); }
+};
 
 template <bool EMBED>
 __device__ __forceinline__ void rmsnorm_quant_row(float *__restrict__ x, const int *__restrict__ tok, const DevMat &emb, float emb_scale,
@@ -52,8 +56,9 @@
     __syncthreads();
     if (prof) t2 = clock64();
     int info0 = 0, info1 = 0;
-    SeqSum2Scratch scratch = seqsum2_carve(reinterpret_cast<unsigned char *>(sm + norm_padded(dim)));
-    float ss = block_seqsum_exact_v2(sq, dim, scratch);
+    SeqSum3Scratch scratch = seqsum3_carve(reinterpret_cast<unsigned char *>(sm + norm_padded(dim)), NORM_SUM_THREADS);
+    float ss = 0.0f;
+    if (tid < NORM_SUM_THREADS) ss = block_seqsum_exact_v3_t<NORM_SUM_THREADS>(sq, dim, scratch, tid, NormSumSync());
     if (prof && tid == 0) { info0 = scratch.info[0]; info1 = scratch.info[1]; }
     if (prof) t3 = clock64();
     if (EMBED) __threadfence_block();
@@ -108,17 +113,35 @@
     rmsnorm_quant_row<EMBED>(x, &st->token, emb, emb_scale, w, eps, dim, xq, xs, xb, prof, tr, tp, tp_wait_op);
 }
 
+struct SeqClockStamp {
+    long long *c;
+    __device__ __forceinline__ void operator()(int k) const {
+        if (threadIdx.x == 0) c[k] = clock64();
+    }
+};
 template <int T>
-__global__ void __launch_bounds__(T, 1) k_test_seqsum2(const float *__restrict__ terms, int n, float *__restrict__ out, int *__restrict__ info) {
+__global__ void __launch_bounds__(T, 1) k_test_seqsum2(const float *__restrict__ terms, int n, float *__restrict__ out, int *__restrict__ info,
+                                                   long long *__restrict__ cyc) {
     extern __shared__ __align__(16) float sm[];
+    __shared__ long long st[12];
     float *sq = sm;
     const int E = (n + T - 1) / T, np = T * E;
-    SeqSum2Scratch scratch = seqsum2_carve(reinterpret_cast<unsigned char *>(sm + np), T);
+    SeqSum3Scratch scratch = seqsum3_carve(reinterpret_cast<unsigned char *>(sm + np), T);
     for (int i = threadIdx.x; i < np; i += T) sq[i] = i < n ? terms[i] : 0.0f;
     if (threadIdx.x == 0) { scratch.info[0] = -1; scratch.info[1] = -2; }
     __syncthreads();
-    const float s = block_seqsum_exact_v2_t<T>(sq, n, scratch, (int)threadIdx.x, SeqSum2BlockSync());
-    if (threadIdx.x == 0) { out[0] = s; info[0] = scratch.info[0]; info[1] = scratch.info[1]; }
+    float s = 0.0f;
+#pragma unroll 1
+    for (int r = 0; r < 2; r++) {
+        if (threadIdx.x == 0) st[6 * r] = clock64();
+        s = block_seqsum_exact_v3_t<T>(sq, n, scratch, (int)threadIdx.x, SeqSum2BlockSync(), 0, SeqClockStamp{st + 6 * r});
+        if (threadIdx.x == 0) st[6 * r + 5] = clock64();
+        __syncthreads();
+    }
+    if (threadIdx.x == 0) {
+        out[0] = s; info[0] = scratch.info[0]; info[1] = scratch.info[1];
+        for (int k = 0; k < 12; k++) cyc[k] = st[k];
+    }
 }
 
 template <int R>
diff --git a/gpullama3.java_b200/csrc/decode_persistent.cuh b/gpullama3.java_b200/csrc/decode_persistent.cuh
--- a/gpullama3.java_b200/csrc/decode_persistent.cuh
+++ b/gpullama3.java_b200/csrc/decode_persistent.cuh
@@ -80,7 +80,7 @@
     L.off_wbuf = o; o += (size_t)dim * 4;
     L.off_rope = o; o += (size_t)head_size * 4;
     o = (o + 15) & ~(size_t)15;
-    L.off_seq = o; o += seqsum2_scratch_bytes(PD_CT);
+    L.off_seq = o; o += seqsum3_scratch_bytes(PD_CT);
     o = (o + 15) & ~(size_t)15;
     L.off_terms = o; o += (size_t)PD_WARPS * 4 * L.tstride * 4;
     L.off_hvals = o; o += SMV_HVALS * 4;
@@ -400,8 +400,13 @@
 }
 
 __device__ __noinline__ float pd_seqsum(const float *sq, int n, int S, unsigned char *smem, const PdSmem &L, int tid) {
-    SeqSum2Scratch scratch = seqsum2_carve(smem + L.off_seq, PD_CT);
-    return block_seqsum_exact_v2_t<PD_CT>(sq, n, scratch, tid, PdConsumerSync(), S);
+    SeqSum3Scratch scratch = seqsum3_carve(smem + L.off_seq, PD_CT);
+    return block_seqsum_exact_v3_t<PD_CT>(sq, n, scratch, tid, PdConsumerSync(), S);
+}
+__device__ __noinline__ float pd_seqsum_fenced(const float *sq, int n, unsigned char *smem, const PdSmem &L, int tid) {
+    const float s = pd_seqsum(sq, n, 0, smem, L, tid);
+    pd_bar_sync();
+    return s;
 }
 
 __device__ __forceinline__ void pd_prefetch_w(const float *w, float *sbuf, int dim, int tid) {
@@ -423,15 +428,10 @@
     __device__ __forceinline__ float4 x4(int i4) const { return ldcg_f32x4(a.x + 4 * i4); }
     __device__ __forceinline__ void store_x(int, float4) const {}
     __device__ __forceinline__ float scale(float ss, int dim, float eps) const {
-        float *misc = reinterpret_cast<float *>(smem + L.off_misc);
-        if (tid == 0) {
-            ss = __fdiv_rn(ss, (float)dim);
-            ss = __fadd_rn(ss, eps);
-            misc[20] = (float)(1.0 / sqrt((double)ss));
-        }
+        ss = __fdiv_rn(ss, (float)dim);
+        ss = __fadd_rn(ss, eps);
         asm volatile("cp.async.wait_group 0;" ::: "memory");
-        pd_bar_sync();
-        return misc[20];
+        return (float)(1.0 / sqrt((double)ss));
     }
     template <int U> __device__ __forceinline__ float4 w4(const float4 (&)[U], int, int i4) const { return *reinterpret_cast<const float4 *>(wbuf + 4 * i4); }
     __device__ __forceinline__ void stamp(int k) const { if (stamp_layer >= 0) pd_stamp(a, stamp_layer, k, tid); }
@@ -611,7 +611,7 @@
         const int E = (nt + PD_CT - 1) / PD_CT;
         for (int t = nt + tid; t < PD_CT * E; t += PD_CT) att[t] = 0.0f;
         pd_bar_sync();
-        sum = pd_seqsum(att, nt, 0, smem, L, tid);
+        sum = pd_seqsum_fenced(att, nt, smem, L, tid);
     } else {
         if (tid == 0) s_val[0] = seq2_literal(0.0f, att, nt, (reinterpret_cast<uintptr_t>(att) & 15) == 0);
         pd_bar_sync();
diff --git a/gpullama3.java_b200/csrc/plan.cu b/gpullama3.java_b200/csrc/plan.cu
--- a/gpullama3.java_b200/csrc/plan.cu
+++ b/gpullama3.java_b200/csrc/plan.cu
@@ -2495,34 +2495,38 @@
     return e == cudaSuccess ? B200_OK : B200_ERR_CUDA;
 }
 
-int b200_test_seqsum2(const float *terms, int32_t n, int32_t threads, float *out, int32_t *info) {
+int b200_test_seqsum2(const float *terms, int32_t n, int32_t threads, float *out, int32_t *info, int64_t *cycles) {
     if (!terms || !out || n <= 0 || n > 8192) return B200_ERR_BAD_ARG;
     if (threads != 256 && threads != 512 && threads != 1024) return B200_ERR_BAD_ARG;
     float *d = nullptr, *o = nullptr;
     if (cudaMalloc(&d, (size_t)n * 4) != cudaSuccess) return B200_ERR_OOM;
-    if (cudaMalloc(&o, 16) != cudaSuccess) { cudaFree(d); return B200_ERR_OOM; }
+    if (cudaMalloc(&o, 16 + 12 * 8) != cudaSuccess) { cudaFree(d); return B200_ERR_OOM; }
+    long long *dc = reinterpret_cast<long long *>(o + 4);
     cudaError_t e = cudaMemcpy(d, terms, (size_t)n * 4, cudaMemcpyHostToDevice);
     if (e == cudaSuccess) {
         if (threads == 1024) {
-            const size_t smem = (size_t)1024 * ((n + 1023) / 1024) * 4 + seqsum2_scratch_bytes(1024);
+            const size_t smem = (size_t)1024 * ((n + 1023) / 1024) * 4 + seqsum3_scratch_bytes(1024);
             e = cudaFuncSetAttribute(k_test_seqsum2<1024>, cudaFuncAttributeMaxDynamicSharedMemorySize, (int)smem);
-            if (e == cudaSuccess) k_test_seqsum2<1024><<<1, 1024, smem>>>(d, n, o, reinterpret_cast<int *>(o) + 1);
+            if (e == cudaSuccess) k_test_seqsum2<1024><<<1, 1024, smem>>>(d, n, o, reinterpret_cast<int *>(o) + 1, dc);
         } else if (threads == 512) {
-            const size_t smem = (size_t)512 * ((n + 511) / 512) * 4 + seqsum2_scratch_bytes(512);
+            const size_t smem = (size_t)512 * ((n + 511) / 512) * 4 + seqsum3_scratch_bytes(512);
             e = cudaFuncSetAttribute(k_test_seqsum2<512>, cudaFuncAttributeMaxDynamicSharedMemorySize, (int)smem);
-            if (e == cudaSuccess) k_test_seqsum2<512><<<1, 512, smem>>>(d, n, o, reinterpret_cast<int *>(o) + 1);
+            if (e == cudaSuccess) k_test_seqsum2<512><<<1, 512, smem>>>(d, n, o, reinterpret_cast<int *>(o) + 1, dc);
         } else {
-            const size_t smem = (size_t)256 * ((n + 255) / 256) * 4 + seqsum2_scratch_bytes(256);
+            const size_t smem = (size_t)256 * ((n + 255) / 256) * 4 + seqsum3_scratch_bytes(256);
             e = cudaFuncSetAttribute(k_test_seqsum2<256>, cudaFuncAttributeMaxDynamicSharedMemorySize, (int)smem);
-            if (e == cudaSuccess) k_test_seqsum2<256><<<1, 256, smem>>>(d, n, o, reinterpret_cast<int *>(o) + 1);
+            if (e == cudaSuccess) k_test_seqsum2<256><<<1, 256, smem>>>(d, n, o, reinterpret_cast<int *>(o) + 1, dc);
         }
     }
     if (e == cudaSuccess) e = cudaGetLastError();
     if (e == cudaSuccess) e = cudaDeviceSynchronize();
     int32_t host[3] = {0, 0, 0};
     if (e == cudaSuccess) e = cudaMemcpy(host, o, 12, cudaMemcpyDeviceToHost);
+    long long hc[12] = {0};
+    if (e == cudaSuccess) e = cudaMemcpy(hc, dc, sizeof(hc), cudaMemcpyDeviceToHost);
     memcpy(out, host, 4);
     if (info) { info[0] = host[1]; info[1] = host[2]; }
+    if (cycles) for (int k = 0; k < 12; k++) cycles[k] = hc[k];
     cudaFree(d);
     cudaFree(o);
     return e == cudaSuccess ? B200_OK : B200_ERR_CUDA;
diff --git a/gpullama3.java_b200/csrc/sampler.cuh b/gpullama3.java_b200/csrc/sampler.cuh
--- a/gpullama3.java_b200/csrc/sampler.cuh
+++ b/gpullama3.java_b200/csrc/sampler.cuh
@@ -14,7 +14,7 @@
 };
 
 __host__ __device__ inline int sampler_padded(int n) { return (n + SAMPLER_THREADS - 1) / SAMPLER_THREADS * SAMPLER_THREADS; }
-__host__ __device__ inline size_t sampler_smem_bytes() { return seqsum2_scratch_bytes(SAMPLER_THREADS) + 96 * 4; }
+__host__ __device__ inline size_t sampler_smem_bytes() { return seqsum3_scratch_bytes(SAMPLER_THREADS) + 96 * 4; }
 
 __device__ __forceinline__ int sampler_cmp(const float *p, int a, int b) {
     const float va = p[a], vb = p[b];
@@ -34,8 +34,8 @@
 
 __global__ void __launch_bounds__(SAMPLER_THREADS, 1) k_sample(SamplerArgs a) {
     extern __shared__ __align__(16) unsigned char smp_sm[];
-    SeqSum2Scratch scratch = seqsum2_carve(smp_sm, SAMPLER_THREADS);
-    float *red = reinterpret_cast<float *>(smp_sm + seqsum2_scratch_bytes(SAMPLER_THREADS));
+    SeqSum3Scratch scratch = seqsum3_carve(smp_sm, SAMPLER_THREADS);
+    float *red = reinterpret_cast<float *>(smp_sm + seqsum3_scratch_bytes(SAMPLER_THREADS));
     int *redi = reinterpret_cast<int *>(red + 32);
     const int tid = threadIdx.x, lane = tid & 31, warp = tid >> 5, n = a.n;
     float *p = a.logits;
@@ -53,7 +53,7 @@
     for (int w = 1; w < SAMPLER_THREADS / 32; w++) mx = fmaxf(mx, red[w]);
     for (int i = tid; i < n; i += SAMPLER_THREADS) p[i] = (float)exp((double)__fsub_rn(p[i], mx));
     __syncthreads();
-    const float sum = block_seqsum_exact_v2_t<SAMPLER_THREADS>(p, n, scratch, tid, SeqSum2BlockSync());
+    const float sum = block_seqsum_exact_v3_t<SAMPLER_THREADS>(p, n, scratch, tid, SeqSum2BlockSync());
     if (tid == 0 && a.info) { a.info[2] = scratch.info[0]; a.info[3] = scratch.info[1]; }
     __syncthreads();
     for (int i = tid; i < n; i += SAMPLER_THREADS) p[i] = __fdiv_rn(p[i], sum);
diff --git a/gpullama3.java_b200/csrc/seqsum2.cuh b/gpullama3.java_b200/csrc/seqsum2.cuh
--- a/gpullama3.java_b200/csrc/seqsum2.cuh
+++ b/gpullama3.java_b200/csrc/seqsum2.cuh
@@ -40,43 +40,31 @@
 }
 
 struct SeqItem {
-    int cls;
+    unsigned lo;
     unsigned a0, a1;
-    int last;
-};
-
-struct SeqSum2Scratch {
+    unsigned span;
+};
+
+struct SeqSum3Scratch {
+    SeqItem *items;
     float *wsum;
-    SeqPair *wtail;
-    int *wtail_f;
-    int *wcls_last;
-    int *wcls_first;
     int *wcnt;
-    int *cls;
-    SeqItem *items;
-    float *result;
     int *info;
 };
-__host__ __device__ inline size_t seqsum2_scratch_bytes(int T = SEQSUM2_THREADS) {
-    return 32 * 4 + 32 * sizeof(SeqPair) + 4 * 32 * 4 + (size_t)T * 4 + (size_t)T * sizeof(SeqItem) + 16 + 16;
-}
-__device__ __forceinline__ SeqSum2Scratch seqsum2_carve(unsigned char *p, int T = SEQSUM2_THREADS) {
-    SeqSum2Scratch s;
+__host__ __device__ inline size_t seqsum3_scratch_bytes(int T = SEQSUM2_THREADS) {
+    return (size_t)T * sizeof(SeqItem) + 32 * 4 + 32 * 4 + 16;
+}
+__device__ __forceinline__ SeqSum3Scratch seqsum3_carve(unsigned char *p, int T = SEQSUM2_THREADS) {
+    SeqSum3Scratch s;
     s.items = reinterpret_cast<SeqItem *>(p); p += (size_t)T * sizeof(SeqItem);
-    s.wtail = reinterpret_cast<SeqPair *>(p); p += 32 * sizeof(SeqPair);
-    s.cls = reinterpret_cast<int *>(p); p += (size_t)T * 4;
     s.wsum = reinterpret_cast<float *>(p); p += 32 * 4;
-    s.wtail_f = reinterpret_cast<int *>(p); p += 32 * 4;
-    s.wcls_last = reinterpret_cast<int *>(p); p += 32 * 4;
-    s.wcls_first = reinterpret_cast<int *>(p); p += 32 * 4;
     s.wcnt = reinterpret_cast<int *>(p); p += 32 * 4;
-    s.result = reinterpret_cast<float *>(p); p += 16;
     s.info = reinterpret_cast<int *>(p);
     return s;
 }
 
-__device__ __noinline__ void seq2_warp_segscan(SeqPair &p, int &f, int lane) {
-#pragma unroll 1
+__device__ __forceinline__ void seq_warp_segscan(SeqPair &p, int &f, int lane) {
+#pragma unroll
     for (int d = 1; d < 32; d <<= 1) {
         const unsigned u0 = __shfl_up_sync(0xffffffffu, p.a0, d), u1 = __shfl_up_sync(0xffffffffu, p.a1, d);
         const int fu = __shfl_up_sync(0xffffffffu, f, d);
@@ -92,6 +80,9 @@
 struct SeqSum2BlockSync {
     __device__ __forceinline__ void operator()() const { __syncthreads(); }
 };
+struct SeqNoStamp {
+    __device__ __forceinline__ void operator()(int) const {}
+};
 
 __host__ __device__ inline int seqsum2_stride(int E) { return (E % 4 == 0 && (E / 4) % 2 == 0) ? E + 4 : E; }
 
@@ -109,19 +100,30 @@
     return s;
 }
 
-__device__ __noinline__ float seq2_warp_scan_f(float v, int lane) {
-#pragma unroll 1
-    for (int d = 1; d < 32; d <<= 1) {
-        const float u = __shfl_up_sync(0xffffffffu, v, d);
-        if (lane >= d) v += u;
-    }
-    return v;
-}
-
-template <int T, class Sync>
-__device__ float block_seqsum_exact_v2_t(const float *sq, int n, SeqSum2Scratch sc, int tid, Sync sync, int S = 0) {
-    static_assert(T % 32 == 0 && T <= SEQSUM2_THREADS, "T threads = T/32 whole warps");
+__device__ __forceinline__ float seq_literal_terms(float s, const float *q, int E, bool vec, bool shared) {
+    if (!shared) return seq2_literal(s, q, E, vec);
+    const unsigned a = (unsigned)__cvta_generic_to_shared(q);
+    int k = 0;
+#pragma unroll 1
+    for (; k + 8 <= E; k += 8) {
+        float4 v, u;
+        asm volatile("ld.shared.v4.f32 {%0,%1,%2,%3}, [%4];" : "=f"(v.x), "=f"(v.y), "=f"(v.z), "=f"(v.w) : "r"(a + 4 * k));
+        asm volatile("ld.shared.v4.f32 {%0,%1,%2,%3}, [%4];" : "=f"(u.x), "=f"(u.y), "=f"(u.z), "=f"(u.w) : "r"(a + 4 * k + 16));
+        s = __fadd_rn(s, v.x); s = __fadd_rn(s, v.y); s = __fadd_rn(s, v.z); s = __fadd_rn(s, v.w);
+        s = __fadd_rn(s, u.x); s = __fadd_rn(s, u.y); s = __fadd_rn(s, u.z); s = __fadd_rn(s, u.w);
+    }
+    if (k < E) {
+        float4 v;
+        asm volatile("ld.shared.v4.f32 {%0,%1,%2,%3}, [%4];" : "=f"(v.x), "=f"(v.y), "=f"(v.z), "=f"(v.w) : "r"(a + 4 * k));
+        s = __fadd_rn(s, v.x); s = __fadd_rn(s, v.y); s = __fadd_rn(s, v.z); s = __fadd_rn(s, v.w);
+    }
+    return s;
+}
+
+template <int T, class Sync, class Stamp = SeqNoStamp>
+__device__ float block_seqsum_exact_v3_t(const float *sq, int n, SeqSum3Scratch sc, int tid, Sync sync, int S = 0, Stamp stamp = Stamp()) {
     constexpr int NW = T / 32;
+    static_assert(T % 32 == 0 && T <= SEQSUM2_THREADS && (NW & (NW - 1)) == 0, "T threads = a power-of-two number of whole warps");
     const int lane = tid & 31, warp = tid >> 5;
     const int E = (n + T - 1) / T;
     if (S == 0) S = E;
@@ -141,16 +143,18 @@
 #pragma unroll 1
         for (; k < E; k++) loc += mine[k];
     }
-    const float inc = seq2_warp_scan_f(loc, lane);
+    float inc = loc;
+#pragma unroll
+    for (int d = 1; d < 32; d <<= 1) {
+        const float u = __shfl_up_sync(0xffffffffu, inc, d);
+        if (lane >= d) inc += u;
+    }
     if (lane == 31) sc.wsum[warp] = inc;
     sync();
-    if (warp == 0) {
-        const float w = lane < NW ? sc.wsum[lane] : 0.0f;
-        const float v = seq2_warp_scan_f(w, lane);
-        if (lane < NW) sc.wsum[lane] = v - w;
-    }
-    sync();
-    const float wex = sc.wsum[warp];
+    stamp(1);
+    float wex = (lane & (NW - 1)) < warp ? sc.wsum[lane & (NW - 1)] : 0.0f;
+#pragma unroll
+    for (int d = 1; d < NW; d <<= 1) wex += __shfl_xor_sync(0xffffffffu, wex, d);
     const float p_end = wex + inc, p_start = wex + (inc - loc);
 
     int cls = SEQSUM2_LITERAL;
@@ -182,90 +186,55 @@
             }
         }
     }
-    sc.cls[tid] = cls;
-    if (lane == 31) sc.wcls_last[warp] = cls;
-    if (lane == 0) sc.wcls_first[warp] = cls;
-    sync();
-
-    int prev_cls = __shfl_up_sync(0xffffffffu, cls, 1);
-    if (lane == 0) prev_cls = warp ? sc.wcls_last[warp - 1] : SEQSUM2_LITERAL;
-    int next_cls = __shfl_down_sync(0xffffffffu, cls, 1);
-    if (lane == 31) next_cls = warp < NW - 1 ? sc.wcls_first[warp + 1] : SEQSUM2_LITERAL;
+    stamp(2);
+
+    const int prev_cls = __shfl_up_sync(0xffffffffu, cls, 1), next_cls = __shfl_down_sync(0xffffffffu, cls, 1);
     const bool clean = cls != SEQSUM2_LITERAL;
-    int f = (clean && prev_cls == cls) ? 0 : 1;
-    seq2_warp_segscan(pr, f, lane);
-    if (lane == 31) { sc.wtail[warp] = pr; sc.wtail_f[warp] = f; }
-    sync();
-    if (warp == 0) {
-        SeqPair t;
-        t.a0 = t.a1 = 0u;
-        int tf = 1;
-        if (lane < NW) { t = sc.wtail[lane]; tf = sc.wtail_f[lane]; }
-        seq2_warp_segscan(t, tf, lane);
-        if (lane < NW) sc.wtail[lane] = t;
-    }
-    sync();
-    if (!f && warp > 0) pr = seq_compose(sc.wtail[warp - 1], pr);
-
-    const bool is_item = !clean || next_cls != cls;
-    const unsigned bal = __ballot_sync(0xffffffffu, is_item);
+    const bool starts = !clean || lane == 0 || prev_cls != cls;
+    const bool ends = !clean || lane == 31 || next_cls != cls;
+    int f = starts;
+    seq_warp_segscan(pr, f, lane);
+
+    const unsigned bal = __ballot_sync(0xffffffffu, ends), sbal = __ballot_sync(0xffffffffu, starts);
+    if (ends) {
+        SeqItem it;
+        it.lo = clean ? (unsigned)(cls + 127) << 23 : 0u;
+        it.a0 = pr.a0; it.a1 = pr.a1;
+        it.span = (unsigned)(warp * 32 + 31 - __clz(sbal & (0xffffffffu >> (31 - lane)))) | ((unsigned)tid << 16);
+        sc.items[warp * 32 + __popc(bal & ((1u << lane) - 1u))] = it;
+    }
     if (lane == 0) sc.wcnt[warp] = __popc(bal);
     sync();
-    if (warp == 0) {
-        const int c = lane < NW ? sc.wcnt[lane] : 0;
-        int v = c;
-#pragma unroll 1
-        for (int d = 1; d < 32; d <<= 1) {
-            const int u = __shfl_up_sync(0xffffffffu, v, d);
-            if (lane >= d) v += u;
-        }
-        if (lane < NW) sc.wcnt[lane] = v - c;
-        if (lane == 31) sc.info[0] = v;
-    }
-    sync();
-    if (is_item) {
-        SeqItem it;
-        it.cls = cls; it.a0 = pr.a0; it.a1 = pr.a1; it.last = tid;
-        sc.items[sc.wcnt[warp] + __popc(bal & ((1u << lane) - 1u))] = it;
-    }
-    sync();
-
-    if (tid == 0) {
-        const int n_items = sc.info[0];
-        float s = 0.0f;
-        int fallbacks = 0;
-        SeqItem nxt = sc.items[0];
-#pragma unroll 1
-        for (int i = 0; i < n_items; i++) {
+    stamp(3);
+
+    const bool shared = vec && __isShared(sq);
+    unsigned sb = 0u;
+    int fallbacks = 0, items = 0;
+#pragma unroll 1
+    for (int w = 0; w < NW; w++) {
+        const SeqItem *reg = sc.items + w * 32;
+        const int cnt = sc.wcnt[w];
+        items += cnt;
+        SeqItem nxt = reg[0];
+#pragma unroll 1
+        for (int i = 0; i < cnt; i++) {
             const SeqItem it = nxt;
-            if (i + 1 < n_items) nxt = sc.items[i + 1];
-            if (it.cls == SEQSUM2_LITERAL) {
-                s = seq2_literal(s, sq + it.last * S, E, vec);
-                continue;
-            }
-            const unsigned sb = __float_as_uint(s);
-            bool ok = f32_exponent(s) == it.cls && (sb >> 23) != 0u;
-            if (ok) {
-                const unsigned M = (sb & 0x7fffffu) | 0x800000u;
-                const unsigned M2 = M + ((M & 1u) ? it.a1 : it.a0);
-                if (M2 < (1u << 24)) s = __uint_as_float(((unsigned)(it.cls + 127) << 23) | (M2 & 0x7fffffu));
-                else ok = false;
-            }
-            if (!ok) {
-                int first = it.last;
-                while (first > 0 && sc.cls[first - 1] == it.cls) first--;
-#pragma unroll 1
-                for (int j = first; j <= it.last; j++) s = seq2_literal(s, sq + j * S, E, vec);
+            nxt = reg[i + 1];
+            if (it.lo != 0u) {
+                const unsigned nb = sb + ((sb & 1u) ? it.a1 : it.a0);
+                if (((sb ^ it.lo) | (nb ^ it.lo)) < 0x800000u) {
+                    sb = nb;
+                    continue;
+                }
                 fallbacks++;
             }
-        }
-        sc.result[0] = s;
-        sc.info[1] = fallbacks;
-    }
-    sync();
-    return sc.result[0];
-}
-
-__device__ __forceinline__ float block_seqsum_exact_v2(const float *sq, int n, SeqSum2Scratch sc) {
-    return block_seqsum_exact_v2_t<SEQSUM2_THREADS>(sq, n, sc, (int)threadIdx.x, SeqSum2BlockSync());
-}
+            float s = __uint_as_float(sb);
+#pragma unroll 1
+            for (int j = (int)(it.span & 0xffffu); j <= (int)(it.span >> 16); j++) s = seq_literal_terms(s, sq + j * S, E, vec, shared);
+            sb = __float_as_uint(s);
+        }
+    }
+    if (tid == 0) { sc.info[0] = items; sc.info[1] = fallbacks; }
+    stamp(4);
+    return __uint_as_float(sb);
+}
diff --git a/gpullama3.java_b200/csrc/stream_matvec.cuh b/gpullama3.java_b200/csrc/stream_matvec.cuh
--- a/gpullama3.java_b200/csrc/stream_matvec.cuh
+++ b/gpullama3.java_b200/csrc/stream_matvec.cuh
@@ -160,7 +160,7 @@
 __host__ inline SmvSmem smv_layout_norm(int cols, int seg, size_t budget, unsigned *off_sq, unsigned *off_seq) {
     SmvSmem L = smv_layout(cols, seg, budget);
     const size_t sq = (size_t)norm_slots_sq_floats(cols, SMV_CONSUMER_WARPS * 32) * 4;
-    const size_t nb = sq + seqsum2_scratch_bytes(SMV_CONSUMER_WARPS * 32);
+    const size_t nb = sq + seqsum3_scratch_bytes(SMV_CONSUMER_WARPS * 32);
     *off_sq = (unsigned)L.off_terms;
     *off_seq = (unsigned)(L.off_terms + sq);
     const size_t dead = L.off_ring - L.off_terms;
@@ -176,7 +176,7 @@
 }
 
 __device__ __noinline__ float smv_seqsum(const float *sq, int n, int S, unsigned char *scratch, int tid) {
-    return block_seqsum_exact_v2_t<SMV_CONSUMER_WARPS * 32>(sq, n, seqsum2_carve(scratch, SMV_CONSUMER_WARPS * 32), tid, SmvConsumerSync(), S);
+    return block_seqsum_exact_v3_t<SMV_CONSUMER_WARPS * 32>(sq, n, seqsum3_carve(scratch, SMV_CONSUMER_WARPS * 32), tid, SmvConsumerSync(), S);
 }
 
 struct SmvNormOps {
diff --git a/gpullama3.java_b200/native.py b/gpullama3.java_b200/native.py
--- a/gpullama3.java_b200/native.py
+++ b/gpullama3.java_b200/native.py
@@ -78,7 +78,7 @@
     L.b200_set_decode_mode.argtypes = [vp, i32]
     L.b200_decode_info.argtypes = [vp, C.POINTER(i32), C.POINTER(i32), C.POINTER(i32), C.POINTER(i32)]
     L.b200_trace_persistent.argtypes = [vp, i32, i32, vp, C.c_int64, C.POINTER(i32), C.POINTER(i32), C.POINTER(i32)]
-    L.b200_test_seqsum2.argtypes = [vp, i32, i32, C.POINTER(C.c_float), C.POINTER(i32)]
+    L.b200_test_seqsum2.argtypes = [vp, i32, i32, C.POINTER(C.c_float), C.POINTER(i32), C.POINTER(C.c_int64)]
     L.b200_test_sample.argtypes = [vp, i32, C.c_float, C.c_float, C.c_float, C.POINTER(i32), C.POINTER(i32), vp]
     L.b200_prefill_info.argtypes = [vp, C.POINTER(i32), C.POINTER(i32), C.POINTER(C.c_float)]
     L.b200_gemm_f16.argtypes = [vp, vp, vp, i32, i32, i32, i32, C.POINTER(C.c_float)]
@@ -115,14 +115,20 @@
     raise B200Error(code, msg)
 
 
-def test_seqsum(terms, want_info: bool = False, threads: int = 1024):
+def test_seqsum(terms, want_info: bool = False, threads: int = 1024, want_cycles: bool = False):
     t = np.ascontiguousarray(terms, dtype=np.float32)
     out = C.c_float(0)
     info = (C.c_int32 * 2)()
-    rc = lib().b200_test_seqsum2(t.ctypes.data, len(t), threads, C.byref(out), info)
+    cyc = np.zeros(12, dtype=np.int64)
+    rc = lib().b200_test_seqsum2(t.ctypes.data, len(t), threads, C.byref(out), info, cyc.ctypes.data_as(C.POINTER(C.c_int64)))
     if rc != B200_OK:
         _raise(rc, "b200_test_seqsum2 failed")
-    return (out.value, info[0], info[1]) if want_info else out.value
+    r = (out.value,)
+    if want_info:
+        r += (info[0], info[1])
+    if want_cycles:
+        r += (cyc.reshape(2, 6),)
+    return r if len(r) > 1 else r[0]
 
 
 def test_sample(logits, temperature: float, topp: float, uniform01: float):
diff --git a/include/b200llama.h b/include/b200llama.h
--- a/include/b200llama.h
+++ b/include/b200llama.h
@@ -141,7 +141,7 @@
 
 int b200_profile_norm(b200_plan *plan, int64_t *cycles);
 
-int b200_test_seqsum2(const float *terms, int32_t n, int32_t threads, float *out, int32_t *info );
+int b200_test_seqsum2(const float *terms, int32_t n, int32_t threads, float *out, int32_t *info , int64_t *cycles );
 
 int b200_test_sample(const float *logits, int32_t n, float temperature, float topp, float uniform01,
                      int32_t *token_out, int32_t *info , float *probs_out );
```

New measurement: 249.7, median of 6. 1.03x the previous value.
